# sloisel/MultiGridBarrier.jl

Measured on AMD Instinct MI355X. Metric: Newton iters/sec + wall-clock to converge, 2D P2 p-Laplace L=9, higher is better.
Workload: dtype f64

## Files before the change

### include/mgbhip.h

```cpp
#ifndef MGBHIP_H
#define MGBHIP_H

#include <stdint.h>

#ifdef __cplusplus
extern "C" {
#endif

#define MGBHIP_OK 0
#define MGBHIP_ERR_INVALID 1
#define MGBHIP_ERR_HIP 2
#define MGBHIP_ERR_NOT_SPD 3
#define MGBHIP_ERR_NONFINITE 4
#define MGBHIP_ERR_CONVERGENCE 5

#define MGBHIP_MAX_PIECES 4
#define MGBHIP_MAX_IDX 10
#define MGBHIP_MAX_LIN 4
#define MGBHIP_MAX_ND 13
#define MGBHIP_MAX_NU 4
#define MGBHIP_MAX_OPS 8

#define MGBHIP_KIND_EP 1
#define MGBHIP_KIND_LINEAR 2
// ... 9 lines not shown
    const double* A;
    const double* b;
    const double* p;
    const double* mu;
    double p_const, mu_const;
    const double* select;
} mgbhip_piece;

typedef struct {
    int32_t npieces;
    mgbhip_piece pieces[MGBHIP_MAX_PIECES];
    int32_t feasibility;
    int32_t NC;
} mgbhip_cone;

typedef struct {
    int64_t rows, cols;
    const int32_t* rowptr;
    const int32_t* colidx;
    const double* values;
} mgbhip_csr;

typedef struct {
    int32_t p;
    int64_t N;
    int32_t nu;
    int32_t nD;
    int32_t n_ops;
    const double* ops[MGBHIP_MAX_OPS];
    int32_t D_state[MGBHIP_MAX_ND];
    int32_t D_op[MGBHIP_MAX_ND];
    const double* w;
    int32_t L;
    const mgbhip_csr* R;
    mgbhip_cone cone;
    const double* barrier_weights;
    const double* x;
    int32_t dim;
} mgbhip_problem_desc;

typedef struct {
    double tol;
    double t;
    double kappa;
    int32_t maxit;
    int32_t max_newton;
    double ls_beta, ls_c1;
    int32_t line_search;
    double stop_lambda_tol;
    double stop_theta;
    int32_t finalize;
    double finalize_theta;
    int32_t early_stop;
    int (*stopping_criterion)(double ymin, double ynext, double gmin, double gnorm_next, double ndecmin, double ndec,
                              void* user);
    int (*early_stop_fn)(const double* z, double t, void* user);
    void* user;
} mgbhip_options;

typedef struct {
    int32_t k;
    int32_t L;
    int32_t failure_code;
    double t_final, t_elapsed;
    double solve_seconds;
    int64_t newton_iterations;
    int64_t f0_evals, f1_evals, f2_evals, factorizations;
    int32_t cap_steps;
    int64_t* its;
    double* ts;
    double* kappas;
    double* times;
    double* c_dot_Dz;
} mgbhip_core_result;

int mgbhip_create(mgbhip_ctx** ctx, int device_id, void* hip_stream );
int mgbhip_destroy(mgbhip_ctx* ctx);
const char* mgbhip_last_error(void);
const char* mgbhip_version(void);

int mgbhip_problem_create(mgbhip_ctx* ctx, const mgbhip_problem_desc* desc,
                          mgbhip_problem* share, mgbhip_problem** out);
int mgbhip_problem_destroy(mgbhip_problem* prob);
int mgbhip_problem_set_box(mgbhip_problem* prob, double b, double R);
int mgbhip_problem_set_barrier_weights(mgbhip_problem* prob, const double* bw );
int64_t mgbhip_level_size(const mgbhip_problem* prob, int32_t level);

int mgbhip_f0(mgbhip_problem* prob, int32_t level, const double* s, const double* c,
              const double* z0, double* value);
int mgbhip_f1(mgbhip_problem* prob, int32_t level, const double* s, const double* c,
              const double* z0, double* grad );
int mgbhip_f2(mgbhip_problem* prob, int32_t level, const double* s, const double* c,
              const double* z0, double* values );
int mgbhip_hessian_pattern(mgbhip_problem* prob, int32_t level, int64_t* nnz,
                           const int32_t** rowptr, const int32_t** colidx);
int mgbhip_solve(mgbhip_problem* prob, int32_t level, const double* g, double* x);
int mgbhip_set_hessian(mgbhip_problem* prob, int32_t level, const double* values );
int mgbhip_solve_newton(mgbhip_problem* prob, int32_t level, const double* g, double* x, double* lambda2);
typedef int (*mgbhip_allreduce_fn)(void* user, double* buf, int64_t count, int32_t op, int32_t on_device);
int mgbhip_problem_set_sharding(mgbhip_problem* prob, int32_t level, int64_t n_iface,
                                const int32_t* iface_cols, const double* own_mask );
int mgbhip_problem_set_collective(mgbhip_problem* prob, mgbhip_allreduce_fn allreduce, void* user,
                                  int32_t accepts_device_ptr);
int mgbhip_newton_direction(mgbhip_problem* prob, int32_t level, const double* s, const double* c,
                            const double* z0, double* x, double* lambda2, int32_t* condensed);
int mgbhip_node_barrier(mgbhip_problem* prob, const double* z, double* F , double* Dz );
int mgbhip_node_slack(mgbhip_problem* prob, const double* z, double* slack );

int mgbhip_mgb_core(mgbhip_problem* prob, double* z , const double* c ,
                    const mgbhip_options* opt, mgbhip_core_result* res);
int mgbhip_matched_t(mgbhip_problem* prob, const double* z, const double* c, double t_default,
                     double* t_out);
void mgbhip_default_options(mgbhip_options* opt, int64_t n_nodes);

typedef struct mgbhip_vec mgbhip_vec;
int mgbhip_vec_alloc(mgbhip_ctx* ctx, int64_t len, mgbhip_vec** out);
int mgbhip_vec_free(mgbhip_vec* v);
int64_t mgbhip_vec_len(const mgbhip_vec* v);
int mgbhip_vec_upload(mgbhip_vec* v, const double* host, int64_t len);
int mgbhip_vec_download(const mgbhip_vec* v, double* host, int64_t len);
int mgbhip_vec_fill(mgbhip_vec* v, double value);
int mgbhip_vec_copy(mgbhip_vec* dst, const mgbhip_vec* src);
int mgbhip_vec_axpy(double alpha, const mgbhip_vec* x, mgbhip_vec* y);
int mgbhip_vec_scale(double alpha, mgbhip_vec* x);
int mgbhip_vec_dot(const mgbhip_vec* a, const mgbhip_vec* b, double* out);
int mgbhip_vec_norm(const mgbhip_vec* a, double* out);
int mgbhip_vec_isfinite(const mgbhip_vec* a, int32_t* all_finite);
int mgbhip_f0_d(mgbhip_problem* prob, int32_t level, const mgbhip_vec* s, const mgbhip_vec* c,
                const mgbhip_vec* z0, double* value);
int mgbhip_f1_d(mgbhip_problem* prob, int32_t level, const mgbhip_vec* s, const mgbhip_vec* c,
                const mgbhip_vec* z0, mgbhip_vec* grad);
int mgbhip_f2_d(mgbhip_problem* prob, int32_t level, const mgbhip_vec* s, const mgbhip_vec* c,
                const mgbhip_vec* z0);
int mgbhip_solve_d(mgbhip_problem* prob, int32_t level, const mgbhip_vec* g, mgbhip_vec* x);
int mgbhip_prolong_add(mgbhip_problem* prob, int32_t level, const mgbhip_vec* s, mgbhip_vec* z);

int mgbhip_stage_ms(mgbhip_problem* prob, const char* stage, double* total_ms, int64_t* launches);
int mgbhip_reset_stage_timers(mgbhip_problem* prob, int enable);
int mgbhip_solver_stats(mgbhip_problem* prob, int32_t level, double* out8);
int mgbhip_solver_chain(mgbhip_problem* prob, int32_t level, double* out8);
enum { MGBHIP_PROJ_NONE = 0, MGBHIP_PROJ_LOOP = 1, MGBHIP_PROJ_STAGED = 2, MGBHIP_PROJ_MFMA = 3, MGBHIP_PROJ_ACCUMULATE = 4 };
int mgbhip_level_plan(mgbhip_problem* prob, int32_t level, int32_t* out16);
enum { MGBHIP_ELEM_F0 = 0, MGBHIP_ELEM_F1 = 1, MGBHIP_ELEM_F2 = 2, MGBHIP_ELEM_NODE_F = 3, MGBHIP_ELEM_NODE_SLACK = 4, MGBHIP_ELEM_F01 = 5 };
enum { MGBHIP_ELEM_KIND_DENSE = 0, MGBHIP_ELEM_KIND_WIDE = 1, MGBHIP_ELEM_KIND_FAST_DEFAULT = 2, MGBHIP_ELEM_KIND_FAST_RUNTIME = 3,
       MGBHIP_ELEM_KIND_CONDENSE = 4, MGBHIP_ELEM_KIND_GENERIC = 5 };
int mgbhip_elem_plan(mgbhip_problem* prob, int32_t mode, int32_t* out16);
int mgbhip_trial_values(mgbhip_problem* prob, int32_t level, const double* x, const double* dir, double step, const double* c,
                        const double* z0, double* y, double* g, double* xn, int32_t* moved, int32_t* finite, int32_t* path);
enum { MGBHIP_LAUNCH_ROW = 16 };
enum { MGBHIP_ASM_NONE = 0, MGBHIP_ASM_GATHER = 1, MGBHIP_ASM_COLUMNS = 2 };
enum { MGBHIP_B0_NA = 0, MGBHIP_B0_GATHER = 1, MGBHIP_B0_DIAG0 = 2, MGBHIP_B0_STEP0 = 3 };
enum { MGBHIP_BWD_NA = 0, MGBHIP_BWD_K8 = 1, MGBHIP_BWD_K16 = 2, MGBHIP_BWD_GENERAL = 3 };
int64_t mgbhip_solver_launches(mgbhip_problem* prob, int32_t level, int32_t* out, int64_t cap);

#define MGBHIP_INTERP_FEM1D 1
#define MGBHIP_INTERP_QK 2
#define MGBHIP_INTERP_P1 3
#define MGBHIP_INTERP_P2 4
#define MGBHIP_INTERP_SPECTRAL1D 5
#define MGBHIP_INTERP_SPECTRAL2D 6
#define MGBHIP_INTERP_P2C 7
int mgbhip_interpolate(mgbhip_ctx* ctx, int32_t family, int32_t d, int32_t k, int32_t p, int64_t N,
                       const double* x, const double* table, int32_t ncomp, const double* z, int64_t M,
                       const double* pts, double* out, int32_t* elem);
int mgbhip_interpolate_grad(mgbhip_ctx* ctx, int32_t family, int32_t d, int32_t k, int32_t p, int64_t N,
                            const double* x, const double* table, int32_t ncomp, const double* z, int64_t M,
                            const double* pts, double* out ,
                            double* grad , int32_t* elem );

typedef struct mgbhip_locator mgbhip_locator;
int mgbhip_locator_create(mgbhip_ctx* ctx, int32_t family, int32_t d, int32_t k, int32_t p, int64_t N,
                          const double* x, const double* table, int64_t M, const double* pts,
                          mgbhip_locator** out);
int mgbhip_locator_elements(const mgbhip_locator* loc, int32_t* elem );
int mgbhip_locator_evaluate(mgbhip_locator* loc, int32_t ncomp, const double* z ,
                            double* out ,
                            double* grad );
int mgbhip_locator_destroy(mgbhip_locator* loc);

typedef struct mgbhip_closest mgbhip_closest;
int mgbhip_closest_create(mgbhip_ctx* ctx, int32_t d, int32_t e, int32_t k, int64_t N, const double* x,
                          const double* nodes, int64_t M, const double* pts, double max_distance,
                          mgbhip_closest** out);
int mgbhip_closest_fetch(const mgbhip_closest* cp, int32_t* elem , double* xi ,
                         double* foot , double* dist , int32_t* flag );
int mgbhip_closest_evaluate(mgbhip_closest* cp, int32_t ncomp, const double* z ,
                            double* out ,
                            double* grad );
int mgbhip_closest_destroy(mgbhip_closest* cp);

enum { MGBHIP_QUAD_VALUE = 0, MGBHIP_QUAD_LP = 1, MGBHIP_QUAD_W1P = 2, MGBHIP_QUAD_ENERGY = 3 };
typedef struct mgbhip_quadrature mgbhip_quadrature;
int mgbhip_quadrature_create(mgbhip_ctx* ctx, int32_t d, int32_t e, int32_t p, int64_t N, const double* x, int32_t Q,
                             const double* wref, const double* phi, const double* dphi, mgbhip_quadrature** out);
int mgbhip_quadrature_points(mgbhip_quadrature* quad, double* points );
int mgbhip_quadrature_weights(mgbhip_quadrature* quad, double* weights );
int mgbhip_quadrature_integrate(mgbhip_quadrature* quad, int32_t kind, double pexp, int32_t ncol,
                                const double* z , const double* minus ,
                                const double* source ,
                                double* per_element , double* totals );
int mgbhip_quadrature_max(mgbhip_quadrature* quad, int32_t kind, int32_t ncol, const double* z ,
                          const double* minus , double* maxima );
int mgbhip_quadrature_plan(int32_t d, int32_t e, int32_t p, int32_t Q, int64_t N, int32_t* out16);
int mgbhip_quadrature_times(const mgbhip_quadrature* quad, double* ms2);
int mgbhip_quadrature_destroy(mgbhip_quadrature* quad);

enum { MGBHIP_FACE_VALUE = 0, MGBHIP_FACE_FLUX = 1 };
typedef struct mgbhip_faces mgbhip_faces;
int mgbhip_faces_create(mgbhip_ctx* ctx, int32_t d, int32_t p, int64_t N, const double* x, const int32_t* t, int32_t F,
                        int32_t Qf, const double* wf, const double* phi, const double* dphi, const double* tangents,
                        const double* normals, const int32_t* corners, int32_t ncode, const int32_t* perm,
                        mgbhip_faces** out, int64_t* nboundary, int64_t* ninterior);
int mgbhip_faces_topology(const mgbhip_faces* faces, int32_t* boundary, int32_t* interior, int32_t* orientation,
                          int32_t* element_faces);
int mgbhip_faces_geometry(mgbhip_faces* faces, int32_t which, double* points, double* normals, double* measures);
int mgbhip_faces_sizes(const mgbhip_faces* faces, double* sizes );
int mgbhip_faces_integrate(mgbhip_faces* faces, int32_t kind, double pexp, int32_t ncol, const double* z ,
                           const double* weight , double* per_face ,
                           double* totals );
int mgbhip_faces_jumps(mgbhip_faces* faces, int32_t kind, double pexp, int32_t ncol, const double* z ,
                       double* jumps );
int mgbhip_faces_indicator(mgbhip_faces* faces, double pexp, int32_t ncol, const double* z ,
                           double* eta2 , double* totals );
int mgbhip_faces_plan(int32_t d, int32_t p, int32_t Qf, int32_t F, int32_t sides, int64_t nfaces, int32_t* out16);
int mgbhip_faces_times(const mgbhip_faces* faces, double* ms3);
int mgbhip_faces_destroy(mgbhip_faces* faces);

typedef struct mgbhip_contour mgbhip_contour;
int mgbhip_contour_create(mgbhip_ctx* ctx, int32_t family, int32_t d, int32_t k, int32_t p, int64_t N,
                          const double* x, const double* table, int32_t nfield , const double* fields,
                          int32_t nlevels, const double* levels, int32_t refine,
                          mgbhip_contour** out, int64_t* nsimplices);
int mgbhip_contour_fetch(const mgbhip_contour* c, double* points, int32_t* level, int32_t* element,
                         double* carried );
int mgbhip_contour_destroy(mgbhip_contour* c);

int mgbhip_contour_create_embedded(mgbhip_ctx* ctx, int32_t family, int32_t d, int32_t e, int32_t k, int32_t p,
                                   int64_t N, const double* x , const double* table,
                                   int32_t nfield , const double* fields, int32_t nlevels,
                                   const double* levels, int32_t refine, mgbhip_contour** out, int64_t* nsimplices);

typedef struct mgbhip_tessellation mgbhip_tessellation;
int mgbhip_tessellate_create(mgbhip_ctx* ctx, int32_t family, int32_t d, int32_t e, int32_t k, int32_t p, int64_t N,
                             const double* x , const double* table, int32_t nfield ,
                             const double* fields, int32_t refine, mgbhip_tessellation** out, int64_t* ntriangles);
int mgbhip_tessellate_fetch(const mgbhip_tessellation* t, double* points, int32_t* element,
                            double* values );
int mgbhip_tessellate_destroy(mgbhip_tessellation* t);

typedef struct mgbhip_weld mgbhip_weld;
int mgbhip_weld_create(mgbhip_ctx* ctx, int64_t S, int32_t nv, int32_t e, const double* points,
                       const int32_t* group , double tol, int32_t want_normals,
                       mgbhip_weld** out, int64_t* V, int64_t* ncomponents);
int mgbhip_weld_fetch(const mgbhip_weld* w, int32_t* cells , int32_t* first_corner ,
                      int32_t* component , double* normals );
int mgbhip_weld_rounds(const mgbhip_weld* w, int32_t* vertex_rounds, int32_t* component_rounds);
int mgbhip_weld_destroy(mgbhip_weld* w);

typedef struct mgbhip_polyline mgbhip_polyline;
int mgbhip_polyline_create(mgbhip_ctx* ctx, int64_t V, int32_t e, const double* vertices , int64_t S,
                           const int32_t* cells , mgbhip_polyline** out, int64_t* L, int64_t* P,
                           int64_t* ndropped);
int mgbhip_polyline_fetch(const mgbhip_polyline* pl, int64_t* offsets , int32_t* vertex ,
                          int32_t* segment , uint8_t* closed , double* arclength ,
                          double* length );
int mgbhip_polyline_rounds(const mgbhip_polyline* pl, int32_t* rounds , int32_t* nphases);
int mgbhip_polyline_destroy(mgbhip_polyline* pl);
int mgbhip_polyline_sample(mgbhip_ctx* ctx, int32_t e, int64_t P, const double* points, int32_t C,
                           const double* data , int64_t L, const int64_t* offsets,
                           const double* arclength, int64_t Q, const int32_t* line, const double* s,
                           double* out_points, double* out_data );

typedef struct mgbhip_raycast mgbhip_raycast;
int mgbhip_raycast_create(mgbhip_ctx* ctx, int32_t family, int32_t d, int32_t k, int32_t p, int64_t N,
                          const double* x, const double* table, int64_t R, const double* origin, const double* dir,
                          const double* box, double step, double t_min, double t_max,
                          mgbhip_raycast** out, int64_t* nsamples);
int mgbhip_raycast_offsets(const mgbhip_raycast* rc, int64_t* offsets );
int mgbhip_raycast_samples(const mgbhip_raycast* rc, double* pts );
int mgbhip_raycast_lengths(const mgbhip_raycast* rc, double* step , double* length );
int mgbhip_raycast_integrate(mgbhip_raycast* rc, int32_t ncomp, const double* z ,
                             double* out );
int mgbhip_raycast_render(mgbhip_raycast* rc, const double* u , int32_t K, const double* transfer ,
                          double lo, double hi, double* out );
int mgbhip_raycast_destroy(mgbhip_raycast* rc);
int mgbhip_raycast_render_layers(mgbhip_raycast* rc, const double* u , int32_t K,
                                 const double* transfer , double lo, double hi, int32_t nhits,
                                 const double* t_hit , const double* layer ,
                                 double* out );

typedef struct mgbhip_surface mgbhip_surface;
int mgbhip_surface_create(mgbhip_ctx* ctx, int64_t T, const double* points , mgbhip_surface** out);
int mgbhip_surface_trace(mgbhip_surface* s, int64_t R, const double* origin, const double* dir, double t_min,
                         double t_max, int32_t K, double* t, int32_t* tri, double* u, double* v );
int mgbhip_surface_shade(mgbhip_surface* s, int64_t R, int32_t K, const double* dir, const int32_t* tri,
                         const double* u, const double* v, const double* values , int32_t Kt,
                         const double* table , double lo, double hi, double ambient,
                         double* layer );
int mgbhip_surface_destroy(mgbhip_surface* s);

typedef struct mgbhip_tubes mgbhip_tubes;
int mgbhip_tubes_create(mgbhip_ctx* ctx, int64_t S, const double* points , const double* radii ,
                        mgbhip_tubes** out);
int mgbhip_tubes_trace(mgbhip_tubes* s, int64_t R, const double* origin, const double* dir, double t_min, double t_max,
                       int32_t K, double* t, int32_t* segment, double* sp );
int mgbhip_tubes_shade(mgbhip_tubes* s, int64_t R, int32_t K, const double* origin, const double* dir, const double* t,
// ... 39 lines not shown
```

### multigridbarrier.jl_amd/csrc/api.cpp

```cpp
#include <chrono>
#include <cmath>
#include <cstring>
#include <algorithm>
#include <limits>
#include <memory>
#include <string>

#include "closest.hpp"
#include "contour.hpp"
#include "faces.hpp"
#include "figure.hpp"
#include "interpolate.hpp"
#include "polyline.hpp"
#include "problem.hpp"
#include "quadrature.hpp"
#include "raycast.hpp"
#include "stream.hpp"
#include "surface.hpp"
#include "tubes.hpp"
#include "weld.hpp"

using namespace mgbhip;

mgbhip_problem* problem_create(mgbhip_ctx* ctx, const mgbhip_problem_desc* d, mgbhip_problem* share);
// ... 589 lines not shown
    *value = P->eval_f0(level, s->buf.p, z0->buf.p, c->buf.p);
    return MGBHIP_OK;
    MGB_API_END
}

int mgbhip_f1_d(mgbhip_problem* P, int32_t level, const mgbhip_vec* s, const mgbhip_vec* c, const mgbhip_vec* z0, mgbhip_vec* grad) {
    MGB_API_BEGIN_ON(P)
    check_closure_args(P, level, s, c, z0);
    MGB_REQUIRE(grad && grad->ctx == P->ctx && grad->len == s->len, "grad has the wrong length");
    P->touch();
    P->eval_f1(level, s->buf.p, z0->buf.p, c->buf.p, grad->buf.p);
    return MGBHIP_OK;
    MGB_API_END
}

int mgbhip_f2_d(mgbhip_problem* P, int32_t level, const mgbhip_vec* s, const mgbhip_vec* c, const mgbhip_vec* z0) {
    MGB_API_BEGIN_ON(P)
    check_closure_args(P, level, s, c, z0);
    P->touch();
    P->eval_f2(level, s->buf.p, z0->buf.p, c->buf.p);
    return MGBHIP_OK;
    MGB_API_END
}

int mgbhip_solve_d(mgbhip_problem* P, int32_t level, const mgbhip_vec* g, mgbhip_vec* x) {
    MGB_API_BEGIN_ON(P)
    check_level(P, level);
    MGB_REQUIRE(g && x && g->ctx == P->ctx && x->ctx == P->ctx, "bad vector");
    MGB_REQUIRE(g->len == P->levels[level].m && x->len == g->len, "solve: length mismatch");
    hipStream_t st = P->stream();
    P->factor(level);
    P->trisolve(level, g->buf.p, x->buf.p);
    const int status = P->levels[level].solver.status(st);
    if (status != MGBHIP_OK) g_last_error = "Cholesky met a non-positive pivot";
    return status;
    MGB_API_END
}

int mgbhip_prolong_add(mgbhip_problem* P, int32_t level, const mgbhip_vec* s, mgbhip_vec* z) {
    MGB_API_BEGIN_ON(P)
    check_level(P, level);
    MGB_REQUIRE(s && z && s->ctx == P->ctx && z->ctx == P->ctx, "bad vector");
    const Level& Lv = P->levels[level];
    MGB_REQUIRE(s->len == Lv.m && z->len == Lv.rows, "prolong_add: length mismatch");
    launch_csr_matvec(Lv.rows, Lv.Rptr.p, Lv.Rcol.p, Lv.Rval.p, s->buf.p, z->buf.p, true, false, P->stream());
    P->touch();
    return MGBHIP_OK;
    MGB_API_END
}

static int node_map(mgbhip_problem* P, const double* z, double* F, double* Dz, int mode) {
    MGB_REQUIRE(P && z && F, "null argument");
    hipStream_t st = P->stream();
    P->d_z0.upload(z, (size_t)P->nu * P->n, st);
    ElemParams E = P->elem_params(nullptr);
    E.z0 = P->d_z0.p;
    if (Dz) {
        P->d_nodeDz.ensure((size_t)P->n * P->nD);
        E.out_Dz = P->d_nodeDz.p;
    }
    launch_elem(E, mode, st);
    P->d_nodeF.download(F, (size_t)P->n, st);
    if (Dz) P->d_nodeDz.download(Dz, (size_t)P->n * P->nD, st);
    MGB_HIP_CHECK(hipStreamSynchronize(st));
    return MGBHIP_OK;
}

int mgbhip_node_barrier(mgbhip_problem* P, const double* z, double* F, double* Dz) {
    MGB_API_BEGIN_ON(P)
    return node_map(P, z, F, Dz, MODE_NODE_F);
    MGB_API_END
}

int mgbhip_node_slack(mgbhip_problem* P, const double* z, double* slack) {
    MGB_API_BEGIN_ON(P)
    return node_map(P, z, slack, nullptr, MODE_NODE_SLACK);
    MGB_API_END
}

void mgbhip_default_options(mgbhip_options* o, int64_t n_nodes) {
    const double eps = std::numeric_limits<double>::epsilon();
    o->tol = std::sqrt(eps);
    o->t = 0.1;
    o->kappa = 10.0;
    o->maxit = 10000;
    o->max_newton = (int32_t)std::ceil(std::log2(-std::log2(eps)) + 2);
    o->ls_beta = 0.5;
    o->ls_c1 = 0.1;
    o->line_search = 0;
    o->stop_lambda_tol = 0.25 / std::sqrt((double)n_nodes);
    o->stop_theta = 0.9;
    o->finalize = 1;
    o->finalize_theta = 0.9;
    o->early_stop = 0;
    o->stopping_criterion = nullptr;
    o->early_stop_fn = nullptr;
    o->user = nullptr;
}

int mgbhip_mgb_core(mgbhip_problem* P, double* z, const double* c, const mgbhip_options* opt, mgbhip_core_result* res) {
    MGB_API_BEGIN_ON(P)
    MGB_REQUIRE(P && z && c && opt && res, "null argument");
    MGB_REQUIRE(opt->tol > 0 && opt->t > 0 && opt->kappa > 1 && opt->maxit >= 1 && opt->max_newton >= 1, "bad options");
    int rc = core_run(P, z, c, opt, res);
    if (rc == MGBHIP_ERR_CONVERGENCE)
        g_last_error = res->failure_code == 2 ? "Convergence failure in mgb_solve: iteration_limit"
                                              : "Convergence failure in mgb_solve: stall";
    return rc;
    MGB_API_END
}

int mgbhip_matched_t(mgbhip_problem* P, const double* z, const double* c, double t_default, double* t_out) {
    MGB_API_BEGIN_ON(P)
    MGB_REQUIRE(P && z && c && t_out, "null argument");
    return matched_t_run(P, z, c, t_default, t_out);
    MGB_API_END
}

int mgbhip_stage_ms(mgbhip_problem* P, const char* stage, double* total_ms, int64_t* launches) {
    MGB_API_BEGIN_ON(P)
    MGB_REQUIRE(P && stage, "null argument");
    P->ctx->timers.collect();
    auto it = P->ctx->timers.recs.find(stage);
    if (total_ms) *total_ms = it == P->ctx->timers.recs.end() ? 0.0 : it->second.ms;
    if (launches) *launches = it == P->ctx->timers.recs.end() ? 0 : it->second.launches;
    return MGBHIP_OK;
    MGB_API_END
}

int mgbhip_solver_stats(mgbhip_problem* P, int32_t level, double* out) {
    MGB_API_BEGIN
    check_level(P, level);
    MGB_REQUIRE(out != nullptr, "null argument");
    const Level& L = P->levels[level];
    const MfPlan& pl = L.solver.plan;
    out[0] = (double)pl.fronts.size();
    out[1] = (double)pl.max_m;
    out[2] = (double)pl.arena_doubles;
    out[3] = (double)pl.factor_flops;
    out[4] = (double)pl.peeled;
    out[5] = pl.level_ptr.empty() ? 0.0 : (double)(pl.level_ptr.size() - 1);
    out[6] = (double)L.nnz;
    out[7] = (double)L.m;
    return MGBHIP_OK;
    MGB_API_END
}

int mgbhip_solver_chain(mgbhip_problem* P, int32_t level, double* out) {
    MGB_API_BEGIN
    check_level(P, level);
    MGB_REQUIRE(out != nullptr, "null argument");
    MGB_REQUIRE(P->levels[level].solver.analyzed, "mgbhip_solver_chain: the level has not been factored yet");
    P->levels[level].solver.chain_stats(out);
    return MGBHIP_OK;
    MGB_API_END
}

static_assert(MGBHIP_LAUNCH_ROW == mgbhip::MF_LAUNCH_ROW && MGBHIP_ASM_GATHER == mgbhip::MF_ASM_GATHER &&
              MGBHIP_ASM_COLUMNS == mgbhip::MF_ASM_COLS && MGBHIP_B0_GATHER == mgbhip::MF_B0_GATHER &&
              MGBHIP_B0_DIAG0 == mgbhip::MF_B0_DIAG0 && MGBHIP_B0_STEP0 == mgbhip::MF_B0_STEP0 && MGBHIP_BWD_K8 == mgbhip::MF_BWD_K8 &&
              MGBHIP_BWD_K16 == mgbhip::MF_BWD_K16 && MGBHIP_BWD_GENERAL == mgbhip::MF_BWD_GENERAL, "mgbhip.h and mf_launch_plan.hpp disagree");

int64_t mgbhip_solver_launches(mgbhip_problem* P, int32_t level, int32_t* out, int64_t cap) {
    int64_t count = 0;
    const int rc = [&]() -> int {
        MGB_API_BEGIN
        check_level(P, level);
        MGB_REQUIRE(cap >= 0 && (out != nullptr || cap == 0), "bad output buffer");
        MGB_REQUIRE(P->levels[level].solver.analyzed, "mgbhip_solver_launches: the level has not been factored yet");
        count = P->levels[level].solver.launches(out, cap);
        return MGBHIP_OK;
        MGB_API_END
    }();
    return rc == MGBHIP_OK ? count : -(int64_t)rc;
}

#ifdef MGB_STEP_PROBE
int mgbhip_debug_probe(long long* out64) { (void)hipDeviceSynchronize(); mgbhip::mf_debug_probe(out64); return 0; }
#endif

int mgbhip_reset_stage_timers(mgbhip_problem* P, int enable) {
    MGB_API_BEGIN_ON(P)
    MGB_REQUIRE(P, "null argument");
    P->ctx->timers.reset(enable != 0);
    return MGBHIP_OK;
    MGB_API_END
}

static void interpolate_check_geometry(InterpIn& in) {
    const int32_t family = in.family, d = in.d, k = in.k, p = in.p;
    const int64_t N = in.N;
    const double* x = in.x;
    const bool fem = interp_is_fem(family);
    if (fem) {
        MGB_REQUIRE(x != nullptr && in.table != nullptr, "interpolate: FEM families need node coordinates and a table");
        MGB_REQUIRE(k >= 1 && k <= INTERP_MAX_DEGREE, "interpolate: element degree out of range");
    }
    switch (family) {
        case MGBHIP_INTERP_FEM1D:
            MGB_REQUIRE(d == 1 && p == k + 1, "interpolate: fem1d needs d = 1, p = k + 1");
            in.table_len = k + 1;
            for (int64_t e = 1; e < N && in.sorted; ++e) in.sorted = x[e * p] >= x[(e - 1) * p];
            break;
        case MGBHIP_INTERP_QK: {
            MGB_REQUIRE(d == 2 || d == 3, "interpolate: Q_k needs d = 2 or 3");
            int64_t s = 1;
            for (int a = 0; a < d; ++a) s *= k + 1;
            MGB_REQUIRE(p == s, "interpolate: Q_k needs p = (k + 1)^d");
            in.table_len = k + 1;
            break;
        }
        case MGBHIP_INTERP_P1:
        case MGBHIP_INTERP_P2:
        case MGBHIP_INTERP_P2C:
            MGB_REQUIRE(d == 2, "interpolate: triangles need d = 2");
            MGB_REQUIRE(family == MGBHIP_INTERP_P1 ? p == 3 : (p == 6 || p == 7), "interpolate: bad nodes per triangle");
            in.table_len = (int64_t)p * 10;
            break;
        case MGBHIP_INTERP_SPECTRAL1D:
            MGB_REQUIRE(d == 1 && N == 1 && k >= 0 && p == k + 1, "interpolate: spectral1d needs d = 1, N = 1, p = n");
            in.table = nullptr;
            break;
        case MGBHIP_INTERP_SPECTRAL2D:
            MGB_REQUIRE(d == 2 && N == 1 && k >= 0 && (int64_t)p == (int64_t)(k + 1) * (k + 1),
                        "interpolate: spectral2d needs d = 2, N = 1, p = n^2");
            in.table = nullptr;
            break;
        default:
            throw InvalidArgument("interpolate: unknown family");
    }
    MGB_REQUIRE((int64_t)p * N < (int64_t)INT32_MAX && in.M < (int64_t)INT32_MAX, "interpolate: sizes exceed 32-bit indexing");
}

static void interpolate_checked(mgbhip_ctx* ctx, int32_t family, int32_t d, int32_t k, int32_t p, int64_t N,
                                const double* x, const double* table, int32_t ncomp, const double* z, int64_t M,
                                const double* pts, double* out, double* grad, int32_t* elem) {
    const bool need_out = grad == nullptr;
    MGB_REQUIRE(ctx != nullptr, "null context");
    MGB_REQUIRE(N > 0, "interpolate: no elements (N = 0)");
    MGB_REQUIRE(M >= 0 && ncomp >= 1 && p >= 1, "interpolate: bad sizes");
    MGB_REQUIRE(z != nullptr && (M == 0 || (pts != nullptr && (out != nullptr || !need_out))), "null argument");
    InterpIn in;
    in.family = family; in.d = d; in.k = k; in.p = p; in.N = N; in.ncomp = ncomp; in.M = M;
    in.x = x; in.table = table; in.z = z; in.pts = pts; in.out = out; in.grad = grad; in.elem = elem;
    interpolate_check_geometry(in);
    MGB_REQUIRE(M * ncomp * (grad ? d : 1) < (int64_t)INT32_MAX, "interpolate: sizes exceed 32-bit indexing");
    interpolate_run(in, ctx->stream);
}

int mgbhip_interpolate(mgbhip_ctx* ctx, int32_t family, int32_t d, int32_t k, int32_t p, int64_t N, const double* x,
                       const double* table, int32_t ncomp, const double* z, int64_t M, const double* pts, double* out,
                       int32_t* elem) {
    MGB_API_BEGIN_ON(ctx)
    interpolate_checked(ctx, family, d, k, p, N, x, table, ncomp, z, M, pts, out, nullptr, elem);
    return MGBHIP_OK;
    MGB_API_END
}

int mgbhip_interpolate_grad(mgbhip_ctx* ctx, int32_t family, int32_t d, int32_t k, int32_t p, int64_t N,
                            const double* x, const double* table, int32_t ncomp, const double* z, int64_t M,
                            const double* pts, double* out, double* grad, int32_t* elem) {
    MGB_API_BEGIN_ON(ctx)
    MGB_REQUIRE(grad != nullptr, "interpolate_grad: null gradient array");
    interpolate_checked(ctx, family, d, k, p, N, x, table, ncomp, z, M, pts, out, grad, elem);
    return MGBHIP_OK;
    MGB_API_END
}

int mgbhip_locator_create(mgbhip_ctx* ctx, int32_t family, int32_t d, int32_t k, int32_t p, int64_t N, const double* x,
                          const double* table, int64_t M, const double* pts, mgbhip_locator** out) {
    MGB_API_BEGIN_ON(ctx)
    MGB_REQUIRE(ctx != nullptr, "null context");
    MGB_REQUIRE(out != nullptr, "null output pointer");
    MGB_REQUIRE(N > 0, "interpolate: no elements (N = 0)");
    MGB_REQUIRE(M >= 0 && p >= 1, "interpolate: bad sizes");
    MGB_REQUIRE(M == 0 || pts != nullptr, "null argument");
    InterpIn in;
    in.family = family; in.d = d; in.k = k; in.p = p; in.N = N; in.M = M;
    in.x = x; in.table = table; in.pts = pts;
    interpolate_check_geometry(in);
    create_handle(ctx, out, [&](Locator& L) { locator_build(L, in, ctx->stream); });
    return MGBHIP_OK;
    MGB_API_END
}

int mgbhip_locator_elements(const mgbhip_locator* loc, int32_t* elem) {
    MGB_API_BEGIN_ON(loc)
    MGB_REQUIRE(loc != nullptr, "null locator");
    MGB_REQUIRE(loc->obj.M == 0 || elem != nullptr, "null argument");
    locator_elements(loc->obj, elem, loc->ctx->stream);
    return MGBHIP_OK;
    MGB_API_END
}

int mgbhip_locator_evaluate(mgbhip_locator* loc, int32_t ncomp, const double* z, double* out, double* grad) {
    MGB_API_BEGIN_ON(loc)
    MGB_REQUIRE(loc != nullptr, "null locator");
    const Locator& L = loc->obj;
    MGB_REQUIRE(ncomp >= 1, "interpolate: bad sizes");
    MGB_REQUIRE(z != nullptr && (L.M == 0 || out != nullptr || grad != nullptr), "null argument");
    MGB_REQUIRE(L.M * ncomp * (grad ? L.d : 1) < (int64_t)INT32_MAX, "interpolate: sizes exceed 32-bit indexing");
    locator_evaluate(loc->obj, ncomp, z, out, grad, loc->ctx->stream);
    return MGBHIP_OK;
    MGB_API_END
}

// ... 817 lines not shown
```

### multigridbarrier.jl_amd/csrc/driver.cpp

```cpp
#include <chrono>
#include <cstdio>
#include <cstdlib>
#include <cmath>
#include <cstring>
#include <functional>
#include <limits>

#include "problem.hpp"

using namespace mgbhip;

namespace {

constexpr double EPS = std::numeric_limits<double>::epsilon();

bool debug_on() {
    static const bool on = env_on("MGBHIP_DEBUG");
    return on;
}
#define DBG(...) do { if (debug_on()) { fprintf(stderr, __VA_ARGS__); } } while (0)

struct Stop {
    double lambda_tol;
    double theta;
    int (*fn)(double, double, double, double, double, double, void*) = nullptr;
    void* user = nullptr;
    bool operator()(double ymin, double ynext, double gmin, double gnorm_next, double ndecmin, double ndec) const {
        if (fn) return fn(ymin, ynext, gmin, gnorm_next, ndecmin, ndec, user) != 0;
        const bool exact = (ynext >= ymin) && (gnorm_next >= theta * gmin);
        if (lambda_tol >= 0) return (ndec < lambda_tol) || exact;
        return exact;
    }
};

struct NewtonResult {
    int k = 0;
    bool converged = false;
    double y = 0;
};

struct VecStats { double sumsq, bad; };

VecStats vec_stats(mgbhip_problem* P, int level, const double* d_v, int64_t len) {
    hipStream_t st = P->stream();
    launch_vec_stats(d_v, len, P->d_scratch.p, P->d_scal.p + 2, st, P->own_mask(level));
    P->read_scalars(2, 2);
    if (P->sharded()) P->allreduce_host(P->pin.d + 2, 2, 0);
    return VecStats{P->pin.d[2], P->pin.d[3]};
}

double dev_dot(mgbhip_problem* P, int level, const double* a, const double* b, int64_t len) {
    hipStream_t st = P->stream();
    launch_dot(a, b, len, P->d_scratch.p, P->d_scal.p + 4, st, P->own_mask(level));
    P->read_scalars(4, 1);
    if (P->sharded()) P->allreduce_host(P->pin.d + 4, 1, 0);
    return P->pin.d[4];
}

struct NewtonCtx {
    mgbhip_problem* P;
    int level;
    const double* d_zJ;
    const double* d_c;
    int64_t m;
    double F0(const double* d_s) { return P->eval_f0(level, d_s, d_zJ, d_c); }
    void F1(const double* d_s, double* d_out, double* d_part) { P->eval_f1(level, d_s, d_zJ, d_c, d_out, P->sharded() ? d_part : nullptr); }
    const double* rhs_of_g() const { return P->sharded() ? P->d_gpart.p : P->d_g.p; }
    void F2(const double* d_s) { P->eval_f2(level, d_s, d_zJ, d_c, false, rhs_of_g()); }
};

bool trial_values(NewtonCtx& C, double& ynext, double& gnorm_next, int32_t* moved = nullptr, const double* step = nullptr,
                  bool* restrict_fused_out = nullptr) {
    mgbhip_problem* P = C.P;
    hipStream_t st = P->stream();
    const bool onfly = step && P->can_fuse_step(C.level);
    if (step) {
        ++P->step_stamp;
        if (!onfly) launch_step(P->d_x.p, P->d_nv.p, *step, P->d_xn.p, C.m, P->d_flag.p, P->step_stamp, st);
        P->touch();
    }
    const bool fused = !P->dense;
    static const bool fuse_restrict = !env_on("MGBHIP_NO_FUSED_RESTRICT");
    TrialRestrict fuse;
    TrialPoint point{};
    if (onfly) {
        point = TrialPoint{P->d_x.p, P->d_nv.p, *step};
        fuse = TrialRestrict{P->d_x.p, P->d_nv.p, *step, P->d_xn.p, P->d_flag.p, P->step_stamp};
    }
    const bool restrict_fused = P->eval_f01_launch(C.level, P->d_xn.p, C.d_zJ, C.d_c, P->d_gn.p, P->sharded() ? P->d_gnpart.p : nullptr, fused,
                                                   onfly ? &point : nullptr, (fused && fuse_restrict) ? &fuse : nullptr);
    if (restrict_fused_out) *restrict_fused_out = restrict_fused;
    if (onfly && !restrict_fused) launch_step(P->d_x.p, P->d_nv.p, *step, P->d_xn.p, C.m, P->d_flag.p, P->step_stamp, st);
    const double seq = P->next_seq();
    launch_trial_finish(P->d_gn.p, C.m, P->d_scratch.p, fused ? P->d_partials.p : nullptr, elem_grid(P->p, P->N), P->d_scal.p,
                        P->d_flag.p, P->pin.dev, st, P->own_mask(C.level), seq, restrict_fused);
    P->wait_results(seq);
    P->pin.i[0] = P->pin.d[4] == (double)P->step_stamp ? 1 : 0;
    if (P->sharded()) {
        P->pin.d[1] = (double)P->pin.i[0];
        P->allreduce_host(P->pin.d, 4, 0);
        P->pin.i[0] = P->pin.d[1] != 0.0 ? 1 : 0;
    }
    if (moved) *moved = P->pin.i[0];
    ynext = P->pin.d[0];
    if (!std::isfinite(ynext)) return false;
    if (P->pin.d[3] != 0.0 || !std::isfinite(P->pin.d[2])) return false;
    gnorm_next = std::sqrt(P->pin.d[2]);
    return true;
}

bool linesearch_backtracking(NewtonCtx& C, const mgbhip_options& opt, double y, double inc, double& ynext,
                             double& gnorm_next) {
    mgbhip_problem* P = C.P;
    hipStream_t st = P->stream();
    double s = 1.0;
    bool have = false;
    while (s > 0.0) {
        double yn, gn;
        int32_t moved = 0;
        if (trial_values(C, yn, gn, &moved, &s)) {
            have = true;
            ynext = yn;
            gnorm_next = gn;
            const bool stalled = (moved == 0);
            if (stalled || yn <= y - opt.ls_c1 * inc * s) return true;
        }
        s *= opt.ls_beta;
    }
    return have;
}

bool linesearch_illinois(NewtonCtx& C, const mgbhip_options& opt, double inc, double& ynext, double& gnorm_next) {
    mgbhip_problem* P = C.P;
    hipStream_t st = P->stream();
    struct Reject {};
    auto phi = [&](double sigma) -> double {
        launch_step(P->d_x.p, P->d_nv.p, sigma, P->d_xn.p, C.m, P->d_flag.p, ++P->step_stamp, st);
        P->touch();
        const double f = C.F0(P->d_xn.p);
        if (!std::isfinite(f)) throw Reject();
        C.F1(P->d_xn.p, P->d_gn.p, P->d_gnpart.p);
        const double v = dev_dot(P, C.level, P->d_gn.p, P->d_nv.p, C.m);
        if (!std::isfinite(v)) throw Reject();
        return v;
    };
    double s = 1.0;
    bool have = false;
    while (s > 0.0) {
        try {
            double a = 0.0, b = s, fa = inc, fb = phi(s), root = b;
            bool done = false;
            if (fa == 0) { root = a; done = true; }
            else if (fa * fb >= 0) { root = b; done = true; }
            for (int it = 0; it < 10000 && !done; ++it) {
                const double c = (a * fb - b * fa) / (fb - fa);
                const double fc = phi(c);
                if (c <= std::fmin(a, b) || c >= std::fmax(a, b) || fc * fa == 0 || fc * fb == 0) { root = c; done = true; break; }
                if (fb * fc < 0) { a = b; fa = fb; } else { fa /= 2; }
                b = c; fb = fc;
            }
            if (!done) throw Reject();
            launch_step(P->d_x.p, P->d_nv.p, root, P->d_xn.p, C.m, P->d_flag.p, ++P->step_stamp, st);
        P->touch();
            double yn, gn;
            if (!trial_values(C, yn, gn)) throw Reject();
            ynext = yn;
            gnorm_next = gn;
            return true;
        } catch (Reject&) {
        }
        s *= opt.ls_beta;
    }
    return have;
}

NewtonResult newton(NewtonCtx& C, const mgbhip_options& opt, const Stop& stop, int maxit) {
    mgbhip_problem* P = C.P;
    hipStream_t st = P->stream();
    NewtonResult R;
    P->d_x.zero(st, (size_t)C.m);
    P->touch();
    double y = C.F0(P->d_x.p);
    if (!std::isfinite(y)) throw InvalidArgument("newton: initial objective value is not finite");
    double ymin = y;
    if (P->sharded()) { P->d_gpart.ensure((size_t)C.m); P->d_gnpart.ensure((size_t)C.m); }
    C.F1(P->d_x.p, P->d_g.p, P->d_gpart.p);
    VecStats gs = vec_stats(P, C.level, P->d_g.p, C.m);
    if (gs.bad != 0.0 || !std::isfinite(gs.sumsq)) throw InvalidArgument("newton: initial gradient has non-finite entries");
    double gnorm = std::sqrt(gs.sumsq);
    double gmin = gnorm;
    double incmin = INFINITY;
    int k = 0;
    bool converged = false;
    Level& L = P->levels[C.level];
    struct RobustReset {
        MfSolver& s;
        ~RobustReset() { s.robust = false; }
    } robust_reset{L.solver};
    while (k < maxit && !converged) {
        ++k;
        C.F2(P->d_x.p);
        auto t0 = std::chrono::steady_clock::now();
        int fstatus = MGBHIP_OK;
        int leaf_flag = 0;
        for (int attempt = 0; attempt < 2; ++attempt) {
            P->factor(C.level, C.rhs_of_g());
            P->trisolve_carried(C.level, P->d_nv.p);
            const double seq = P->next_seq();
            launch_dir_finish(P->d_nv.p, P->d_g.p, C.m, P->d_scratch.p, P->d_scal.p, L.solver.status_flags_rw(), P->pin.dev, st,
                              P->own_mask(C.level), seq);
            L.solver.flags_cleared();
            P->wait_results(seq);
            P->pin.i[1] = P->pin.d[5] != 0.0 ? 1 : 0;
            leaf_flag |= P->pin.d[6] != 0.0 ? 1 : 0;
            P->pin.i[2] = leaf_flag;
            fstatus = MfSolver::status_from(P->pin.i + 1, L.solver.factored_condensed);
            if (P->sharded()) {
                P->pin.d[5] = fstatus != MGBHIP_OK ? 1.0 : 0.0;
                P->allreduce_host(P->pin.d + 2, 4, 0);
                fstatus = P->pin.d[5] != 0.0 ? MGBHIP_ERR_NOT_SPD : MGBHIP_OK;
            }
            const bool at_floor = std::fabs(P->pin.d[4]) <= EPS * std::fmax(std::fabs(y), 1.0);
            const bool suspicious = fstatus != MGBHIP_OK || P->pin.d[3] != 0.0 || !std::isfinite(P->pin.d[2]) ||
                                    (!(P->pin.d[4] > 0) && !at_floor);
            if (!suspicious || attempt == 1 || !L.solver.has_inverse_path() || L.solver.robust) break;
            DBG("newton[lev %d] k=%d: direction rejected (status %d, lambda^2=%.3e): refactoring with the substitution kernels\n",
                C.level, k, fstatus, P->pin.d[4]);
            L.solver.robust = true;
            L.H.drop_factors();
        }
        if (fstatus != MGBHIP_OK && P->lu_fallback(C.level, P->d_g.p, P->d_nv.p)) {
            DBG("newton[lev %d] k=%d: LDL' met a zero pivot; direction from the pivoted LU fallback\n", C.level, k);
            launch_dir_finish(P->d_nv.p, P->d_g.p, C.m, P->d_scratch.p, P->d_scal.p, L.solver.status_flags_rw(), P->pin.dev, st,
                              P->own_mask(C.level));
            L.solver.flags_cleared();
            MGB_HIP_CHECK(hipStreamSynchronize(st));
            fstatus = MGBHIP_OK;
        }
        P->cnt.solve_seconds += std::chrono::duration<double>(std::chrono::steady_clock::now() - t0).count();
        if (fstatus != MGBHIP_OK) {
            DBG("newton[lev %d] k=%d: Cholesky met a non-positive pivot (y=%.17g |g|=%.6e)\n", C.level, k, y, gnorm);
            converged = false;
            break;
        }
        if (P->pin.d[3] != 0.0 || !std::isfinite(P->pin.d[2])) throw InvalidArgument("newton: Newton direction has non-finite entries");
        const double inc = P->pin.d[4];
        DBG("newton[lev %d] k=%d y=%.17g |g|=%.6e lambda^2=%.6e\n", C.level, k, y, gnorm, inc);
        if (inc <= 0) {
            converged = std::fabs(inc) <= EPS * std::fmax(std::fabs(y), 1.0);
            break;
        }
        double ynext = y, gnorm_next = gnorm;
        bool moved = (opt.line_search == 1) ? linesearch_illinois(C, opt, inc, ynext, gnorm_next)
                                            : linesearch_backtracking(C, opt, y, inc, ynext, gnorm_next);
        if (!moved) {
            ynext = y;
            gnorm_next = gnorm;
        }
        if (stop(ymin, ynext, gmin, gnorm_next, std::sqrt(incmin), std::sqrt(inc))) converged = true;
        if (moved) {
            std::swap(P->d_x, P->d_xn);
            std::swap(P->d_g, P->d_gn);
            std::swap(P->d_gpart, P->d_gnpart);
        }
        y = ynext;
        gnorm = gnorm_next;
        gmin = std::fmin(gmin, gnorm);
        ymin = std::fmin(ymin, y);
        incmin = std::fmin(inc, incmin);
    }
    DBG("newton[lev %d] done k=%d converged=%d y=%.17g\n", C.level, k, (int)converged, y);
    R.k = k;
    R.converged = converged;
    R.y = y;
    P->cnt.newton += k;
    return R;
}

struct StepResult {
    bool converged;
    std::vector<int64_t> its;
};

StepResult mgb_step(mgbhip_problem* P, const double* d_c, const mgbhip_options& opt, bool finalize_now,
                    bool initial_step) {
    const int L = (int)P->levels.size();
    StepResult out;
    out.its.assign(L, 0);
    hipStream_t st = P->stream();
    const Stop sc{opt.stop_lambda_tol, opt.stop_theta, opt.stopping_criterion, opt.user};
    const Stop fin{-1.0, opt.finalize_theta};
    const size_t zn = (size_t)P->nu * P->n;
    auto eta = [&](int j, int J, const Stop& stop, int maxit) -> bool {
        (void)j;
        const int lev = J - 1;
        MGB_HIP_CHECK(hipMemcpyAsync(P->d_z0.p, P->d_z.p, zn * sizeof(double), hipMemcpyDeviceToDevice, st));
        NewtonCtx C{P, lev, P->d_z0.p, d_c, P->levels[lev].m};
        NewtonResult r = newton(C, opt, stop, maxit);
        out.its[lev] += r.k;
        if (r.converged) {
            const Level& Lv = P->levels[lev];
            StageScope scp(P->ctx->timers, "prolong");
            launch_csr_matvec(Lv.rows, Lv.Rptr.p, Lv.Rcol.p, Lv.Rval.p, P->d_x.p, P->d_z.p, true, false, st);
        }
        return r.converged;
    };
    std::function<bool(int, int)> dac = [&](int j, int J) -> bool {
        const int mn = (initial_step && J - j == 1) ? opt.maxit : opt.max_newton;
        if (eta(j, J, sc, mn)) return true;
        const int jmid = (j + J) / 2;
        if (jmid == j || jmid == J) return false;
        return dac(j, jmid) && dac(jmid, J);
    };
    bool converged = dac(0, L);
    if (finalize_now) {
        const bool foo = eta(L - 1, L, fin, opt.maxit);
        converged = converged && foo;
    }
    out.converged = converged;
    return out;
}

double c_dot_Dz(mgbhip_problem* P, const double* d_c) {
    hipStream_t st = P->stream();
    ElemParams E = P->elem_params(d_c);
    E.z0 = P->d_z.p;
    E.invn = 0.0;
    E.bw = nullptr;
    launch_elem(E, MODE_F0, st);
    launch_reduce_partials(P->d_partials.p, elem_grid(P->p, P->N), P->d_scal.p, st);
    double v;
    P->d_scal.download(&v, 1, st);
    MGB_HIP_CHECK(hipStreamSynchronize(st));
    if (P->sharded()) P->allreduce_host(&v, 1, 0);
    return v;
}

bool slack_feasible(mgbhip_problem* P, std::vector<double>& hbuf) {
    hipStream_t st = P->stream();
    hbuf.resize((size_t)P->n);
    MGB_HIP_CHECK(hipMemcpyAsync(hbuf.data(), P->d_z.p + (size_t)(P->nu - 1) * P->n, (size_t)P->n * sizeof(double),
                                 hipMemcpyDeviceToHost, st));
    MGB_HIP_CHECK(hipStreamSynchronize(st));
    double mx = -INFINITY;
    for (double v : hbuf) mx = std::fmax(mx, v);
    if (P->sharded()) P->allreduce_host(&mx, 1, 1);
    return mx < 0;
}

}

void trial_values_run(mgbhip_problem* P, int level, double step, double* y, int32_t* moved, int32_t* finite, int32_t* path) {
    NewtonCtx C{P, level, P->d_z0.p, P->d_c.p, P->levels[level].m};
    double yn = 0.0, gn = 0.0;
    const bool onfly = P->can_fuse_step(level);
    bool restrict_fused = false;
    *finite = trial_values(C, yn, gn, moved, &step, &restrict_fused) ? 1 : 0;
    *y = yn;
    *path = (onfly ? 1 : 0) | (restrict_fused ? 2 : 0);
}

int core_run(mgbhip_problem* P, double* z, const double* c, const mgbhip_options* optp, mgbhip_core_result* res) {
    const mgbhip_options opt = *optp;
    hipStream_t st = P->stream();
    const size_t zn = (size_t)P->nu * P->n;
    const size_t cn = (size_t)P->n * P->nD;
    const int L = (int)P->levels.size();
    P->prepare_all();
    P->d_z.upload(z, zn, st);
    P->d_c0.upload(c, cn, st);
    P->cnt = Counters();
    auto tb = std::chrono::steady_clock::now();
    auto now = [&] { return std::chrono::duration<double>(std::chrono::steady_clock::now() - tb).count(); };
    double t = opt.t;
    const double target = 1.0 / opt.tol;
    double kappa = opt.kappa;
    const double kappa0 = kappa;
    int k = 1;
    std::vector<double> hbuf;
    double t_first = INFINITY;
    std::vector<double> zhost;
    auto early = [&](double tt) -> bool {
        if (opt.early_stop_fn) {
            zhost.resize(zn);
            P->d_z.download(zhost.data(), zn, st);
            MGB_HIP_CHECK(hipStreamSynchronize(st));
            if (opt.early_stop_fn(zhost.data(), tt, opt.user) != 0) return true;
        }
        if (opt.early_stop != 1) return false;
        if (!slack_feasible(P, hbuf)) return false;
        t_first = std::fmin(t_first, tt);
        return tt >= 2 * t_first;
    };
    auto record = [&](int kk, const std::vector<int64_t>& its, bool add) {
        if (kk - 1 < res->cap_steps && res->its) {
            for (int l = 0; l < L; ++l) {
                if (add) res->its[(size_t)(kk - 1) * L + l] += its[l];
                else res->its[(size_t)(kk - 1) * L + l] = its[l];
            }
        }
    };
    auto setc = [&](double tt) { launch_scale_copy(P->d_c0.p, tt, P->d_c.p, (int64_t)cn, st); };
    res->failure_code = 0;
    res->L = L;
    if (res->times && res->cap_steps > 0) res->times[0] = now();
    setc(t);
    StepResult S = mgb_step(P, P->d_c.p, opt, opt.finalize && t >= target, true);
    if (!S.converged) {
        res->failure_code = 1;
        res->k = 1;
        res->t_final = t;
        res->t_elapsed = now();
        return MGBHIP_ERR_CONVERGENCE;
    }
    record(1, S.its, false);
    auto diag = [&](int kk) {
        if (kk - 1 < res->cap_steps) {
            if (res->ts) res->ts[kk - 1] = t;
            if (res->kappas) res->kappas[kk - 1] = kappa;
            if (res->c_dot_Dz) res->c_dot_Dz[kk - 1] = c_dot_Dz(P, P->d_c0.p);
        }
    };
    diag(1);
    bool stopped_early = false;
    while (t < target && kappa > 1 && k < opt.maxit) {
        if (early(t)) { stopped_early = true; break; }
        ++k;
        if (k - 1 < res->cap_steps && res->its)
            for (int l = 0; l < L; ++l) res->its[(size_t)(k - 1) * L + l] = 0;
        if (res->times && k - 1 < res->cap_steps) res->times[k - 1] = now();
        while (kappa > 1) {
            const double t1 = kappa * t;
            setc(t1);
            P->d_tmp.ensure(zn);
            MGB_HIP_CHECK(hipMemcpyAsync(P->d_tmp.p, P->d_z.p, zn * sizeof(double), hipMemcpyDeviceToDevice, st));
            S = mgb_step(P, P->d_c.p, opt, opt.finalize && t1 >= target, false);
            record(k, S.its, true);
            if (S.converged) {
                int64_t mx = 0;
                for (int64_t v : S.its) mx = std::max(mx, v);
                if ((double)mx <= opt.max_newton * 0.5) kappa = std::fmin(kappa0, kappa * kappa);
                t = t1;
                break;
            }
            MGB_HIP_CHECK(hipMemcpyAsync(P->d_z.p, P->d_tmp.p, zn * sizeof(double), hipMemcpyDeviceToDevice, st));
            kappa = std::sqrt(kappa);
        }
        diag(k);
    }
    bool converged = (t >= target) || stopped_early || early(t);
    res->k = k;
    res->t_final = t;
    res->t_elapsed = now();
    res->solve_seconds = P->cnt.solve_seconds;
    res->newton_iterations = P->cnt.newton;
    res->f0_evals = P->cnt.f0;
    res->f1_evals = P->cnt.f1;
    res->f2_evals = P->cnt.f2;
    res->factorizations = P->cnt.factor;
    P->d_z.download(z, zn, st);
    MGB_HIP_CHECK(hipStreamSynchronize(st));
    if (!converged) {
        res->failure_code = (kappa <= 1) ? 1 : 2;
        return MGBHIP_ERR_CONVERGENCE;
    }
    return MGBHIP_OK;
}

int matched_t_run(mgbhip_problem* P, const double* z, const double* c, double t_default, double* t_out) {
    hipStream_t st = P->stream();
    const size_t zn = (size_t)P->nu * P->n;
    const size_t cn = (size_t)P->n * P->nD;
    const int lev = (int)P->levels.size() - 1;
    const int64_t m = P->levels[lev].m;
    P->d_z0.upload(z, zn, st);
    P->d_c0.upload(c, cn, st);
    P->d_c.zero(st, cn);
    P->d_x.zero(st, (size_t)m);
    P->touch();
    *t_out = t_default;
    const bool sh = P->sharded();
    if (sh) { P->d_gpart.ensure((size_t)m); P->d_gnpart.ensure((size_t)m); }
    P->eval_f1(lev, P->d_x.p, P->d_z0.p, P->d_c.p, P->d_g.p, sh ? P->d_gpart.p : nullptr);
    P->eval_f1(lev, P->d_x.p, P->d_z0.p, P->d_c0.p, P->d_gn.p, sh ? P->d_gnpart.p : nullptr);
    launch_axpy(-1.0, P->d_g.p, P->d_gn.p, m, st);
    if (sh) launch_axpy(-1.0, P->d_gpart.p, P->d_gnpart.p, m, st);
    P->eval_f2(lev, P->d_x.p, P->d_z0.p, P->d_c0.p);
    if (sh) {
        P->d_tmp.ensure((size_t)m + 1);
        P->factor(lev, P->d_gpart.p);
        P->trisolve_carried(lev, P->d_tmp.p);
        int bad = P->levels[lev].solver.status(st) != MGBHIP_OK;
        MGB_HIP_CHECK(hipMemcpyAsync(P->d_nv.p, P->d_tmp.p, sizeof(double) * (size_t)m, hipMemcpyDeviceToDevice, st));
        P->levels[lev].H.drop_factors();
        P->factor(lev, P->d_gnpart.p);
        P->trisolve_carried(lev, P->d_tmp.p);
        bad |= P->levels[lev].solver.status(st) != MGBHIP_OK;
        MGB_HIP_CHECK(hipMemcpyAsync(P->d_xn.p, P->d_tmp.p, sizeof(double) * (size_t)m, hipMemcpyDeviceToDevice, st));
        double fb = bad ? 1.0 : 0.0;
        P->allreduce_host(&fb, 1, 0);
        if (fb != 0.0) return MGBHIP_OK;
    } else {
        P->factor(lev);
        if (P->levels[lev].solver.status(st) != MGBHIP_OK) return MGBHIP_OK;
        P->trisolve(lev, P->d_g.p, P->d_nv.p);
        P->trisolve(lev, P->d_gn.p, P->d_xn.p);
    }
    const double d = dev_dot(P, lev, P->d_gn.p, P->d_xn.p, m);
    const double b = dev_dot(P, lev, P->d_g.p, P->d_xn.p, m) + dev_dot(P, lev, P->d_gn.p, P->d_nv.p, m);
    if (!(d > 0)) return MGBHIP_OK;
    const double tstar = -b / (2 * d);
    if (!(std::isfinite(tstar) && tstar > 0)) return MGBHIP_OK;
    *t_out = std::fmin(std::fmax(tstar, std::sqrt(EPS)), t_default);
    return MGBHIP_OK;
}
```

### multigridbarrier.jl_amd/csrc/kernels.hpp

```cpp
#pragma once
#include "common.hpp"
#include "cone.hpp"
#include "elem_layout.hpp"
#include "panel_layout.hpp"

namespace mgbhip {

struct LeafDesc {
    int64_t F_off;
    int32_t interior;
    uint32_t packed;
};

struct ElemParams {
    int32_t p, nu, nD, nstage;
    int32_t ymask;
    int64_t N, n;
    const double* ops[MGBHIP_MAX_OPS];
    const double* stage_ptr[MGBHIP_MAX_OPS];
    int32_t D_state[MGBHIP_MAX_ND];
    int32_t D_op[MGBHIP_MAX_ND];
    int32_t D_stage[MGBHIP_MAX_ND];
    const double* w;
    const double* c;
    const double* z0;
    const double* bw;
    double invn;
    ConeDev cone;
    double* out_partial;
    double* out_ret;
    double* out_hel;
    double* out_F;
    double* out_Dz;
    int32_t diag_mask;
    int64_t blk_off[MGBHIP_MAX_NU * (MGBHIP_MAX_NU + 1) / 2];
    double* dn_Dz;
    double* dn_Y;
    const LeafDesc* leaf_desc;
    double* leaf_arena;
    const double* leaf_g;
    int64_t leaf_slack0;
    int32_t* leaf_status;
    int32_t leaf_packed;
    const int32_t* zsel;
    const double* zs;
    double* zout;
    const double* zx;
    double zalpha;
    int32_t wide;
};
static_assert(sizeof(ElemParams) <= 4096 - 64, "ElemParams must stay well inside the kernel argument limit");

bool launch_elem_f2_condense(const ElemParams& P, hipStream_t st);

int64_t elem_grid(int p, int64_t N);
inline size_t elem_lds_bytes(const ElemParams& P, int mode) {
    return elem_lds_bytes(elem_threads(P.wide != 0, mode), P.p, P.nu, P.nD, P.nstage, mode);
}
inline bool elem_default_signature(const ElemParams& P) {
    const int NY = P.nD;
    if (P.nu != 2 || P.ymask != (((1 << NY) - 1) & ~1)) return false;
    for (int k = 0; k < NY; ++k) {
        if (P.D_state[k] != (k == NY - 1 ? 1 : 0)) return false;
        if (P.D_stage[k] != ((k == 0 || k == NY - 1) ? -1 : k - 1)) return false;
    }
    return true;
}
inline int elem_unstaged_rows(const ElemParams& P) {
    int cnt = 0;
    for (int k = 0; k < P.nD; ++k) cnt += P.D_stage[k] == -2;
    return cnt;
}
inline ElemPlan elem_plan_of(const ElemParams& P, int mode, bool condensing) {
    return elem_decide(P.p, P.nu, P.nD, P.nstage, P.wide != 0, P.p > 64, elem_unstaged_rows(P) == 0, elem_default_signature(P), mode,
                       condensing, P.N);
}
void launch_elem(const ElemParams& P, int mode, hipStream_t st);

void launch_reduce_partials(const double* partials, int64_t count, double* out, hipStream_t st);
void launch_vec_stats(const double* v, int64_t n, double* scratch, double* stats, hipStream_t st, const double* mask = nullptr,
                      const int32_t* ints = nullptr, int nints = 0);
void launch_dir_stats(const double* v, const double* g, int64_t n, double* scratch, double* stats3, hipStream_t st,
                      const double* mask = nullptr, const int32_t* ints = nullptr, int nints = 0);
void launch_dot(const double* a, const double* b, int64_t n, double* scratch, double* out, hipStream_t st, const double* mask = nullptr);
void launch_restrict_trial(int64_t rows, const int32_t* ptr, const int32_t* col, const double* val, const double* ret, double* g,
                            double* scratch, const double* x, const double* nn, double s, double* xn, int32_t* moved, int32_t stamp,
                            hipStream_t st);
void launch_publish(const double* src, int n, double* host_block, int host_lo, double seq, hipStream_t st);
void launch_dir_finish(const double* v, const double* g, int64_t n, double* scratch, double* scal, int32_t* status2, double* host,
                       hipStream_t st, const double* mask = nullptr, double seq = 0.0);
void launch_trial_finish(const double* g, int64_t n, double* scratch, const double* f0_partials, int64_t f0_count, double* scal,
                         int32_t* moved, double* host, hipStream_t st, const double* mask = nullptr, double seq = 0.0,
                         bool partials_ready = false);
void launch_index_gather(const double* v, const int32_t* idx, int64_t cnt, double* out, hipStream_t st);
void launch_index_scatter(const double* in, const int32_t* idx, int64_t cnt, double* v, hipStream_t st);
int64_t reduce_scratch_doubles(int64_t n);

void launch_csr_matvec(int64_t rows, const int32_t* ptr, const int32_t* col, const double* val,
                       const double* x, double* y, bool add, bool long_rows, hipStream_t st);
int csr_chunks(int64_t max_row_len);
void launch_csr_matvec_chunked(int64_t rows, const int32_t* ptr, const int32_t* col, const double* val,
                               const double* x, double* y, double* scratch, int nchunk, hipStream_t st);
void launch_prolong(int64_t rows, const int32_t* ptr, const int32_t* col, const double* val, const double* s,
                    const double* z0, double* zfull, hipStream_t st);
void launch_step(const double* x, const double* n, double s, double* xn, int64_t len, int32_t* moved, int32_t stamp,
                 hipStream_t st);
void launch_scale_copy(const double* src, double alpha, double* dst, int64_t len, hipStream_t st);
void launch_border_tail(const double* g, double* tail, int64_t m, hipStream_t st);
void launch_axpy(double alpha, const double* x, double* y, int64_t len, hipStream_t st);
void launch_fill(double value, double* y, int64_t len, hipStream_t st);

void launch_gather_shared(int64_t nshared, const int32_t* sh_q, const int32_t* cptr, const int32_t* cidx, const double* slab,
                          double* out, hipStream_t st);
void launch_gather_assemble(int64_t nnz, const int32_t* cptr, const int32_t* cidx, const double* slab,
                            double* Hval, bool long_lists, hipStream_t st, int32_t chunk = 0, int32_t nchunk = 0,
                            double* part = nullptr, const int32_t* qmap = nullptr, int64_t nq = 0);

struct PanelParams {
    int32_t p, nu;
    int64_t N;
    const int32_t* ecol_ptr;
    const double* panels;
    const int32_t* eoff;
    const double* hel;
    double* slab;
    int32_t cmax;
    int32_t upper_only;
    const int32_t* spos;
};
bool launch_panel_project_mfma(const PanelParams& P, hipStream_t st);
void launch_invert_lists(const int32_t* cidx, int64_t total, int32_t* spos, hipStream_t st);
void launch_panel_project(const PanelParams& P, hipStream_t st);
void launch_panel_accumulate(const PanelParams& P, const int32_t* ecols, int32_t m, int32_t nstream, int32_t nsplit,
                             int32_t chunk, int32_t ctmax, double* partial, double* H, hipStream_t st);
void launch_panel_project_staged(const PanelParams& P, int32_t ctmax, hipStream_t st);

}
```

### multigridbarrier.jl_amd/csrc/mf_numeric.hip

```cpp
#include <hip/hip_runtime.h>

#include <cstdio>

#include <algorithm>
#include <cstdlib>

#include "../../include/mgbhip.h"
#include "mf_solver.hpp"
#include "mf_device.hpp"
#include "mf_small.hpp"
#include "mf_big_subst.hpp"
#include "mf_big_inv.hpp"

namespace mgbhip {

namespace {

int32_t query_lds_cap() {
    if (hipFuncSetAttribute((const void*)mf_factor_small<8, true>, hipFuncAttributeMaxDynamicSharedMemorySize,
                            (int)factor_small_lds(128)) == hipSuccess)
        return 128;
    (void)hipGetLastError();
    return 88;
}
bool query_inv_optin() {
    if (hipFuncSetAttribute((const void*)mf_fwd_inv, hipFuncAttributeMaxDynamicSharedMemorySize, (int)fwd_inv_lds(BIG_INV_MAX_M)) == hipSuccess &&
        hipFuncSetAttribute((const void*)mf_bwd_inv, hipFuncAttributeMaxDynamicSharedMemorySize,
                            (int)bwd_inv_lds(BIG_INV_MAX_M, BIG_INV_MAX_M)) == hipSuccess &&
        hipFuncSetAttribute((const void*)mf_bwd_inv_split, hipFuncAttributeMaxDynamicSharedMemorySize,
                            (int)bwd_inv_lds(BIG_INV_MAX_M, BIG_INV_MAX_M)) == hipSuccess)
        return true;
    (void)hipGetLastError();
    return false;
}

void build_gather_lists(const MfPlan& plan, const std::vector<char>& on_big_path, std::vector<FrontDev>& fd,
                        std::vector<int64_t>& ug_ptr, std::vector<int64_t>& ug_src) {
    for (int32_t i = 0; i < (int32_t)plan.fronts.size(); ++i) {
        const Front& f = plan.fronts[i];
        if (!on_big_path[i]) continue;
        fd[i].ug_off = (int64_t)ug_ptr.size();
        std::vector<int32_t> cnt((size_t)f.m + 1, 0);
        for (int32_t c = 0; c < f.nchild; ++c) {
            const Front& ch = plan.fronts[plan.children[f.child_off + c]];
            for (int32_t j = 0; j < ch.m - ch.k; ++j) cnt[plan.rel[ch.rel_off + j] + 1]++;
        }
        const int64_t base = (int64_t)ug_src.size();
        std::vector<int64_t> pos((size_t)f.m + 1);
        pos[0] = base;
        for (int32_t j = 0; j < f.m; ++j) pos[j + 1] = pos[j] + cnt[j + 1];
        ug_ptr.insert(ug_ptr.end(), pos.begin(), pos.end());
        ug_src.resize((size_t)pos[f.m]);
        std::vector<int64_t> fill(pos.begin(), pos.end() - 1);
        for (int32_t c = 0; c < f.nchild; ++c) {
            const Front& ch = plan.fronts[plan.children[f.child_off + c]];
            for (int32_t j = 0; j < ch.m - ch.k; ++j) ug_src[(size_t)fill[plan.rel[ch.rel_off + j]]++] = ch.u_off + j;
        }
    }
    if (ug_ptr.empty()) ug_ptr.push_back(0);
    if (ug_src.empty()) ug_src.push_back(0);
}

bool pack_leaf_fronts(const MfPlan& plan, const LevelLaunches& levels, const std::vector<char>& on_big_path,
                      std::vector<FrontDev>& fd) {
    if (!leaf_fronts_packable(plan, levels, on_big_path)) return false;
    for (auto& lev : levels)
        for (auto& L : lev)
            if (L.tiny)
                for (int32_t q = L.first; q < L.first + L.count; ++q) fd[q].packed = 1;
    return true;
}

std::vector<int32_t> remap_a_dst(const MfPlan& plan, const LevelLaunches& levels) {
    std::vector<int32_t> ad(plan.a_dst);
    for (auto& lev : levels)
        for (auto& L : lev) {
            const int stride = L.tiny ? 16 : (L.wave ? (L.cls <= 32 ? 32 : 48) : 0);
            const bool lds_front = L.cls >= 88 && !stride;
            if (!stride && !lds_front) continue;
            for (int32_t q = L.first; q < L.first + L.count; ++q) {
                const Front& f = plan.fronts[q];
                const int32_t sd = lds_front ? f.m : stride;
                for (int32_t t = 0; t < f.a_cnt; ++t) {
                    const int32_t d = plan.a_dst[f.a_off + t], lu = d % f.m, lv = d / f.m;
                    ad[f.a_off + t] = lv * sd - lv * (lv - 1) / 2 + (lu - lv);
                }
            }
        }
    return ad;
}

void dump_plan(const MfPlan& plan, const LevelLaunches& levels) {
    fprintf(stderr, "[mgbhip] solver plan: n=%lld fronts=%d levels=%d arena=%.1f MB\n", (long long)plan.n, (int)plan.fronts.size(),
            (int)levels.size(), plan.arena_doubles * 8e-6);
    for (size_t l = 0; l < levels.size(); ++l)
        for (auto& L : levels[l]) {
            double sm = 0, sk = 0, fl = 0;
            for (int32_t q = L.first; q < L.first + L.count; ++q) {
                const Front& f = plan.fronts[q];
                sm += f.m; sk += f.k;
                for (int c = 0; c < f.k; ++c) fl += (double)(f.m - c) * (f.m - c);
            }
            fprintf(stderr, "[mgbhip]   level %2d cls %3d count %7d max_m %4d max_k %4d avg_m %6.1f avg_k %6.1f Mflop %8.2f\n",
                    (int)l, L.cls, L.count, L.max_m, L.max_k, sm / L.count, sk / L.count, fl * 1e-6);
        }
}

StageTimers g_dummy_timers;
struct LevelScope {
    char nm[32];
    StageScope scope;
    static StageTimers& timers_or_dummy(StageTimers* t) {
        static const bool on = env_on("MGBHIP_LEVEL_TIMING");
        return (t && on) ? *t : g_dummy_timers;
    }
    LevelScope(StageTimers* t, const char* sweep, int level)
        : scope(timers_or_dummy(t), (snprintf(nm, sizeof(nm), "%s_lv%02d", sweep, level), nm)) {}
};

}

void MfSolver::upload_plan(hipStream_t st) {
    d_front_idx.upload(plan.front_idx, st);
    d_children.upload(plan.children, st);
    d_rel.upload(plan.rel, st);
    d_a_src.upload(plan.a_src, st);
    d_a_colptr.upload(plan.a_colptr, st);
    d_arena.alloc((size_t)std::max<int64_t>(plan.arena_doubles, 1));
    d_uvec.alloc((size_t)std::max<int64_t>(plan.uvec_doubles, 1));
    d_y.alloc((size_t)plan.n + 1);
    y_zero = y_border_one = status_zero = leaf_zero = false;
    d_bx.alloc((size_t)plan.n + 1);
    d_xx.alloc((size_t)plan.n + 1);
    {
        const double one = 1.0;
        d_one.upload(&one, 1, st);
        MGB_HIP_CHECK(hipStreamSynchronize(st));
    }
    d_tbig.alloc(plan.front_idx.size() ? plan.front_idx.size() : 1);
    d_tsol.alloc(plan.front_idx.size() ? plan.front_idx.size() : 1);
    d_dvec.alloc(plan.front_idx.size() ? plan.front_idx.size() : 1);
    d_status.alloc(2);
    d_status.zero(st);
}

void MfSolver::analyze(int64_t n, const int32_t* rowptr, const int32_t* colidx, hipStream_t st,
                       const double* coords, int dim, bool protect_peeled, const int32_t* top, int64_t ntop) {
    const MfSwitches sw = MfSwitches::from_env();
    MfOptions opt;
    opt.protect_peeled = protect_peeled;
    opt.top = top;
    opt.ntop = ntop;
    opt.border = true;
    mf_analyze(n, rowptr, colidx, opt, plan, sw.no_geo ? nullptr : coords, dim);
    const int32_t nf = (int32_t)plan.fronts.size();
    std::vector<FrontDev> fd(nf);
    for (int32_t i = 0; i < nf; ++i) {
        const Front& f = plan.fronts[i];
        fd[i] = FrontDev{f.k, f.m, f.nchild, f.a_cnt, f.F_off, f.idx_off, f.u_off, f.child_off, f.rel_off, f.a_off, f.acol_off, -1, 0, 0};
    }
    upload_plan(st);

    lds_cap = query_lds_cap();
    const bool inv_ok = !sw.old_big && query_inv_optin();
    level_launches = classify_launches(plan, lds_cap, inv_ok, sw);
    level_solves = merge_level_solves(level_launches);
    uses_inv = false;
    const std::vector<char> on_big_path = fronts_on_big_path(plan, level_launches);
    int32_t max_big = 1;
    for (auto& lev : level_launches)
        for (auto& L : lev) {
            uses_inv = uses_inv || L.inv;
            if (!L.cls) max_big = std::max(max_big, L.count);
        }
    d_dscr.alloc((size_t)max_big * 2 * NB * NB);
    {
        int64_t need[2] = {0, 0};
        if (sw.bwd_split) bwd_split_scratch(level_solves, need);
        if (need[0] == 0) { d_bwd_g.release(); d_bwd_cnt.release(); }
        else {
            d_bwd_g.alloc((size_t)need[1]);
            d_bwd_cnt.alloc((size_t)need[0]);
            d_bwd_cnt.zero(st);
        }
    }

    std::vector<int64_t> ug_ptr, ug_src;
    build_gather_lists(plan, on_big_path, fd, ug_ptr, ug_src);
    leaf_packed = sw.packed_leaves && pack_leaf_fronts(plan, level_launches, on_big_path, fd);
    d_ug_ptr.upload(ug_ptr, st);
    d_ug_src.upload(ug_src, st);
    std::vector<GatherRec> grec;
    std::vector<int32_t> gmap;
    if (!sw.gather_lds_maps) build_gather_maps(plan, level_launches, grec, gmap);
    gather_ct = sw.gather_ct;
    if (grec.empty()) { d_grec.release(); d_gmap.release(); }
    else { d_grec.upload(grec, st); d_gmap.upload(gmap, st); }
    d_fronts.upload(fd, st);
    h_fronts = fd;
    h_a_dst = remap_a_dst(plan, level_launches);
    d_a_dst.upload(h_a_dst, st);
    if (debug_level() >= 2) dump_plan(plan, level_launches);
    analyzed = true;
    MGB_HIP_CHECK(hipStreamSynchronize(st));
}

void MfSolver::set_direct_map(const int32_t* value_map, int64_t nnz, int64_t tail_base, hipStream_t st) {
    std::vector<int32_t> as(plan.a_src.size());
    for (size_t t = 0; t < as.size(); ++t) {
        const int64_t src = plan.a_src[t];
        const int64_t v = src < nnz ? (int64_t)value_map[src] : tail_base + (src - nnz);
        MGB_REQUIRE(v < (int64_t)INT32_MAX, "direct value index exceeds 32 bits");
        as[t] = (int32_t)v;
    }
    d_a_src_direct.upload(as, st);
    MGB_HIP_CHECK(hipStreamSynchronize(st));
}

void MfSolver::factor(const double* d_values, hipStream_t st, StageTimers* timers, bool direct, bool condensed) {
    MGB_REQUIRE(!direct || d_a_src_direct.n > 0, "MfSolver::factor: no direct value map");
    MGB_REQUIRE(!condensed || (direct && condensed_ok), "MfSolver::factor: condensed leaves are not enabled");
    MGB_REQUIRE(analyzed, "MfSolver::factor before analyze");
    const FactorArgs a{condensed ? d_fronts_c.p : d_fronts.p, d_children.p, d_rel.p,
                       condensed ? d_a_src_c.p : (direct ? d_a_src_direct.p : d_a_src.p), condensed ? d_a_dst_c.p : d_a_dst.p,
                       condensed ? d_a_colptr_c.p : d_a_colptr.p, d_values, d_arena.p, d_dscr.p, d_dvec.p, d_status.p, st,
                       d_grec.n ? d_grec.p : nullptr, d_gmap.p, gather_ct};
    if (timers) timers->begin("factor");
    factored_inv = !robust;
    if (!status_zero) MGB_HIP_CHECK(hipMemsetAsync(d_status.p, 0, sizeof(int32_t), st));
    status_zero = false;
    factored_condensed = condensed;
    int lvno = -1;
    for (auto& lev : level_launches) {
        LevelScope lvscope(timers, "fac", ++lvno);
        for (auto& L : lev) {
            if (L.count == 0) continue;
            if (condensed && lvno == 0) continue;
            if (L.tiny) launch_factor_tiny(a, L);
            else if (L.wave && L.cls <= 32) launch_factor_wave<32>(a, L);
            else if (L.wave) launch_factor_wave<48>(a, L);
            else if (L.cls) launch_factor_small(a, L);
            else {
                const bool inv = L.inv && !robust;
                const MfBlock0 b0 = big_block0_kind(L, inv);
                MGB_REQUIRE(!L.iface || (bool)iface_reduce, "MfSolver: interface front without a reduction hook");
                launch_big_assemble(a, L, b0 == MF_B0_GATHER);
                if (L.iface) {
                    const Front& fi = plan.fronts[L.first];
                    const int64_t tri = (int64_t)fi.m * (fi.m + 1) / 2;
                    d_ifpack.ensure((size_t)tri);
                    launch_tri_pack(fi.m, d_arena.p + fi.F_off, d_ifpack.p, false, st);
                    iface_reduce(d_ifpack.p, tri);
                    launch_tri_pack(fi.m, d_arena.p + fi.F_off, d_ifpack.p, true, st);
                }
                if (inv) {
                    if (b0 == MF_B0_DIAG0) launch_big_diag0(a, L, L.count);
                    launch_inv_steps(a, L, L.count, b0 == MF_B0_STEP0);
                } else
                    launch_subst_steps(a, L, L.count);
            }
        }
    }
    MGB_HIP_CHECK(hipGetLastError());
    if (timers) timers->end();
}

void MfSolver::solve(const double* d_b, double* d_x, hipStream_t st, StageTimers* timers) {
    MGB_REQUIRE(analyzed, "MfSolver::solve before analyze");
    if (timers) timers->begin("trisolve");
    const size_t n = (size_t)plan.n;
    MGB_HIP_CHECK(hipMemcpyAsync(d_bx.p, d_b, n * sizeof(double), hipMemcpyDeviceToDevice, st));
    MGB_HIP_CHECK(hipMemsetAsync(d_bx.p + n, 0, sizeof(double), st));
    forward_pass(d_bx.p, st, timers);
    backward_pass(d_xx.p, st, timers);
    MGB_HIP_CHECK(hipMemcpyAsync(d_x, d_xx.p, n * sizeof(double), hipMemcpyDeviceToDevice, st));
    MGB_HIP_CHECK(hipGetLastError());
    if (timers) timers->end();
}

void MfSolver::solve_border(double* d_x_np1, hipStream_t st, StageTimers* timers) {
    MGB_REQUIRE(analyzed, "MfSolver::solve_border before analyze");
    if (timers) timers->begin("trisolve");
    const size_t n = (size_t)plan.n;
    if (!y_zero) {
        MGB_HIP_CHECK(hipMemsetAsync(d_y.p, 0, n * sizeof(double), st));
        y_zero = true;
    }
    if (!y_border_one) {
        MGB_HIP_CHECK(hipMemcpyAsync(d_y.p + n, d_one.p, sizeof(double), hipMemcpyDeviceToDevice, st));
        y_border_one = true;
    }
    backward_pass(d_x_np1, st, timers);
    MGB_HIP_CHECK(hipGetLastError());
    if (timers) timers->end();
}

void MfSolver::forward_pass(const double* d_b, hipStream_t st, StageTimers* timers) {
    y_border_one = false;
    y_zero = false;
    const SolveArgs a = solve_args(d_b, nullptr, st);
    int lvno = -1;
    for (auto& lev : level_solves) {
        LevelScope lvscope(timers, "fwd", ++lvno);
        for (auto& L : lev) {
            if (L.count == 0) continue;
            if (L.tiny) launch_forward_tiny(a, L);
            else if (L.cls) launch_forward_small(a, L);
            else if (L.inv && factored_inv) launch_fwd_inv(a, L);
            else if (L.max_m <= BIG1_MAX_M) launch_fwd_big1(a, L);
            else launch_fwd_big_steps(a, L);
        }
    }
}

void MfSolver::backward_pass(double* d_x, hipStream_t st, StageTimers* timers) {
    const SolveArgs a = solve_args(nullptr, d_x, st);
    for (int32_t l = (int32_t)level_solves.size() - 1; l >= 0; --l) {
        LevelScope lvscope(timers, "bwd", l);
        for (auto it = level_solves[l].rbegin(); it != level_solves[l].rend(); ++it) {
            const MfLaunch& L = *it;
            if (L.count == 0) continue;
            if (L.tiny) launch_backward_tiny(a, L);
            else if (L.cls) launch_backward_small(a, L);
            else if (L.inv && factored_inv) launch_bwd_inv(a, L);
            else if (L.max_m <= BIG1_MAX_M) launch_bwd_big1(a, L);
            else launch_bwd_big_steps(a, L);
        }
    }
}

#ifdef MGB_STEP_PROBE
void mf_debug_probe(long long* out64) {
    (void)hipMemcpyFromSymbol(out64, HIP_SYMBOL(g_probe), 64 * sizeof(long long));
    long long init[64];
    for (int i = 0; i < 64; ++i) init[i] = 0;
    init[56] = 0x7fffffffffffffffll;
    (void)hipMemcpyToSymbol(HIP_SYMBOL(g_probe), init, sizeof(init));
}
#endif

void MfSolver::chain_stats(double* out) const {
    double blocks = 0, big_levels = 0, fac = 0, bwd = 0, extra = 0;
    for (auto& lev : level_launches) {
        int lev_blocks = 0;
        for (auto& L : lev) {
            if (L.count == 0) continue;
            if (L.tiny || L.wave || L.cls) { fac += 1; continue; }
            const int nb = (L.max_k + NB - 1) / NB;
            lev_blocks = std::max(lev_blocks, nb);
            fac += 1 + nb + (L.iface ? 3 : 0);
            for (int32_t q = L.first; q < L.first + L.count; ++q) {
                const Front& f = plan.fronts[q];
                const double mk = (double)(f.m - f.k), steps = (double)((f.k + NB - 1) / NB);
                extra += 2.0 * 0.5 * (mk * mk + mk * f.k) * std::max(0.0, steps - 1.0);
            }
        }
        if (lev_blocks) { big_levels += 1; blocks += lev_blocks; }
    }
    for (auto& lev : level_solves)
        for (auto& L : lev)
            if (L.count) bwd += 1;
    out[0] = blocks; out[1] = big_levels; out[2] = fac; out[3] = bwd;
    out[4] = (double)plan.arena_doubles; out[5] = (double)plan.factor_flops; out[6] = extra; out[7] = 0.0;
}

int64_t MfSolver::launches(int32_t* out, int64_t cap) const {
    return launch_rows(level_launches, level_solves, leaf_packed, robust, out, cap);
}

void MfSolver::status_async(int32_t* h_dst2, hipStream_t st) const {
    MGB_HIP_CHECK(hipMemcpyAsync(h_dst2, d_status.p, 2 * sizeof(int32_t), hipMemcpyDeviceToHost, st));
}

int MfSolver::status(hipStream_t st) {
    int32_t h[2] = {0, 0};
    d_status.download(h, 2, st);
    MGB_HIP_CHECK(hipStreamSynchronize(st));
    return status_from(h, factored_condensed);
}

bool MfSolver::enable_condensed(int64_t N, int P, const int32_t* ucol, int64_t slack0, int64_t nnz, int64_t tail_base,
                                hipStream_t st) {
    condensed_ok = false;
    int why = 0;
    struct Report { int& w; ~Report() { if (w) if (debug_level() >= 2) fprintf(stderr, "[mgbhip] condensed leaves: plan shape check %d failed\n", w); } } report{why};
    const int32_t nlev = (int32_t)plan.level_ptr.size() - 1;
    if (!analyzed || !plan.border || nlev < 2 || P > 7) { why = 1; return false; }
    const int32_t n0 = plan.level_ptr[1];
    if ((int64_t)n0 != N) { why = 2; return false; }
    const int32_t nbor = (int32_t)plan.n;
    std::vector<LeafDesc> desc((size_t)N);
    std::vector<char> seen((size_t)N, 0);
    for (int32_t i = 0; i < n0; ++i) {
        const Front& f = plan.fronts[i];
        const int32_t* idx = plan.front_idx.data() + f.idx_off;
        if (f.k != P + 1 || f.m > 15 || f.nchild != 0 || idx[f.m - 1] != nbor) { why = 3; return false; }
        const int64_t e = ((int64_t)idx[0] - slack0) / P;
        if (e < 0 || e >= N || seen[(size_t)e]) { why = 4; return false; }
        for (int q = 0; q < P; ++q)
            if ((int64_t)idx[q] != slack0 + e * P + q) { why = 5; return false; }
        if (idx[P] != ucol[e * P + (P - 1)] || idx[P] < 0) { why = 6; return false; }
        uint32_t packed = (uint32_t)f.m;
        int found = 0;
        for (int q = 0; q < P - 1; ++q) {
            uint32_t pos = 15;
            const int32_t c = ucol[e * P + q];
            if (c >= 0)
                for (int32_t t = P + 1; t < f.m - 1; ++t)
                    if (idx[t] == c) { pos = (uint32_t)t; ++found; break; }
            packed |= pos << (4 + 4 * q);
        }
        if (found != f.m - 1 - (P + 1)) { why = 7; return false; }
        for (int q = 0; q < P - 1; ++q)
            if (ucol[e * P + q] >= 0 && ((packed >> (4 + 4 * q)) & 15u) == 15u) { why = 8; return false; }
        packed |= 15u << (4 + 4 * (P - 1));
        desc[(size_t)e] = LeafDesc{f.F_off, idx[P], packed};
        seen[(size_t)e] = 1;
    }
    const int32_t nf = (int32_t)plan.fronts.size();
    std::vector<FrontDev> fd(h_fronts);
    std::vector<int32_t> as, ad, ac;
    for (int32_t i = 0; i < nf; ++i) {
        const Front& f = plan.fronts[i];
        fd[i].a_off = (int64_t)as.size();
        fd[i].acol_off = (int64_t)ac.size();
        const int32_t* cp = plan.a_colptr.data() + f.acol_off;
        for (int32_t c = 0; c < f.k; ++c) {
            ac.push_back((int32_t)((int64_t)as.size() - fd[i].a_off));
            if (i < n0) continue;
            for (int32_t t = cp[c]; t < cp[c + 1]; ++t) {
                const int64_t src = plan.a_src[f.a_off + t];
                if (src < nnz) continue;
                const int64_t v = tail_base + (src - nnz);
                if (v >= (int64_t)INT32_MAX) return false;
                as.push_back((int32_t)v);
                ad.push_back(h_a_dst[f.a_off + t]);
            }
        }
        fd[i].a_cnt = (int32_t)((int64_t)as.size() - fd[i].a_off);
        ac.push_back(fd[i].a_cnt);
    }
    if (as.empty()) { as.push_back(0); ad.push_back(0); }
    d_fronts_c.upload(fd, st);
    d_a_src_c.upload(as, st);
    d_a_dst_c.upload(ad, st);
    d_a_colptr_c.upload(ac, st);
    d_leaf_desc.upload(desc, st);
    MGB_HIP_CHECK(hipStreamSynchronize(st));
    condensed_ok = true;
    return true;
}

}
```

### multigridbarrier.jl_amd/csrc/mf_solver.hpp

```cpp
#pragma once
#include <functional>

#include "common.hpp"
#include "mf_analysis.hpp"
#include "mf_launch_plan.hpp"
#include "kernels.hpp"

namespace mgbhip {

struct FrontDev {
    int32_t k, m, nchild, a_cnt;
    int64_t F_off, idx_off, u_off, child_off, rel_off, a_off, acol_off;
    int64_t ug_off;
    int32_t packed;
    int32_t pad_;
};

struct FactorArgs {
    const FrontDev* fr;
    const int32_t *children, *rel, *a_src, *a_dst, *a_colptr;
    const double* values;
    double *arena, *dscr, *dvec;
    int32_t* status;
    hipStream_t st;
    const GatherRec* grec;
    const int32_t* gmap;
    int gather_ct;
};
struct SolveArgs {
    const FrontDev* fr;
    const int32_t *front_idx, *children, *rel;
    const int64_t *ug_ptr, *ug_src;
    const double *arena, *dvec;
    const double* b;
    double *y, *x, *uvec, *tbig, *tsol;
    hipStream_t st;
    double* bwd_g;
    uint32_t* bwd_cnt;
};

class MfSolver {
   public:
    MfPlan plan;
    void analyze(int64_t n, const int32_t* rowptr, const int32_t* colidx, hipStream_t st,
                 const double* coords = nullptr, int dim = 0, bool protect_peeled = false,
                 const int32_t* top = nullptr, int64_t ntop = 0);
    std::function<void(double*, int64_t)> iface_reduce;
    void factor(const double* d_values, hipStream_t st, StageTimers* timers, bool direct = false, bool condensed = false);
    bool enable_condensed(int64_t N, int P, const int32_t* ucol, int64_t slack0, int64_t nnz, int64_t tail_base, hipStream_t st);
    bool condensed_ready() const { return condensed_ok; }
    bool leaves_packed() const { return leaf_packed; }
    const LeafDesc* leaf_desc() const { return d_leaf_desc.p; }
    double* arena() { return d_arena.p; }
    int32_t* leaf_status() { return d_status.p + 1; }
    const int32_t* status_flags() const { return d_status.p; }
    int32_t* status_flags_rw() { return d_status.p; }
    void flags_cleared() { status_zero = true; leaf_zero = true; }
    bool leaf_flag_zero() const { return leaf_zero; }
    void leaf_flag_used() { leaf_zero = false; }
    void set_direct_map(const int32_t* value_map, int64_t nnz, int64_t tail_base, hipStream_t st);
    bool has_direct_map() const { return d_a_src_direct.n > 0; }
    void solve(const double* d_b, double* d_x, hipStream_t st, StageTimers* timers);
    void solve_border(double* d_x_np1, hipStream_t st, StageTimers* timers);
    void chain_stats(double* out8) const;
    int64_t launches(int32_t* out, int64_t cap) const;
    int status(hipStream_t st);
    void status_async(int32_t* h_dst, hipStream_t st) const;
    static int status_from(const int32_t* flags2, bool with_leaves) {
        return (flags2[0] || (with_leaves && flags2[1])) ? MGBHIP_ERR_NOT_SPD : MGBHIP_OK;
    }
    bool factored_condensed = false;
    bool analyzed = false;
    bool robust = false;
    bool has_inverse_path() const { return uses_inv; }
    bool factored_inv = false;

   private:
    void upload_plan(hipStream_t st);
    SolveArgs solve_args(const double* d_b, double* d_x, hipStream_t st) const {
        return {d_fronts.p, d_front_idx.p, d_children.p, d_rel.p, d_ug_ptr.p, d_ug_src.p, d_arena.p, d_dvec.p, d_b, d_y.p, d_x,
                d_uvec.p, d_tbig.p, d_tsol.p, st, d_bwd_g.p, d_bwd_cnt.n ? d_bwd_cnt.p : nullptr};
    }
    void forward_pass(const double* d_b_np1, hipStream_t st, StageTimers* timers);
    void backward_pass(double* d_x_np1, hipStream_t st, StageTimers* timers);
    DevBuf<double> d_bx, d_xx, d_one;
    DevBuf<FrontDev> d_fronts;
    DevBuf<int32_t> d_front_idx, d_children, d_rel, d_a_src, d_a_src_direct, d_a_dst, d_a_colptr;
    DevBuf<GatherRec> d_grec;
    DevBuf<int32_t> d_gmap;
    DevBuf<int64_t> d_ug_ptr, d_ug_src;
    DevBuf<double> d_arena, d_uvec, d_y, d_tbig, d_tsol, d_dscr, d_dvec;
    DevBuf<double> d_ifpack;
    DevBuf<int32_t> d_status;
    DevBuf<double> d_bwd_g;
    DevBuf<uint32_t> d_bwd_cnt;
    bool condensed_ok = false;
    bool leaf_packed = false;
    std::vector<FrontDev> h_fronts;
    std::vector<int32_t> h_a_dst;
    DevBuf<FrontDev> d_fronts_c;
    DevBuf<int32_t> d_a_src_c, d_a_dst_c, d_a_colptr_c;
    DevBuf<LeafDesc> d_leaf_desc;
    std::vector<std::vector<MfLaunch>> level_launches;
    std::vector<std::vector<MfLaunch>> level_solves;
    int gather_ct = 0;
    int32_t lds_cap = 88;
    bool uses_inv = false;
    bool y_border_one = false;
    bool y_zero = false;
    bool status_zero = false, leaf_zero = false;
};

}
```

### multigridbarrier.jl_amd/csrc/problem.cpp

```cpp
#include "problem.hpp"
#include "assembly_plan.hpp"
#include "plan_device.hpp"
#include "dense.hpp"

#include <algorithm>
#include <cmath>
#include <cstdio>
#include <atomic>
#include <exception>
#include <cstdlib>
#include <string>
#include <thread>
#include <cstring>
#include <numeric>

using namespace mgbhip;



static void upload_csr(const mgbhip_csr& R, Level& L, hipStream_t st) {
    MGB_REQUIRE(R.rows >= 0 && R.cols >= 0 && R.rowptr && (R.rowptr[R.rows] == 0 || (R.colidx && R.values)),
                "bad prolongation CSR");
    MGB_REQUIRE(R.rows < INT32_MAX && R.cols < INT32_MAX, "prolongation too large for 32-bit indices");
    L.rows = R.rows;
// ... 540 lines not shown
        launch_restrict_trial(L.m, L.Tptr.p, L.Tcol.p, L.Tval.p, d_ret.p, d_gout, d_scratch.p, fuse->x, fuse->n, fuse->s,
                              fuse->xn, fuse->moved, fuse->stamp, st);
        return true;
    }
    if (L.T_chunks > 0)
        launch_csr_matvec_chunked(L.m, L.Tptr.p, L.Tcol.p, L.Tval.p, d_ret.p, d_gout, d_tchunk.p, L.T_chunks, st);
    else
        launch_csr_matvec(L.m, L.Tptr.p, L.Tcol.p, L.Tval.p, d_ret.p, d_gout, false, L.T_long, st);
    return false;
}

void mgbhip_problem::eval_f1(int level, const double* d_s, const double* d_zz, const double* d_cc, double* d_gout, double* d_part) {
    {
        StageScope sc(ctx->timers, stage_name(STAGE_F1, level));
        ElemParams E = elem_params(d_cc);
        launch_elem_at(E, MODE_F1, level, d_s, d_zz);
    }
    restrict_ret(level, d_gout);
    if (levels[level].sharded) reduce_interface(level, d_gout, d_part);
    cnt.f1++;
}

bool mgbhip_problem::eval_f01_launch(int level, const double* d_s, const double* d_zz, const double* d_cc, double* d_gout,
                                     double* d_part, bool defer_f0_sum, const TrialPoint* trial, const TrialRestrict* fuse) {
    MGB_REQUIRE(!trial || can_fuse_step(level), "a trial point is given only on a level whose element kernel forms it on the fly");
    if (dense) {
        eval_f0_launch(level, d_s, d_zz, d_cc);
        eval_f1(level, d_s, d_zz, d_cc, d_gout, d_part);
        return false;
    }
    hipStream_t st = stream();
    {
        StageScope sc(ctx->timers, stage_name(STAGE_F01, level));
        ElemParams E = elem_params(d_cc);
        launch_elem_at(E, MODE_F01, level, d_s, d_zz, trial);
        if (!defer_f0_sum) launch_reduce_partials(d_partials.p, elem_grid(p, N), d_scal.p, st);
    }
    const bool fused = restrict_ret(level, d_gout, fuse);
    if (levels[level].sharded) reduce_interface(level, d_gout, d_part);
    cnt.f0++;
    cnt.f1++;
    return fused;
}

bool mgbhip_problem::try_enable_condensed(int level) {
    Level& L = levels[level];
    static const bool off = env_on("MGBHIP_NO_CONDENSE");
    if (off || dense || !L.selection || !L.direct || nu != 2 || p != 7 || L.hRptr.empty()) return false;
    if (!L.solver.analyzed || !L.solver.has_direct_map()) return false;
    const int64_t slack0 = L.m - n;
    if (slack0 < 0 || L.rows != 2 * n) return false;
    std::vector<int32_t> ucol((size_t)n, -1);
    for (int64_t node = 0; node < n; ++node) {
        const int32_t b = L.hRptr[node], e = L.hRptr[node + 1];
        if (e - b > 1) return false;
        if (e - b == 1) ucol[(size_t)node] = L.hRcol[b];
        const int64_t rs = n + node;
        if (L.hRptr[rs + 1] - L.hRptr[rs] != 1 || (int64_t)L.hRcol[L.hRptr[rs]] != slack0 + node) return false;
    }
    const bool ok = L.solver.enable_condensed(N, p, ucol.data(), slack0, L.nnz, hel_cap + L.nshared, stream());
    if (debug_level() >= 2)
        fprintf(stderr, "[mgbhip] level %d: condensed leaves %s\n", level, ok ? "enabled" : "not applicable");
    return ok;
}

void mgbhip_problem::eval_f2(int level, const double* d_s, const double* d_zz, const double* d_cc, bool materialize,
                             const double* rhs) {
    ensure_plan(level);
    hipStream_t st = stream();
    Level& L = levels[level];
    int E_ymask = 0;
    if (L.condense && !materialize && rhs != nullptr && L.selection && L.direct && !dense) {
        StageScope sc(ctx->timers, stage_name(STAGE_F2, level));
        ElemParams E = elem_params(d_cc);
        const bool writes_zfull = bind_point(E, level, d_s, d_zz);
        E.leaf_desc = L.solver.leaf_desc();
        E.leaf_arena = L.solver.arena();
        E.leaf_g = rhs;
        E.leaf_slack0 = L.m - n;
        E.leaf_status = L.solver.leaf_status();
        E.leaf_packed = L.solver.leaves_packed() ? 1 : 0;
        if (!L.solver.leaf_flag_zero()) MGB_HIP_CHECK(hipMemsetAsync(E.leaf_status, 0, sizeof(int32_t), st));
        L.solver.leaf_flag_used();
        if (launch_elem_f2_condense(E, st)) {
            if (writes_zfull) zf = PointKey{zstamp, level, d_s, d_zz};
            L.H.written_condensed(hel_owner, level, rhs);
            cnt.f2++;
            return;
        }
    }
    L.proj_kernel = MGBHIP_PROJ_NONE;
    {
        StageScope sc(ctx->timers, stage_name(STAGE_F2, level));
        ElemParams E = elem_params(d_cc);
        E_ymask = E.ymask;
        E.diag_mask = (L.selection && !dense) ? diag_mask_sel : 0;
        hel_layout(nu, N, p, E.diag_mask, E.blk_off);
        launch_elem_at(E, MODE_F2, level, d_s, d_zz);
    }
    {
        StageScope sc(ctx->timers, stage_name(STAGE_ASSEMBLE, level));
        if (dense) {
            int klo = nD, khi = -1;
            for (int k = 0; k < nD; ++k)
                if ((E_ymask >> k) & 1) { klo = std::min(klo, k); khi = std::max(khi, k); }
            const int64_t ld = (int64_t)nD * n;
            if (khi < klo) {
                MGB_HIP_CHECK(hipMemsetAsync(L.Hval.p, 0, sizeof(double) * (size_t)L.nnz, st));
            } else {
                launch_dense_weight(nD, klo, khi, n, L.m, ld, L.denseDR.p, d_dnY.p, L.denseW.p, st);
                launch_dense_gemm_tn((int)L.m, (int)L.m, (int)((khi - klo + 1) * n), L.denseDR.p + (int64_t)klo * n, ld,
                                     nullptr, L.denseW.p + (int64_t)klo * n, ld, L.Hval.p, L.m, false, true, st);
            }
        } else if (L.selection && L.direct && !materialize) {
            launch_gather_shared(L.nshared, L.sh_q.p, L.cptr.p, L.cidx.p, d_hel.p, d_hel.p + hel_cap, st);
        } else if (L.selection) {
            launch_gather_assemble(L.nnz, L.cptr.p, L.cidx.p, d_hel.p, L.Hval.p, L.long_lists, st, L.gather_chunk, L.gather_nchunk, L.gather_part.p);
        } else {
            PanelParams PP;
            PP.p = p; PP.nu = nu; PP.N = N;
            PP.ecol_ptr = L.ecol_ptr.p; PP.panels = L.panels.p; PP.eoff = L.eoff.p;
            PP.hel = d_hel.p; PP.slab = L.slab.p; PP.cmax = L.cmax; PP.spos = nullptr;
            static const bool full_h = env_on("MGBHIP_FULL_COARSE_H");
            const bool upper = !materialize && rhs != nullptr && L.nup > 0 && !L.acc && !full_h;
            PP.upper_only = upper ? 1 : 0;
            if (L.acc) {
                L.proj_kernel = MGBHIP_PROJ_ACCUMULATE;
                launch_panel_accumulate(PP, L.ecols.p, (int32_t)L.m, L.acc_waves, L.acc_split, L.acc_chunk, L.acc_ctmax,
                                        L.acc_copies.p, L.Hval.p, st);
            } else {
                PP.spos = L.sorted_slab ? L.spos.p : nullptr;
                if (launch_panel_project_mfma(PP, st)) {
                    L.proj_kernel = MGBHIP_PROJ_MFMA;
                } else if (panel_accumulate_lds(p, nu, L.acc_ctmax) <= 40 * 1024) {
                    L.proj_kernel = MGBHIP_PROJ_STAGED;
                    launch_panel_project_staged(PP, L.acc_ctmax, st);
                } else {
                    L.proj_kernel = MGBHIP_PROJ_LOOP;
                    launch_panel_project(PP, st);
                }
                launch_gather_assemble(L.nnz, L.cptr.p, L.sorted_slab ? nullptr : L.cidx.p, L.slab.p, L.Hval.p, L.long_lists, st, L.gather_chunk,
                                       L.gather_nchunk, L.gather_part.p, upper ? L.upq.p : nullptr, upper ? L.nup : 0);
            }
        }
    }
    if (L.selection && L.direct && !materialize && !dense) L.H.written_to_slab(hel_owner, level);
    else L.H.written_to_csr(hel_owner);
    cnt.f2++;
}

void mgbhip_problem::wait_results(double seq) {
    static const bool poll = !env_on("MGBHIP_NO_POLL");
    hipStream_t st = stream();
    if (poll && seq != 0.0) {
        volatile const double* stamp = pin.d + 15;
        const Stopwatch sw;
        for (int spins = 0;; ++spins) {
            if (__atomic_load_n(reinterpret_cast<const volatile uint64_t*>(stamp), __ATOMIC_ACQUIRE) ==
                *reinterpret_cast<const uint64_t*>(&seq))
                return;
            if ((spins & 1023) == 1023 && sw.seconds() > 1e-3)
                break;
        }
    }
    MGB_HIP_CHECK(hipStreamSynchronize(st));
}

void mgbhip_problem::read_scalars(int lo, int n) {
    const double seq = next_seq();
    launch_publish(d_scal.p + lo, n, pin.dev, lo, seq, stream());
    wait_results(seq);
}

bool mgbhip_problem::can_fuse_step(int level) const {
    static const bool off = env_on("MGBHIP_NO_FUSED_STEP");
    return !off && !dense && !sharded() && levels[level].R_unit;
}

void mgbhip_problem::ensure_analysis(int level) {
    Level& L = levels[level];
    if (L.solver.analyzed) return;
    hipStream_t st = stream();
    const Stopwatch sw;
    std::vector<double> cen;
    if (!hx.empty() && xdim > 0 && !L.hRptr.empty()) {
        cen.assign((size_t)L.m * xdim, 0.0);
        std::vector<double> wsum((size_t)L.m, 0.0);
        for (int64_t r = 0; r < L.rows; ++r) {
            const int64_t node = r % n;
            for (int32_t q = L.hRptr[r]; q < L.hRptr[r + 1]; ++q) {
                const double a = std::fabs(L.hRval[q]);
                const int32_t j = L.hRcol[q];
                wsum[j] += a;
                for (int d = 0; d < xdim; ++d) cen[(size_t)j * xdim + d] += a * hx[(size_t)d * n + node];
            }
        }
        for (int64_t j = 0; j < L.m; ++j)
            for (int d = 0; d < xdim; ++d) cen[(size_t)j * xdim + d] = wsum[j] > 0 ? cen[(size_t)j * xdim + d] / wsum[j] : 0.0;
    }
    const bool leaves = L.selection && L.direct && !dense && nu == 2 && p == 7;
    if (L.sharded) {
        mgbhip_problem* self = this;
        L.solver.iface_reduce = [self](double* d, int64_t cnt2) { self->allreduce_device(d, cnt2, 0); };
    }
    L.solver.analyze(L.m, L.hHptr.data(), L.hHcol.data(), st, cen.empty() ? nullptr : cen.data(), xdim, leaves,
                     L.sharded ? L.h_iface.data() : nullptr, L.sharded ? (int64_t)L.h_iface.size() : 0);
    if (debug_level() >= 2)
        fprintf(stderr, "[mgbhip] symbolic analysis level %d (m=%lld, nnz=%lld): %.2f s\n", level, (long long)L.m,
                (long long)L.nnz, sw.seconds());
}

void mgbhip_problem::prepare_all() {
    if (prepared) return;
    prepared = true;
    static const bool off = env_on("MGBHIP_LAZY_PLANS");
    if (off || dense || sharded() || levels.size() < 2) return;
    const int Ln = (int)levels.size();
    const Stopwatch prep_sw;
    std::vector<std::exception_ptr> errors((size_t)Ln);
    std::atomic<int> next{Ln - 1};
    auto worker = [&] {
        (void)hipSetDevice(ctx->device);
        for (int l = next.fetch_sub(1); l >= 0; l = next.fetch_sub(1)) {
            try {
                Level& L = levels[l];
                if (L.sharded) continue;
                ensure_plan(l);
                if (L.m < 1) continue;
                ensure_analysis(l);
                ensure_direct(l);
            } catch (...) {
                errors[(size_t)l] = std::current_exception();
            }
        }
    };
    const int nthreads = std::min(Ln, 3);
    std::vector<std::thread> pool;
    for (int t = 1; t < nthreads; ++t) pool.emplace_back(worker);
    worker();
    for (auto& t : pool) t.join();
    if (debug_level() >= 2)
        fprintf(stderr, "[mgbhip] prepare_all: %d levels in %.3f s\n", Ln, prep_sw.seconds());
    for (size_t l = 0; l < errors.size(); ++l) {
        if (!errors[l]) continue;
        (void)hipGetLastError();
        if (debug_level() >= 1) {
            try { std::rethrow_exception(errors[l]); }
            catch (const std::exception& ex) { fprintf(stderr, "[mgbhip] prepare: level %zu left to the lazy path (%s)\n", l, ex.what()); }
            catch (...) { fprintf(stderr, "[mgbhip] prepare: level %zu left to the lazy path\n", l); }
        }
    }
}

void mgbhip_problem::ensure_direct(int level) {
    Level& L = levels[level];
    if (!(L.selection && L.direct) || dense || !L.solver.analyzed) return;
    hipStream_t st = stream();
    const bool dbg2 = debug_level() >= 2;
    if (!L.solver.has_direct_map()) {
        const Stopwatch sw;
        L.solver.set_direct_map(L.h_vmap.data(), L.nnz, hel_cap + L.nshared, st);
        std::vector<int32_t>().swap(L.h_vmap);
        if (dbg2) fprintf(stderr, "[mgbhip] direct value map level %d: %.2f s\n", level, sw.seconds());
    }
    if (!L.condense_tried) {
        const Stopwatch sw;
        L.condense_tried = true;
        L.condense = try_enable_condensed(level);
        if (dbg2) fprintf(stderr, "[mgbhip] condensed-leaf set-up level %d: %.2f s\n", level, sw.seconds());
    }
}

void mgbhip_problem::factor(int level, const double* rhs) {
    Level& L = levels[level];
    const FactorPlan plan = L.H.about_to_factor(hel_owner, level, rhs);
    hipStream_t st = stream();
    ensure_analysis(level);
    if (plan.slab()) {
        ensure_direct(level);
        launch_border_tail(rhs, d_hel.p + hel_cap + L.nshared, L.m, st);
        L.solver.factor(d_hel.p, st, &ctx->timers, true, plan.condensed());
    } else {
        if (plan.write == HTail::Rhs) {
            launch_border_tail(rhs, L.Hval.p + L.nnz, L.m, st);
        } else if (plan.write == HTail::Identity) {
            MGB_HIP_CHECK(hipMemsetAsync(L.Hval.p + L.nnz, 0, sizeof(double) * (size_t)L.m, st));
            launch_fill(1.0, L.Hval.p + L.nnz + L.m, 1, st);
        }
        L.solver.factor(L.Hval.p, st, &ctx->timers);
    }
    L.H.factors_ready(plan);
    cnt.factor++;
}

bool mgbhip_problem::lu_fallback(int level, const double* d_g, double* d_xout) {
    Level& L = levels[level];
    static const bool off = env_on("MGBHIP_NO_LU_FALLBACK");
    if (off || sharded() || !L.H.in_csr() || L.m < 1 || L.m > DENSE_LU_MAX_M || L.Hval.n < (size_t)L.nnz || !L.Hptr.p || !L.Hcol.p)
        return false;
    hipStream_t st = stream();
    d_lu.ensure((size_t)L.m * (size_t)L.m);
    d_lustat.ensure(1);
    d_lustat.zero(st, 1);
    launch_dense_lu_solve((int)L.m, L.Hptr.p, L.Hcol.p, L.Hval.p, d_lu.p, d_g, d_xout, d_lustat.p, st);
    int32_t bad = 1;
    d_lustat.download(&bad, 1, st);
    MGB_HIP_CHECK(hipStreamSynchronize(st));
    if (bad == 0) ++lu_fallbacks;
    return bad == 0;
}

void mgbhip_problem::trisolve(int level, const double* d_g, double* d_xout) {
    Level& L = levels[level];
    L.H.may_solve();
    L.solver.solve(d_g, d_xout, stream(), &ctx->timers);
}

void mgbhip_problem::trisolve_carried(int level, double* d_xout_np1) {
    Level& L = levels[level];
    L.H.may_solve_carried();
    L.solver.solve_border(d_xout_np1, stream(), &ctx->timers);
}
```

### multigridbarrier.jl_amd/csrc/problem.hpp

```cpp
#pragma once
#include <mutex>
#include <memory>
#include <string>
#include <vector>

#include "../../include/mgbhip.h"
#include "common.hpp"
#include "hessian_state.hpp"
#include "kernels.hpp"
#include "mf_solver.hpp"

struct mgbhip_ctx {
    int device = 0;
    hipStream_t stream = nullptr;
    bool own_stream = false;
    mgbhip::StageTimers timers;
    mgbhip::DevBuf<double> vscratch, vscal;
};

struct mgbhip_vec {
    mgbhip_ctx* ctx = nullptr;
    mgbhip::DevBuf<double> buf;
    int64_t len = 0;
};

namespace mgbhip {

struct OpStore {
    std::vector<DevBuf<double>> ops;
    std::vector<bool> identity;
    DevBuf<double> w;
};

struct Level {
    int64_t rows = 0, m = 0;
    std::vector<int32_t> hRptr, hRcol;
    std::vector<double> hRval;
    DevBuf<int32_t> Rptr, Rcol, Tptr, Tcol;
    DevBuf<double> Rval, Tval;
    bool T_long = false, R_long = false;
    int32_t max_row = 0, max_col = 0;
    bool R_unit = false;
    DevBuf<int32_t> Rsel;
    int32_t T_chunks = 0;
    bool planned = false;
    bool selection = false;
    bool acc = false;
    int32_t acc_waves = 0, acc_ctmax = 0;
    int32_t acc_split = 1, acc_chunk = 0;
    DevBuf<double> acc_copies;
    std::vector<int32_t> hHptr, hHcol;
    DevBuf<int32_t> Hptr, Hcol, cptr, cidx, ecol_ptr, ecols, eoff;
    DevBuf<int32_t> spos;
    bool sorted_slab = false;
    DevBuf<double> Hval, panels, slab;
    int64_t slab_doubles = 0;
    int32_t cmax = 1;
    bool long_lists = false;
    int64_t list_total = 0;
    int32_t proj_kernel = 0;
    int32_t gather_chunk = 0, gather_nchunk = 0;
    DevBuf<double> gather_part;
    DevBuf<int32_t> upq;
    int64_t nup = 0;
    int64_t nnz = 0;
    DevBuf<double> denseDR, denseW;
    MfSolver solver;
    HessianState H;
    bool direct = false;
    int64_t nshared = 0;
    DevBuf<int32_t> sh_q;
    std::vector<int32_t> h_vmap;
    bool sharded = false;
    std::vector<int32_t> h_iface;
    DevBuf<int32_t> d_iface;
    DevBuf<double> own, iface_buf;
    bool condense_tried = false, condense = false;
};

struct TrialPoint { const double* x; const double* dir; double alpha; };

struct TrialRestrict { const double* x = nullptr; const double* n = nullptr; double s = 0.0;
                       double* xn = nullptr; int32_t* moved = nullptr; int32_t stamp = 0; };

struct Counters {
    int64_t f0 = 0, f1 = 0, f2 = 0, factor = 0, newton = 0;
    double solve_seconds = 0;
};

}

struct mgbhip_problem {
    mgbhip_ctx* ctx = nullptr;
    int32_t p = 0, nu = 0, nD = 0;
    int64_t N = 0, n = 0;
    int32_t diag_mask_sel = 0;
    bool dense = false;
    bool wide = false;
    std::shared_ptr<mgbhip::OpStore> store;
    int32_t D_state[MGBHIP_MAX_ND], D_op[MGBHIP_MAX_ND], D_stage[MGBHIP_MAX_ND];
    int32_t nstage = 0;
    const double* stage_ptr[MGBHIP_MAX_OPS];
    mgbhip::ConeDev cone;
    std::vector<mgbhip::DevBuf<double>> cone_grids;
    mgbhip::DevBuf<double> bw;
    bool has_bw = false;
    std::vector<mgbhip::Level> levels;
    std::vector<double> hx;
    int32_t xdim = 0;
    mgbhip::DevBuf<double> d_z, d_z0, d_zfull, d_c, d_ret, d_hel, d_partials, d_scal, d_scratch, d_nodeF, d_nodeDz, d_dnDz, d_dnY, d_tchunk;
    mgbhip::DevBuf<double> d_x, d_g, d_nv, d_xn, d_gn, d_tmp, d_c0;
    mgbhip::DevBuf<int32_t> d_flag;
    int32_t step_stamp = 0;
    mgbhip::PinnedBuf pin;
    mgbhip::Counters cnt;
    int64_t zstamp = 0;
    struct PointKey {
        int64_t stamp = -1; int level = -1; const double* s = nullptr; const double* z = nullptr;
        bool operator==(const PointKey& o) const { return stamp == o.stamp && level == o.level && s == o.s && z == o.z; }
    } zf;
    void touch() { ++zstamp; }
    mgbhip_allreduce_fn coll_fn = nullptr;
    void* coll_user = nullptr;
    bool coll_device = false;
    bool sharded() const { return coll_fn != nullptr; }
    std::vector<double> coll_host;
    void allreduce_host(double* h, int64_t count, int op);
    void allreduce_device(double* d, int64_t count, int op);
    void reduce_interface(int level, double* d_g, double* d_part);
    const double* own_mask(int level) const { return levels[level].sharded ? levels[level].own.p : nullptr; }
    mgbhip::DevBuf<double> d_gpart, d_gnpart;

    mgbhip::ElemParams elem_params(const double* d_cc) const;
    bool bind_point(mgbhip::ElemParams& E, int level, const double* d_s, const double* d_zz, const mgbhip::TrialPoint* trial = nullptr);
    void launch_elem_at(mgbhip::ElemParams& E, int mode, int level, const double* d_s, const double* d_zz,
                        const mgbhip::TrialPoint* trial = nullptr);
    enum Stage { STAGE_F0, STAGE_F1, STAGE_F01, STAGE_F2, STAGE_ASSEMBLE };
    const char* stage_name(Stage s, int level) const;
    bool restrict_ret(int level, double* d_gout, const mgbhip::TrialRestrict* fuse = nullptr);
    hipStream_t stream() const { return ctx->stream; }
    void ensure_plan(int level);
    void ensure_analysis(int level);
    void ensure_direct(int level);
    void prepare_all();
    double next_seq() { return ++result_seq; }
    void wait_results(double seq);
    bool can_fuse_step(int level) const;
    void read_scalars(int lo, int n);
    double result_seq = 0.0;
    std::mutex shared_mutex;
    bool prepared = false;
    void ensure_plan_dense(int level);
    double eval_f0(int level, const double* d_s, const double* d_zz, const double* d_cc);
    void eval_f0_launch(int level, const double* d_s, const double* d_zz, const double* d_cc);
    void eval_f1(int level, const double* d_s, const double* d_zz, const double* d_cc, double* d_gout, double* d_part = nullptr);
    bool eval_f01_launch(int level, const double* d_s, const double* d_zz, const double* d_cc, double* d_gout, double* d_part = nullptr,
                         bool defer_f0_sum = false, const mgbhip::TrialPoint* trial = nullptr, const mgbhip::TrialRestrict* fuse = nullptr);
    void eval_f2(int level, const double* d_s, const double* d_zz, const double* d_cc, bool materialize = true,
                 const double* rhs = nullptr);
    bool try_enable_condensed(int level);
    int64_t hel_cap = 0;
    mgbhip::SlabOwner hel_owner;
    void factor(int level, const double* rhs = nullptr);
    void trisolve(int level, const double* d_g, double* d_xout);
    void trisolve_carried(int level, double* d_xout_np1);
    bool lu_fallback(int level, const double* d_g, double* d_xout);
    mgbhip::DevBuf<double> d_lu;
    mgbhip::DevBuf<int32_t> d_lustat;
    int64_t lu_fallbacks = 0;
};
```

### multigridbarrier.jl_amd/csrc/vector_kernels.hpp

```cpp
#pragma once
#include "reduce_kernels.hpp"

namespace mgbhip {

namespace {


template <bool ADD>
__global__ __launch_bounds__(256) void csr_matvec_row_kernel(int64_t rows, const int32_t* __restrict__ ptr,
                                                             const int32_t* __restrict__ col,
                                                             const double* __restrict__ val,
                                                             const double* __restrict__ x, double* __restrict__ y) {
    const int64_t i = (int64_t)blockIdx.x * 256 + threadIdx.x;
    if (i >= rows) return;
    double s = 0.0;
    for (int32_t q = ptr[i]; q < ptr[i + 1]; ++q) s += val[q] * x[col[q]];
    y[i] = ADD ? y[i] + s : s;
}

template <bool ADD>
__global__ __launch_bounds__(256) void csr_matvec_wave_kernel(int64_t rows, const int32_t* __restrict__ ptr,
                                                              const int32_t* __restrict__ col,
                                                              const double* __restrict__ val,
                                                              const double* __restrict__ x, double* __restrict__ y) {
    const int lane = threadIdx.x & 63;
    const int64_t i = (int64_t)blockIdx.x * 4 + (threadIdx.x >> 6);
    if (i >= rows) return;
    DSum a;
    for (int32_t q = ptr[i] + lane; q < ptr[i + 1]; q += 64) a.add(val[q] * x[col[q]]);
    dsum_wave_reduce(a);
    if (lane == 0) y[i] = ADD ? y[i] + a.value() : a.value();
}

constexpr int CHUNK = 4096;
__global__ __launch_bounds__(256) void csr_matvec_chunk_kernel(const int32_t* __restrict__ ptr,
                                                               const int32_t* __restrict__ col,
                                                               const double* __restrict__ val,
                                                               const double* __restrict__ x,
                                                               double* __restrict__ partial, int nchunk) {
    __shared__ double red[256];
    const int row = blockIdx.y, ch = blockIdx.x, tid = threadIdx.x;
    const int32_t q0 = ptr[row] + ch * CHUNK;
    const int32_t q1 = min(ptr[row + 1], q0 + CHUNK);
    __shared__ double redc[256];
    DSum a;
    for (int32_t q = q0 + tid; q < q1; q += 256) a.add(val[q] * x[col[q]]);
    red[tid] = a.s;
    redc[tid] = a.c;
    __syncthreads();
    for (int off = 128; off > 0; off >>= 1) {
        if (tid < off) {
            DSum b;
            b.s = red[tid]; b.c = redc[tid];
            b.merge(red[tid + off], redc[tid + off]);
            red[tid] = b.s; redc[tid] = b.c;
        }
        __syncthreads();
    }
    if (tid == 0) {
        partial[2 * ((int64_t)row * nchunk + ch)] = red[0];
        partial[2 * ((int64_t)row * nchunk + ch) + 1] = redc[0];
    }
}

__global__ __launch_bounds__(256) void csr_matvec_chunk_sum_kernel(int64_t rows, const double* __restrict__ partial,
                                                                   int nchunk, double* __restrict__ y) {
    const int lane = threadIdx.x & 63;
    const int64_t i = (int64_t)blockIdx.x * 4 + (threadIdx.x >> 6);
    if (i >= rows) return;
    DSum a;
    for (int c = lane; c < nchunk; c += 64) a.merge(partial[2 * (i * nchunk + c)], partial[2 * (i * nchunk + c) + 1]);
    dsum_wave_reduce(a);
    if (lane == 0) y[i] = a.value();
}

__global__ __launch_bounds__(256) void prolong_kernel(int64_t rows, const int32_t* __restrict__ ptr,
                                                      const int32_t* __restrict__ col,
                                                      const double* __restrict__ val,
                                                      const double* __restrict__ s, const double* __restrict__ z0,
                                                      double* __restrict__ zfull) {
    const int64_t i = (int64_t)blockIdx.x * 256 + threadIdx.x;
    if (i >= rows) return;
    double v = z0[i];
    for (int32_t q = ptr[i]; q < ptr[i + 1]; ++q) v += val[q] * s[col[q]];
    zfull[i] = v;
}

__global__ __launch_bounds__(256) void step_kernel(const double* __restrict__ x, const double* __restrict__ nn,
                                                   double s, double* __restrict__ xn, int64_t len,
                                                   int32_t* __restrict__ moved, int32_t stamp) {
    const int64_t i = (int64_t)blockIdx.x * 256 + threadIdx.x;
    bool m = false;
    if (i < len) {
        const double xi = x[i];
        const double v = __builtin_fma(-s, nn[i], xi);
        xn[i] = v;
        m = (v != xi);
    }
    __shared__ int any_moved;
    if (threadIdx.x == 0) any_moved = 0;
    __syncthreads();
    if (m) any_moved = 1;
    __syncthreads();
    if (threadIdx.x == 0 && any_moved) *moved = stamp;
}

__global__ __launch_bounds__(256) void scale_copy_kernel(const double* __restrict__ src, double alpha,
                                                         double* __restrict__ dst, int64_t len) {
    const int64_t i = (int64_t)blockIdx.x * 256 + threadIdx.x;
    if (i < len) dst[i] = alpha * src[i];
}

__global__ __launch_bounds__(256) void border_tail_kernel(const double* __restrict__ g, double* __restrict__ tail, int64_t m) {
    const int64_t i = (int64_t)blockIdx.x * 256 + threadIdx.x;
    if (i < m) tail[i] = -1.0 * g[i];
    else if (i == m) tail[i] = -1.0;
}

__global__ __launch_bounds__(256) void axpy_kernel(double alpha, const double* __restrict__ x,
                                                   double* __restrict__ y, int64_t len) {
    const int64_t i = (int64_t)blockIdx.x * 256 + threadIdx.x;
    if (i < len) y[i] += alpha * x[i];
}

__global__ __launch_bounds__(256) void fill_kernel(double value, double* __restrict__ y, int64_t len) {
    const int64_t i = (int64_t)blockIdx.x * 256 + threadIdx.x;
    if (i < len) y[i] = value;
}

}

__global__ __launch_bounds__(256) void index_gather_kernel(const double* __restrict__ v, const int32_t* __restrict__ idx,
                                                           int64_t cnt, double* __restrict__ out) {
    const int64_t i = (int64_t)blockIdx.x * 256 + threadIdx.x;
    if (i < cnt) out[i] = v[idx[i]];
}
__global__ __launch_bounds__(256) void index_scatter_kernel(const double* __restrict__ in, const int32_t* __restrict__ idx,
                                                            int64_t cnt, double* __restrict__ v) {
    const int64_t i = (int64_t)blockIdx.x * 256 + threadIdx.x;
    if (i < cnt) v[idx[i]] = in[i];
}
void launch_index_gather(const double* v, const int32_t* idx, int64_t cnt, double* out, hipStream_t st) {
    if (cnt == 0) return;
    hipLaunchKernelGGL(index_gather_kernel, dim3((unsigned)((cnt + 255) / 256)), dim3(256), 0, st, v, idx, cnt, out);
    MGB_HIP_CHECK(hipGetLastError());
}
void launch_index_scatter(const double* in, const int32_t* idx, int64_t cnt, double* v, hipStream_t st) {
    if (cnt == 0) return;
    hipLaunchKernelGGL(index_scatter_kernel, dim3((unsigned)((cnt + 255) / 256)), dim3(256), 0, st, in, idx, cnt, v);
    MGB_HIP_CHECK(hipGetLastError());
}

void launch_csr_matvec(int64_t rows, const int32_t* ptr, const int32_t* col, const double* val,
                       const double* x, double* y, bool add, bool long_rows, hipStream_t st) {
    if (rows == 0) return;
    if (long_rows) {
        const dim3 grid((unsigned)((rows + 3) / 4));
        if (add) hipLaunchKernelGGL(csr_matvec_wave_kernel<true>, grid, dim3(256), 0, st, rows, ptr, col, val, x, y);
        else hipLaunchKernelGGL(csr_matvec_wave_kernel<false>, grid, dim3(256), 0, st, rows, ptr, col, val, x, y);
    } else {
        const dim3 grid((unsigned)((rows + 255) / 256));
        if (add) hipLaunchKernelGGL(csr_matvec_row_kernel<true>, grid, dim3(256), 0, st, rows, ptr, col, val, x, y);
        else hipLaunchKernelGGL(csr_matvec_row_kernel<false>, grid, dim3(256), 0, st, rows, ptr, col, val, x, y);
    }
    MGB_HIP_CHECK(hipGetLastError());
}

int csr_chunks(int64_t max_row_len) { return (int)((max_row_len + CHUNK - 1) / CHUNK); }

void launch_csr_matvec_chunked(int64_t rows, const int32_t* ptr, const int32_t* col, const double* val,
                               const double* x, double* y, double* scratch, int nchunk, hipStream_t st) {
    if (rows == 0) return;
    hipLaunchKernelGGL(csr_matvec_chunk_kernel, dim3((unsigned)nchunk, (unsigned)rows), dim3(256), 0, st, ptr, col, val, x,
                       scratch, nchunk);
    hipLaunchKernelGGL(csr_matvec_chunk_sum_kernel, dim3((unsigned)((rows + 3) / 4)), dim3(256), 0, st, rows, scratch,
                       nchunk, y);
    MGB_HIP_CHECK(hipGetLastError());
}

void launch_prolong(int64_t rows, const int32_t* ptr, const int32_t* col, const double* val, const double* s,
                    const double* z0, double* zfull, hipStream_t st) {
    if (rows == 0) return;
    hipLaunchKernelGGL(prolong_kernel, dim3((unsigned)((rows + 255) / 256)), dim3(256), 0, st, rows, ptr, col, val, s,
                       z0, zfull);
    MGB_HIP_CHECK(hipGetLastError());
}

void launch_step(const double* x, const double* n, double s, double* xn, int64_t len, int32_t* moved, int32_t stamp,
                 hipStream_t st) {
    if (len == 0) return;
    hipLaunchKernelGGL(step_kernel, dim3((unsigned)((len + 255) / 256)), dim3(256), 0, st, x, n, s, xn, len, moved, stamp);
    MGB_HIP_CHECK(hipGetLastError());
}

void launch_scale_copy(const double* src, double alpha, double* dst, int64_t len, hipStream_t st) {
    if (len == 0) return;
    hipLaunchKernelGGL(scale_copy_kernel, dim3((unsigned)((len + 255) / 256)), dim3(256), 0, st, src, alpha, dst, len);
    MGB_HIP_CHECK(hipGetLastError());
}

void launch_border_tail(const double* g, double* tail, int64_t m, hipStream_t st) {
    hipLaunchKernelGGL(border_tail_kernel, dim3((unsigned)((m + 1 + 255) / 256)), dim3(256), 0, st, g, tail, m);
    MGB_HIP_CHECK(hipGetLastError());
}

void launch_axpy(double alpha, const double* x, double* y, int64_t len, hipStream_t st) {
    if (len == 0) return;
    hipLaunchKernelGGL(axpy_kernel, dim3((unsigned)((len + 255) / 256)), dim3(256), 0, st, alpha, x, y, len);
    MGB_HIP_CHECK(hipGetLastError());
}

void launch_fill(double value, double* y, int64_t len, hipStream_t st) {
    if (len == 0) return;
    hipLaunchKernelGGL(fill_kernel, dim3((unsigned)((len + 255) / 256)), dim3(256), 0, st, value, y, len);
    MGB_HIP_CHECK(hipGetLastError());
}

}
```

### multigridbarrier.jl_amd/device.py

```python
from __future__ import annotations

import ctypes as C
import os
import weakref
from typing import List, Optional

import numpy as np
import scipy.sparse as sp

from .blockmatrices import BlockColumn, BlockDiag
from .convex import KIND_EP, KIND_LINEAR, Convex
from .multigrid import AMG
from .problem import MGBProblem

MAX_PIECES, MAX_IDX, MAX_ND, MAX_NU, MAX_OPS = 4, 10, 13, 4, 8
MAX_LIN = 4
OK, ERR_INVALID, ERR_HIP, ERR_NOT_SPD, ERR_NONFINITE, ERR_CONVERGENCE = range(6)


class Device:
    """reference: src/device.jl:18"""


class CPUDevice(Device):
    """Marker only: the native CPU path is the reference itself (src/device.jl:25)."""


class HIPDevice(Device):
    """The MI355X backend (the reference's `CUDADevice` slot, src/device.jl:32)."""


_DEFAULT = [HIPDevice]


def default_device():
    return _DEFAULT[0]


def default_device_set(D):
    _DEFAULT[0] = D
    return D



_dp = C.POINTER(C.c_double)
_ip = C.POINTER(C.c_int32)


class _Piece(C.Structure):
    _fields_ = [("kind", C.c_int32), ("ni", C.c_int32), ("nc", C.c_int32), ("idx", C.c_int32 * MAX_IDX),
                ("A", _dp), ("b", _dp), ("p", _dp), ("mu", _dp), ("p_const", C.c_double),
                ("mu_const", C.c_double), ("select", _dp)]


class _Cone(C.Structure):
    _fields_ = [("npieces", C.c_int32), ("pieces", _Piece * MAX_PIECES), ("feasibility", C.c_int32),
                ("NC", C.c_int32)]


class _CSR(C.Structure):
    _fields_ = [("rows", C.c_int64), ("cols", C.c_int64), ("rowptr", _ip), ("colidx", _ip), ("values", _dp)]


class _Desc(C.Structure):
    _fields_ = [("p", C.c_int32), ("N", C.c_int64), ("nu", C.c_int32), ("nD", C.c_int32), ("n_ops", C.c_int32),
                ("ops", _dp * MAX_OPS), ("D_state", C.c_int32 * MAX_ND), ("D_op", C.c_int32 * MAX_ND),
                ("w", _dp), ("L", C.c_int32), ("R", C.POINTER(_CSR)), ("cone", _Cone),
                ("barrier_weights", _dp), ("x", _dp), ("dim", C.c_int32)]


class Options(C.Structure):
    _fields_ = [("tol", C.c_double), ("t", C.c_double), ("kappa", C.c_double), ("maxit", C.c_int32),
                ("max_newton", C.c_int32), ("ls_beta", C.c_double), ("ls_c1", C.c_double),
                ("line_search", C.c_int32), ("stop_lambda_tol", C.c_double), ("stop_theta", C.c_double),
                ("finalize", C.c_int32), ("finalize_theta", C.c_double), ("early_stop", C.c_int32),
                ("stopping_criterion", C.c_void_p), ("early_stop_fn", C.c_void_p), ("user", C.c_void_p)]


STOP_FN = C.CFUNCTYPE(C.c_int, C.c_double, C.c_double, C.c_double, C.c_double, C.c_double, C.c_double, C.c_void_p)
EARLY_FN = C.CFUNCTYPE(C.c_int, C.POINTER(C.c_double), C.c_double, C.c_void_p)
ALLREDUCE_FN = C.CFUNCTYPE(C.c_int, C.c_void_p, C.c_void_p, C.c_int64, C.c_int32, C.c_int32)


class _CoreResult(C.Structure):
    _fields_ = [("k", C.c_int32), ("L", C.c_int32), ("failure_code", C.c_int32), ("t_final", C.c_double),
                ("t_elapsed", C.c_double), ("solve_seconds", C.c_double), ("newton_iterations", C.c_int64),
                ("f0_evals", C.c_int64), ("f1_evals", C.c_int64), ("f2_evals", C.c_int64),
                ("factorizations", C.c_int64), ("cap_steps", C.c_int32), ("its", C.POINTER(C.c_int64)),
                ("ts", _dp), ("kappas", _dp), ("times", _dp), ("c_dot_Dz", _dp)]


EXPORTS = [
    "mgbhip_create", "mgbhip_destroy", "mgbhip_last_error", "mgbhip_version", "mgbhip_problem_create",
    "mgbhip_problem_destroy", "mgbhip_problem_set_box", "mgbhip_problem_set_barrier_weights",
    "mgbhip_level_size", "mgbhip_f0", "mgbhip_f1", "mgbhip_f2", "mgbhip_hessian_pattern", "mgbhip_solve",
    "mgbhip_set_hessian", "mgbhip_solve_newton", "mgbhip_newton_direction", "mgbhip_problem_set_sharding",
    "mgbhip_problem_set_collective",
    "mgbhip_node_barrier", "mgbhip_node_slack", "mgbhip_mgb_core", "mgbhip_matched_t",
    "mgbhip_default_options", "mgbhip_stage_ms", "mgbhip_reset_stage_timers", "mgbhip_solver_stats", "mgbhip_solver_chain",
    "mgbhip_vec_alloc", "mgbhip_vec_free", "mgbhip_vec_len", "mgbhip_vec_upload", "mgbhip_vec_download",
    "mgbhip_vec_fill", "mgbhip_vec_copy", "mgbhip_vec_axpy", "mgbhip_vec_scale", "mgbhip_vec_dot",
    "mgbhip_vec_norm", "mgbhip_vec_isfinite", "mgbhip_f0_d", "mgbhip_f1_d", "mgbhip_f2_d", "mgbhip_solve_d",
    "mgbhip_prolong_add", "mgbhip_level_plan", "mgbhip_elem_plan", "mgbhip_trial_values", "mgbhip_solver_launches", "mgbhip_interpolate", "mgbhip_interpolate_grad",
    "mgbhip_locator_create", "mgbhip_locator_elements", "mgbhip_locator_evaluate", "mgbhip_locator_destroy",
    "mgbhip_closest_create", "mgbhip_closest_fetch", "mgbhip_closest_evaluate", "mgbhip_closest_destroy",
    "mgbhip_quadrature_create", "mgbhip_quadrature_points", "mgbhip_quadrature_weights", "mgbhip_quadrature_integrate",
    "mgbhip_quadrature_max", "mgbhip_quadrature_plan", "mgbhip_quadrature_times", "mgbhip_quadrature_destroy",
    "mgbhip_faces_create", "mgbhip_faces_topology", "mgbhip_faces_geometry", "mgbhip_faces_sizes", "mgbhip_faces_integrate",
    "mgbhip_faces_jumps", "mgbhip_faces_indicator", "mgbhip_faces_plan", "mgbhip_faces_times", "mgbhip_faces_destroy",
    "mgbhip_contour_create", "mgbhip_contour_fetch", "mgbhip_contour_destroy", "mgbhip_contour_create_embedded",
    "mgbhip_tessellate_create", "mgbhip_tessellate_fetch", "mgbhip_tessellate_destroy",
    "mgbhip_weld_create", "mgbhip_weld_fetch", "mgbhip_weld_rounds", "mgbhip_weld_destroy",
    "mgbhip_polyline_create", "mgbhip_polyline_fetch", "mgbhip_polyline_rounds", "mgbhip_polyline_destroy",
    "mgbhip_polyline_sample",
    "mgbhip_raycast_create", "mgbhip_raycast_offsets", "mgbhip_raycast_samples", "mgbhip_raycast_lengths",
    "mgbhip_raycast_integrate", "mgbhip_raycast_render", "mgbhip_raycast_destroy", "mgbhip_raycast_render_layers",
    "mgbhip_surface_create", "mgbhip_surface_trace", "mgbhip_surface_shade", "mgbhip_surface_destroy",
    "mgbhip_stream_create", "mgbhip_stream_set_field", "mgbhip_stream_trace", "mgbhip_stream_destroy",
    "mgbhip_tubes_create", "mgbhip_tubes_trace", "mgbhip_tubes_shade", "mgbhip_tubes_destroy",
    "mgbhip_figure_create", "mgbhip_figure_render", "mgbhip_figure_render_rgba8", "mgbhip_figure_counts",
    "mgbhip_figure_destroy",
]


def library_path() -> str:
    here = os.path.dirname(os.path.abspath(__file__))
    return os.environ.get("MGBHIP_LIB") or os.path.join(here, "lib", "libmgbhip.so")


_LIB = None


def load_library():
    global _LIB
    if _LIB is not None:
        return _LIB
    path = library_path()
    if not os.path.exists(path):
        raise RuntimeError(f"{path} not found: build it with `make -C multigridbarrier.jl_amd/csrc` "
                           "(or __graft_entry__.build()); this package has no CPU fallback")
    lib = C.CDLL(path)
    lib.mgbhip_last_error.restype = C.c_char_p
    lib.mgbhip_version.restype = C.c_char_p
    lib.mgbhip_level_size.restype = C.c_int64
    lib.mgbhip_level_size.argtypes = [C.c_void_p, C.c_int32]
    lib.mgbhip_create.argtypes = [C.POINTER(C.c_void_p), C.c_int, C.c_void_p]
    lib.mgbhip_destroy.argtypes = [C.c_void_p]
    lib.mgbhip_problem_create.argtypes = [C.c_void_p, C.POINTER(_Desc), C.c_void_p, C.POINTER(C.c_void_p)]
    lib.mgbhip_problem_destroy.argtypes = [C.c_void_p]
    lib.mgbhip_problem_set_box.argtypes = [C.c_void_p, C.c_double, C.c_double]
    lib.mgbhip_problem_set_barrier_weights.argtypes = [C.c_void_p, _dp]
    for name in ("mgbhip_f0", "mgbhip_f1", "mgbhip_f2"):
        getattr(lib, name).argtypes = [C.c_void_p, C.c_int32, _dp, _dp, _dp, _dp]
    lib.mgbhip_hessian_pattern.argtypes = [C.c_void_p, C.c_int32, C.POINTER(C.c_int64), C.POINTER(_ip), C.POINTER(_ip)]
    lib.mgbhip_solve.argtypes = [C.c_void_p, C.c_int32, _dp, _dp]
    lib.mgbhip_set_hessian.argtypes = [C.c_void_p, C.c_int32, _dp]
    lib.mgbhip_solve_newton.argtypes = [C.c_void_p, C.c_int32, _dp, _dp, _dp]
    lib.mgbhip_newton_direction.argtypes = [C.c_void_p, C.c_int32, _dp, _dp, _dp, _dp, _dp, _ip]
    lib.mgbhip_problem_set_sharding.argtypes = [C.c_void_p, C.c_int32, C.c_int64, _ip, _dp]
    lib.mgbhip_problem_set_collective.argtypes = [C.c_void_p, C.c_void_p, C.c_void_p, C.c_int32]
    lib.mgbhip_node_barrier.argtypes = [C.c_void_p, _dp, _dp, _dp]
    lib.mgbhip_node_slack.argtypes = [C.c_void_p, _dp, _dp]
    lib.mgbhip_mgb_core.argtypes = [C.c_void_p, _dp, _dp, C.POINTER(Options), C.POINTER(_CoreResult)]
    lib.mgbhip_matched_t.argtypes = [C.c_void_p, _dp, _dp, C.c_double, _dp]
    lib.mgbhip_default_options.argtypes = [C.POINTER(Options), C.c_int64]
    lib.mgbhip_default_options.restype = None
    lib.mgbhip_stage_ms.argtypes = [C.c_void_p, C.c_char_p, _dp, C.POINTER(C.c_int64)]
    lib.mgbhip_reset_stage_timers.argtypes = [C.c_void_p, C.c_int]
    lib.mgbhip_solver_stats.argtypes = [C.c_void_p, C.c_int32, _dp]
    lib.mgbhip_solver_chain.argtypes = [C.c_void_p, C.c_int32, _dp]
    lib.mgbhip_level_plan.argtypes = [C.c_void_p, C.c_int32, _ip]
    lib.mgbhip_elem_plan.argtypes = [C.c_void_p, C.c_int32, _ip]
    lib.mgbhip_trial_values.argtypes = [C.c_void_p, C.c_int32, _dp, _dp, C.c_double, _dp, _dp, _dp, _dp, _dp, _ip, _ip, _ip]
    lib.mgbhip_solver_launches.argtypes = [C.c_void_p, C.c_int32, _ip, C.c_int64]
    lib.mgbhip_solver_launches.restype = C.c_int64
    vp = C.c_void_p
    lib.mgbhip_vec_alloc.argtypes = [vp, C.c_int64, C.POINTER(vp)]
    lib.mgbhip_vec_free.argtypes = [vp]
    lib.mgbhip_vec_len.argtypes = [vp]
    lib.mgbhip_vec_len.restype = C.c_int64
    lib.mgbhip_vec_upload.argtypes = [vp, _dp, C.c_int64]
    lib.mgbhip_vec_download.argtypes = [vp, _dp, C.c_int64]
    lib.mgbhip_vec_fill.argtypes = [vp, C.c_double]
    lib.mgbhip_vec_copy.argtypes = [vp, vp]
    lib.mgbhip_vec_axpy.argtypes = [C.c_double, vp, vp]
    lib.mgbhip_vec_scale.argtypes = [C.c_double, vp]
    lib.mgbhip_vec_dot.argtypes = [vp, vp, _dp]
    lib.mgbhip_vec_norm.argtypes = [vp, _dp]
    lib.mgbhip_vec_isfinite.argtypes = [vp, C.POINTER(C.c_int32)]
    lib.mgbhip_f0_d.argtypes = [vp, C.c_int32, vp, vp, vp, _dp]
    lib.mgbhip_f1_d.argtypes = [vp, C.c_int32, vp, vp, vp, vp]
    lib.mgbhip_f2_d.argtypes = [vp, C.c_int32, vp, vp, vp]
    lib.mgbhip_solve_d.argtypes = [vp, C.c_int32, vp, vp]
    lib.mgbhip_prolong_add.argtypes = [vp, C.c_int32, vp, vp]
    lib.mgbhip_interpolate.argtypes = [vp, C.c_int32, C.c_int32, C.c_int32, C.c_int32, C.c_int64, _dp, _dp, C.c_int32,
                                       _dp, C.c_int64, _dp, _dp, _ip]
    lib.mgbhip_interpolate_grad.argtypes = [vp, C.c_int32, C.c_int32, C.c_int32, C.c_int32, C.c_int64, _dp, _dp,
                                            C.c_int32, _dp, C.c_int64, _dp, _dp, _dp, _ip]
    lib.mgbhip_locator_create.argtypes = [vp, C.c_int32, C.c_int32, C.c_int32, C.c_int32, C.c_int64, _dp, _dp, C.c_int64,
                                          _dp, C.POINTER(vp)]
    lib.mgbhip_locator_elements.argtypes = [vp, _ip]
    lib.mgbhip_locator_evaluate.argtypes = [vp, C.c_int32, _dp, _dp, _dp]
    lib.mgbhip_locator_destroy.argtypes = [vp]
    lib.mgbhip_closest_create.argtypes = [vp, C.c_int32, C.c_int32, C.c_int32, C.c_int64, _dp, _dp, C.c_int64, _dp, C.c_double,
                                          C.POINTER(vp)]
    lib.mgbhip_closest_fetch.argtypes = [vp, _ip, _dp, _dp, _dp, _ip]
    lib.mgbhip_closest_evaluate.argtypes = [vp, C.c_int32, _dp, _dp, _dp]
    lib.mgbhip_closest_destroy.argtypes = [vp]
    lib.mgbhip_quadrature_create.argtypes = [vp, C.c_int32, C.c_int32, C.c_int32, C.c_int64, _dp, C.c_int32, _dp, _dp, _dp,
                                             C.POINTER(vp)]
    lib.mgbhip_quadrature_points.argtypes = [vp, _dp]
    lib.mgbhip_quadrature_weights.argtypes = [vp, _dp]
    lib.mgbhip_quadrature_integrate.argtypes = [vp, C.c_int32, C.c_double, C.c_int32, _dp, _dp, _dp, _dp, _dp]
    lib.mgbhip_quadrature_max.argtypes = [vp, C.c_int32, C.c_int32, _dp, _dp, _dp]
    lib.mgbhip_quadrature_plan.argtypes = [C.c_int32, C.c_int32, C.c_int32, C.c_int32, C.c_int64, _ip]
    lib.mgbhip_quadrature_times.argtypes = [vp, _dp]
    lib.mgbhip_quadrature_destroy.argtypes = [vp]
    lib.mgbhip_faces_create.argtypes = [vp, C.c_int32, C.c_int32, C.c_int64, _dp, _ip, C.c_int32, C.c_int32, _dp, _dp, _dp, _dp,
                                        _dp, _ip, C.c_int32, _ip, C.POINTER(vp), C.POINTER(C.c_int64), C.POINTER(C.c_int64)]
    lib.mgbhip_faces_topology.argtypes = [vp, _ip, _ip, _ip, _ip]
    lib.mgbhip_faces_geometry.argtypes = [vp, C.c_int32, _dp, _dp, _dp]
    lib.mgbhip_faces_sizes.argtypes = [vp, _dp]
    lib.mgbhip_faces_integrate.argtypes = [vp, C.c_int32, C.c_double, C.c_int32, _dp, _dp, _dp, _dp]
    lib.mgbhip_faces_jumps.argtypes = [vp, C.c_int32, C.c_double, C.c_int32, _dp, _dp]
    lib.mgbhip_faces_indicator.argtypes = [vp, C.c_double, C.c_int32, _dp, _dp, _dp]
    lib.mgbhip_faces_plan.argtypes = [C.c_int32, C.c_int32, C.c_int32, C.c_int32, C.c_int32, C.c_int64, _ip]
    lib.mgbhip_faces_times.argtypes = [vp, _dp]
    lib.mgbhip_faces_destroy.argtypes = [vp]
    lib.mgbhip_contour_create.argtypes = [vp, C.c_int32, C.c_int32, C.c_int32, C.c_int32, C.c_int64, _dp, _dp, C.c_int32,
                                          _dp, C.c_int32, _dp, C.c_int32, C.POINTER(vp), C.POINTER(C.c_int64)]
    lib.mgbhip_contour_create_embedded.argtypes = [vp, C.c_int32, C.c_int32, C.c_int32, C.c_int32, C.c_int32, C.c_int64, _dp,
                                                   _dp, C.c_int32, _dp, C.c_int32, _dp, C.c_int32, C.POINTER(vp),
                                                   C.POINTER(C.c_int64)]
    lib.mgbhip_tessellate_create.argtypes = [vp, C.c_int32, C.c_int32, C.c_int32, C.c_int32, C.c_int32, C.c_int64, _dp, _dp,
                                             C.c_int32, _dp, C.c_int32, C.POINTER(vp), C.POINTER(C.c_int64)]
    lib.mgbhip_tessellate_fetch.argtypes = [vp, _dp, _ip, _dp]
    lib.mgbhip_tessellate_destroy.argtypes = [vp]
    lib.mgbhip_contour_fetch.argtypes = [vp, _dp, _ip, _ip, _dp]
    lib.mgbhip_contour_destroy.argtypes = [vp]
    lib.mgbhip_weld_create.argtypes = [vp, C.c_int64, C.c_int32, C.c_int32, _dp, _ip, C.c_double, C.c_int32, C.POINTER(vp),
                                       C.POINTER(C.c_int64), C.POINTER(C.c_int64)]
    lib.mgbhip_weld_fetch.argtypes = [vp, _ip, _ip, _ip, _dp]
    lib.mgbhip_weld_rounds.argtypes = [vp, _ip, _ip]
    lib.mgbhip_weld_destroy.argtypes = [vp]
    _lp = C.POINTER(C.c_int64)
    lib.mgbhip_polyline_create.argtypes = [vp, C.c_int64, C.c_int32, _dp, C.c_int64, _ip, C.POINTER(vp), _lp, _lp, _lp]
    lib.mgbhip_polyline_fetch.argtypes = [vp, _lp, _ip, _ip, C.POINTER(C.c_uint8), _dp, _dp]
    lib.mgbhip_polyline_rounds.argtypes = [vp, _ip, _ip]
    lib.mgbhip_polyline_destroy.argtypes = [vp]
    lib.mgbhip_polyline_sample.argtypes = [vp, C.c_int32, C.c_int64, _dp, C.c_int32, _dp, C.c_int64, _lp, _dp, C.c_int64,
                                           _ip, _dp, _dp, _dp]
    lib.mgbhip_raycast_create.argtypes = [vp, C.c_int32, C.c_int32, C.c_int32, C.c_int32, C.c_int64, _dp, _dp, C.c_int64,
                                          _dp, _dp, _dp, C.c_double, C.c_double, C.c_double, C.POINTER(vp),
                                          C.POINTER(C.c_int64)]
    lib.mgbhip_raycast_offsets.argtypes = [vp, C.POINTER(C.c_int64)]
    lib.mgbhip_raycast_samples.argtypes = [vp, _dp]
    lib.mgbhip_raycast_lengths.argtypes = [vp, _dp, _dp]
    lib.mgbhip_raycast_integrate.argtypes = [vp, C.c_int32, _dp, _dp]
    lib.mgbhip_raycast_render.argtypes = [vp, _dp, C.c_int32, _dp, C.c_double, C.c_double, _dp]
    lib.mgbhip_raycast_destroy.argtypes = [vp]
    lib.mgbhip_raycast_render_layers.argtypes = [vp, _dp, C.c_int32, _dp, C.c_double, C.c_double, C.c_int32, _dp, _dp, _dp]
    lib.mgbhip_surface_create.argtypes = [vp, C.c_int64, _dp, C.POINTER(vp)]
    lib.mgbhip_surface_trace.argtypes = [vp, C.c_int64, _dp, _dp, C.c_double, C.c_double, C.c_int32, _dp, _ip, _dp, _dp]
    lib.mgbhip_surface_shade.argtypes = [vp, C.c_int64, C.c_int32, _dp, _ip, _dp, _dp, _dp, C.c_int32, _dp, C.c_double,
                                         C.c_double, C.c_double, _dp]
    lib.mgbhip_surface_destroy.argtypes = [vp]
    lib.mgbhip_tubes_create.argtypes = [vp, C.c_int64, _dp, _dp, C.POINTER(vp)]
    lib.mgbhip_tubes_trace.argtypes = [vp, C.c_int64, _dp, _dp, C.c_double, C.c_double, C.c_int32, _dp, _ip, _dp]
    lib.mgbhip_tubes_shade.argtypes = [vp, C.c_int64, C.c_int32, _dp, _dp, _dp, _ip, _dp, _dp, C.c_int32, _dp, C.c_double,
                                       C.c_double, C.c_double, _dp]
    lib.mgbhip_tubes_destroy.argtypes = [vp]
    lib.mgbhip_stream_create.argtypes = [vp, C.c_int32, C.c_int32, C.c_int32, C.c_int32, C.c_int64, _dp, _dp, C.c_int32, _dp,
                                         C.POINTER(vp)]
    lib.mgbhip_stream_set_field.argtypes = [vp, _dp]
    lib.mgbhip_stream_trace.argtypes = [vp, C.c_int64, _dp, C.c_double, C.c_int32, C.c_int32, C.c_double, _dp, _ip, _ip]
    lib.mgbhip_stream_destroy.argtypes = [vp]
    lib.mgbhip_figure_create.argtypes = [vp, C.c_int32, C.c_int32, C.c_int32, C.c_int32, C.c_int64, _dp, _dp, C.c_int64,
                                         _dp, _dp, _dp, C.c_double, C.c_int32, C.c_int32, _dp, C.c_int32, _ip, _dp,
                                         C.c_int32, _dp, _dp, C.c_double, C.c_double, C.c_double, C.c_int32,
                                         C.POINTER(vp)]
    lib.mgbhip_figure_render.argtypes = [vp, _dp, _dp]
    lib.mgbhip_figure_render_rgba8.argtypes = [vp, _dp, _dp, C.POINTER(C.c_uint8)]
    lib.mgbhip_figure_counts.argtypes = [vp, C.POINTER(C.c_int64), C.POINTER(C.c_int64)]
    lib.mgbhip_figure_destroy.argtypes = [vp]
    _LIB = lib
    return lib


class MGBHipError(RuntimeError):
    def __init__(self, status, message):
        super().__init__(f"libmgbhip status {status}: {message}")
        self.status = status


def _check(lib, status):
    if status != OK:
        raise MGBHipError(status, lib.mgbhip_last_error().decode())


def _ptr(a: Optional[np.ndarray]):
    return None if a is None else a.ctypes.data_as(_dp)


def _f64(a, order="C") -> np.ndarray:
    return np.require(a, dtype=np.float64, requirements=["C" if order == "C" else "F", "ALIGNED"])


class HipContext:

    def __init__(self, device_id: int = 0, stream: Optional[int] = None):
        self.lib = load_library()
        h = C.c_void_p()
        _check(self.lib, self.lib.mgbhip_create(C.byref(h), int(device_id), C.c_void_p(stream) if stream else None))
        self.handle = h
        self._vectors = weakref.WeakSet()

    def close(self):
        if self.handle:
            for v in list(self._vectors):
                v.close()
            self.lib.mgbhip_destroy(self.handle)
            self.handle = None

    def __del__(self):
        try:
            self.close()
        except Exception:
            pass
# ... 274 lines not shown
        lam, cond = C.c_double(), C.c_int32()
        _check(self.lib, self.lib.mgbhip_newton_direction(self.handle, level, _ptr(s), _ptr(c), _ptr(z0), _ptr(x),
                                                          C.cast(C.byref(lam), _dp), C.byref(cond)))
        return x, lam.value, bool(cond.value)

    def node_barrier(self, z, want_Dz: bool = False):
        z = _f64(z)
        F = np.empty(self.n)
        Dz = np.empty((self.n, self.nD), order="F") if want_Dz else None
        _check(self.lib, self.lib.mgbhip_node_barrier(self.handle, _ptr(z), _ptr(F), _ptr(Dz)))
        return (F, Dz) if want_Dz else F

    def node_slack(self, z) -> np.ndarray:
        z = _f64(z)
        out = np.empty(self.n)
        _check(self.lib, self.lib.mgbhip_node_slack(self.handle, _ptr(z), _ptr(out)))
        return out

    def set_sharding(self, shards, collective, accepts_device_ptr: bool = False):
        for level, sh in enumerate(shards):
            ic = np.ascontiguousarray(sh.iface, dtype=np.int32)
            own = _f64(sh.own)
            _check(self.lib, self.lib.mgbhip_problem_set_sharding(self.handle, level, ic.size, ic.ctypes.data_as(_ip), _ptr(own)))
        self._collective = collective
        _check(self.lib, self.lib.mgbhip_problem_set_collective(self.handle, C.cast(collective, C.c_void_p), None,
                                                               1 if accepts_device_ptr else 0))

    def set_box(self, b: float, R: float):
        _check(self.lib, self.lib.mgbhip_problem_set_box(self.handle, float(b), float(R)))

    def set_barrier_weights(self, bw):
        a = None if bw is None else _f64(bw)
        _check(self.lib, self.lib.mgbhip_problem_set_barrier_weights(self.handle, _ptr(a)))

    def default_options(self, n_nodes: Optional[int] = None) -> Options:
        o = Options()
        self.lib.mgbhip_default_options(C.byref(o), int(self.n if n_nodes is None else n_nodes))
        return o

    def mgb_core(self, z, c, opt: Options, cap_steps: int = 256):
        z = _f64(z).copy()
        c = np.asfortranarray(c, dtype=np.float64)
        L = len(self.level_sizes)
        its = np.zeros((L, cap_steps), dtype=np.int64, order="F")
        ts, kappas, times, cdz = (np.zeros(cap_steps) for _ in range(4))
        r = _CoreResult()
        r.cap_steps = cap_steps
        r.its = its.ctypes.data_as(C.POINTER(C.c_int64))
        r.ts, r.kappas, r.times, r.c_dot_Dz = _ptr(ts), _ptr(kappas), _ptr(times), _ptr(cdz)
        status = self.lib.mgbhip_mgb_core(self.handle, _ptr(z), _ptr(c), C.byref(opt), C.byref(r))
        if status not in (OK, ERR_CONVERGENCE):
            _check(self.lib, status)
        k = min(r.k, cap_steps)
        diag = dict(its=its[:, :k].copy(), ts=ts[:k].copy(), kappas=kappas[:k].copy(), times=times[:k].copy(),
                    c_dot_Dz=cdz[:k].copy(), t_elapsed=r.t_elapsed, t_final=r.t_final,
                    solve_seconds=r.solve_seconds, newton_iterations=int(r.newton_iterations),
                    f0_evals=int(r.f0_evals), f1_evals=int(r.f1_evals), f2_evals=int(r.f2_evals),
                    factorizations=int(r.factorizations), failure_code=int(r.failure_code), k=int(r.k))
        return status, z, diag

    def matched_t(self, z, c, t_default: float) -> float:
        z = _f64(z)
        c = np.asfortranarray(c, dtype=np.float64)
        out = C.c_double()
        _check(self.lib, self.lib.mgbhip_matched_t(self.handle, _ptr(z), _ptr(c), float(t_default), C.cast(C.byref(out), _dp)))
        return out.value

    def reset_stage_timers(self, enable: bool = True):
        _check(self.lib, self.lib.mgbhip_reset_stage_timers(self.handle, 1 if enable else 0))

    def stage_ms(self, stage: str):
        ms, cnt = C.c_double(), C.c_int64()
        _check(self.lib, self.lib.mgbhip_stage_ms(self.handle, stage.encode(), C.cast(C.byref(ms), _dp), C.byref(cnt)))
        return ms.value, cnt.value

    def solver_stats(self, level: int) -> dict:
        out = np.zeros(8)
        _check(self.lib, self.lib.mgbhip_solver_stats(self.handle, level, _ptr(out)))
        keys = ("fronts", "max_front", "arena_doubles", "factor_flops", "peeled", "tree_levels", "nnz", "unknowns")
        return dict(zip(keys, out.tolist()))

    def solver_chain(self, level: int) -> dict:
        out = np.zeros(8)
        _check(self.lib, self.lib.mgbhip_solver_chain(self.handle, level, _ptr(out)))
        keys = ("pivot_blocks_on_critical_path", "large_front_tree_levels", "launches_per_factorization",
                "launches_per_backward_sweep", "arena_doubles", "factor_flops", "extra_trailing_doubles", "reserved")
        return dict(zip(keys, out.tolist()))

    PLAN_KEYS = ("R_unit", "R_long", "T_long", "T_chunks", "selection", "acc", "acc_split", "long_lists", "gather_chunk",
                 "gather_nchunk", "projection", "max_row", "max_col", "cmax", "mean_list", "planned")
    PROJECTION = ("none", "loop", "staged", "mfma", "accumulate")

    def level_plan(self, level: int) -> dict:
        out = (C.c_int32 * 16)()
        _check(self.lib, self.lib.mgbhip_level_plan(self.handle, level, out))
        d = dict(zip(self.PLAN_KEYS, (int(v) for v in out)))
        d["projection"] = self.PROJECTION[d["projection"]]
        d["direct"] = bool(d["selection"] & 2)
        d["selection"] = bool(d["selection"] & 1)
        for k in ("R_unit", "R_long", "T_long", "acc", "long_lists", "planned"):
            d[k] = bool(d[k])
        return d

    ELEM_MODES = ("f0", "f1", "f2", "node_F", "node_slack", "f01")
    ELEM_KINDS = ("dense", "wide", "fast_default", "fast_runtime", "condense", "generic")

    def elem_plan(self, mode) -> dict:
        mode = self.ELEM_MODES.index(mode) if isinstance(mode, str) else int(mode)
        out = (C.c_int32 * 16)()
        _check(self.lib, self.lib.mgbhip_elem_plan(self.handle, mode, out))
        keys = ("kind", "NY", "P", "threads", "G", "EPB", "grid", "lds", "nstage", "unstaged", "ymask", "newton_kind")
        d = dict(zip(keys, (int(v) for v in out)))
        d["kind"], d["newton_kind"] = self.ELEM_KINDS[d["kind"]], self.ELEM_KINDS[d["newton_kind"]]
        return d

    def trial_values(self, level: int, x, direction, step: float, c, z0) -> dict:
        x, direction, c, z0 = _f64(x), _f64(direction), np.asfortranarray(c, dtype=np.float64), _f64(z0)
        m = self.level_sizes[level]
        g, xn = np.empty(m), np.empty(m)
        y, moved, finite, path = C.c_double(), C.c_int32(), C.c_int32(), C.c_int32()
        _check(self.lib, self.lib.mgbhip_trial_values(self.handle, level, _ptr(x), _ptr(direction), float(step), _ptr(c), _ptr(z0),
                                                      C.cast(C.byref(y), _dp), _ptr(g), _ptr(xn), C.byref(moved), C.byref(finite),
                                                      C.byref(path)))
        return dict(y=y.value, g=g, xn=xn, moved=int(moved.value), finite=int(finite.value), on_the_fly=bool(path.value & 1),
                    fused_restrict=bool(path.value & 2))

    LAUNCH_KEYS = ("level", "first", "count", "cls", "max_m", "max_k", "max_child", "tiny", "wave", "inv", "iface", "packed",
                   "assembly", "block0", "backward")
    ASSEMBLY = ("none", "gather", "columns")
    BLOCK0 = ("n/a", "gather", "diag0", "step0")
    BACKWARD = ("n/a", "k8", "k16", "general")

    @classmethod
    def launch_rows(cls, raw) -> list:
        rows = []
        for r in np.asarray(raw, dtype=np.int64).reshape(-1, 16):
            d = dict(zip(cls.LAUNCH_KEYS, (int(v) for v in r)))
            for k in ("tiny", "wave", "inv", "iface", "packed"):
                d[k] = bool(d[k])
            d["assembly"], d["block0"], d["backward"] = cls.ASSEMBLY[d["assembly"]], cls.BLOCK0[d["block0"]], cls.BACKWARD[d["backward"]]
            rows.append(d)
        return rows

    def solver_launches(self, level: int) -> list:
        n = self.lib.mgbhip_solver_launches(self.handle, level, None, 0)
        if n < 0:
            _check(self.lib, int(-n))
        out = (C.c_int32 * (16 * max(int(n), 1)))()
        n = self.lib.mgbhip_solver_launches(self.handle, level, out, n)
        if n < 0:
            _check(self.lib, int(-n))
        return self.launch_rows(np.frombuffer(out, dtype=np.int32)[:16 * int(n)])

    def close(self):
        if self.handle:
            self.lib.mgbhip_problem_destroy(self.handle)
            self.handle = None

    def __del__(self):
        try:
            self.close()
        except Exception:
            pass


def dense_as_block(M: AMG) -> AMG:
    if isinstance(M.D_fine[0], BlockColumn):
        return M
    n = M.w.size
    geom = M.geometry
    ops = {k: BlockDiag(np.asarray(v, dtype=np.float64).reshape(n, n, 1)) for k, v in geom.operators.items()}
    from dataclasses import replace
    g2 = replace(geom, operators=ops)
    nu = len(M.state_names)
    D_fine = [BlockColumn(ops[name], state, nu) for (state, name) in M.D_spec]
    return AMG(geometry=g2, x=M.x, w=M.w, R_fine=M.R_fine, D_fine=D_fine, state_names=M.state_names, D_spec=M.D_spec)


class DeviceMGBProblem:

    def __init__(self, prob: MGBProblem, device_id: int = 0, stream: Optional[int] = None, shards=None, collective=None,
                 accepts_device_ptr: bool = False):
        self.prob = prob
        self.ctx = HipContext(device_id, stream)
        self.M1 = dense_as_block(prob.M[0])
        self.main = DeviceProblem(self.ctx, self.M1, prob.Q)
        self._feas = None
        self._shards, self._collective, self._coll_dev = shards, collective, accepts_device_ptr
        if shards is not None:
            self.main.set_sharding(shards[0], collective, accepts_device_ptr)

    @property
    def feasibility(self) -> DeviceProblem:
        if self._feas is None:
            M2 = dense_as_block(self.prob.M[1])
            self._feas = DeviceProblem(self.ctx, M2, self.prob.Q, feasibility=True, NC=self.main.nD + 1,
                                       share=self.main)
            if self._shards is not None:
                self._feas.set_sharding(self._shards[1], self._collective, self._coll_dev)
        return self._feas

    def close(self):
        if self._feas is not None:
            self._feas.close()
        self.main.close()
        self.ctx.close()


def native_to_device(D, prob: MGBProblem, **kw) -> DeviceMGBProblem:
    if D is HIPDevice:
        return DeviceMGBProblem(prob, **kw)
    raise RuntimeError(f"native_to_device: device {getattr(D, '__name__', D)} is unavailable in this package "
                       "(only HIPDevice is implemented; the CPU path is the reference itself)")


def device_to_native(D, sol):
    return sol


def mgb_cleanup(dev: Optional[DeviceMGBProblem] = None):
    if dev is not None:
        dev.close()
```

Before: 691.7.

## Skip trivial border root factor/solve and replace z copies with buffer swaps

When the bordered system's root front is a 1x1 border node, the factor and backward passes skip that last level and set the border solution entry to one directly, either in the border-tail kernel or with a small copy. Device-to-device copies of the z vector before each Newton level and around the kappa retry are replaced by pointer swaps. The prolongation now writes into the alternate buffer through a new add-to matvec kernel. Counters and an API for launch statistics are added. The intent is to cut kernel launches and memory copies per Newton step, at the cost of fragile guard-state logic and a new border-pivot finiteness check.

New measurement: 697.9, median of 3. No clear change (+0.9%).

```diff
diff --git a/include/mgbhip.h b/include/mgbhip.h
--- a/include/mgbhip.h
+++ b/include/mgbhip.h
@@ -185,6 +185,7 @@
 enum { MGBHIP_B0_NA = 0, MGBHIP_B0_GATHER = 1, MGBHIP_B0_DIAG0 = 2, MGBHIP_B0_STEP0 = 3 };
 enum { MGBHIP_BWD_NA = 0, MGBHIP_BWD_K8 = 1, MGBHIP_BWD_K16 = 2, MGBHIP_BWD_GENERAL = 3 };
 int64_t mgbhip_solver_launches(mgbhip_problem* prob, int32_t level, int32_t* out, int64_t cap);
+int mgbhip_newton_launch_counts(mgbhip_problem* prob, int64_t* out8);
 
 #define MGBHIP_INTERP_FEM1D 1
 #define MGBHIP_INTERP_QK 2
diff --git a/multigridbarrier.jl_amd/csrc/api.cpp b/multigridbarrier.jl_amd/csrc/api.cpp
--- a/multigridbarrier.jl_amd/csrc/api.cpp
+++ b/multigridbarrier.jl_amd/csrc/api.cpp
@@ -765,6 +765,16 @@
     MGB_REQUIRE(out != nullptr, "null argument");
     MGB_REQUIRE(P->levels[level].solver.analyzed, "mgbhip_solver_chain: the level has not been factored yet");
     P->levels[level].solver.chain_stats(out);
+    return MGBHIP_OK;
+    MGB_API_END
+}
+
+int mgbhip_newton_launch_counts(mgbhip_problem* P, int64_t* out) {
+    MGB_API_BEGIN
+    MGB_REQUIRE(P != nullptr && out != nullptr, "null argument");
+    const mgbhip::Counters& c = P->cnt;
+    out[0] = c.newton; out[1] = c.waits; out[2] = c.finish; out[3] = c.border_tail;
+    out[4] = c.z_copies; out[5] = c.solver_rows; out[6] = c.factor; out[7] = c.robust_factor;
     return MGBHIP_OK;
     MGB_API_END
 }
diff --git a/multigridbarrier.jl_amd/csrc/driver.cpp b/multigridbarrier.jl_amd/csrc/driver.cpp
--- a/multigridbarrier.jl_amd/csrc/driver.cpp
+++ b/multigridbarrier.jl_amd/csrc/driver.cpp
@@ -16,6 +16,10 @@
 
 bool debug_on() {
     static const bool on = env_on("MGBHIP_DEBUG");
+    return on;
+}
+bool z_copies() {
+    static const bool on = env_on("MGBHIP_Z_COPIES");
     return on;
 }
 #define DBG(...) do { if (debug_on()) { fprintf(stderr, __VA_ARGS__); } } while (0)
@@ -43,6 +47,7 @@
 
 VecStats vec_stats(mgbhip_problem* P, int level, const double* d_v, int64_t len) {
     hipStream_t st = P->stream();
+    ++P->cnt.finish;
     launch_vec_stats(d_v, len, P->d_scratch.p, P->d_scal.p + 2, st, P->own_mask(level));
     P->read_scalars(2, 2);
     if (P->sharded()) P->allreduce_host(P->pin.d + 2, 2, 0);
@@ -51,6 +56,7 @@
 
 double dev_dot(mgbhip_problem* P, int level, const double* a, const double* b, int64_t len) {
     hipStream_t st = P->stream();
+    ++P->cnt.finish;
     launch_dot(a, b, len, P->d_scratch.p, P->d_scal.p + 4, st, P->own_mask(level));
     P->read_scalars(4, 1);
     if (P->sharded()) P->allreduce_host(P->pin.d + 4, 1, 0);
@@ -92,6 +98,7 @@
     if (restrict_fused_out) *restrict_fused_out = restrict_fused;
     if (onfly && !restrict_fused) launch_step(P->d_x.p, P->d_nv.p, *step, P->d_xn.p, C.m, P->d_flag.p, P->step_stamp, st);
     const double seq = P->next_seq();
+    ++P->cnt.finish;
     launch_trial_finish(P->d_gn.p, C.m, P->d_scratch.p, fused ? P->d_partials.p : nullptr, elem_grid(P->p, P->N), P->d_scal.p,
                         P->d_flag.p, P->pin.dev, st, P->own_mask(C.level), seq, restrict_fused);
     P->wait_results(seq);
@@ -207,11 +214,13 @@
             P->factor(C.level, C.rhs_of_g());
             P->trisolve_carried(C.level, P->d_nv.p);
             const double seq = P->next_seq();
+            ++P->cnt.finish;
             launch_dir_finish(P->d_nv.p, P->d_g.p, C.m, P->d_scratch.p, P->d_scal.p, L.solver.status_flags_rw(), P->pin.dev, st,
                               P->own_mask(C.level), seq);
             L.solver.flags_cleared();
             P->wait_results(seq);
-            P->pin.i[1] = P->pin.d[5] != 0.0 ? 1 : 0;
+            const bool border_pivot_bad = L.solver.border_skipped() && !std::isfinite(P->pin.d[4]);
+            P->pin.i[1] = (P->pin.d[5] != 0.0 || border_pivot_bad) ? 1 : 0;
             leaf_flag |= P->pin.d[6] != 0.0 ? 1 : 0;
             P->pin.i[2] = leaf_flag;
             fstatus = MfSolver::status_from(P->pin.i + 1, L.solver.factored_condensed);
@@ -231,6 +240,7 @@
         }
         if (fstatus != MGBHIP_OK && P->lu_fallback(C.level, P->d_g.p, P->d_nv.p)) {
             DBG("newton[lev %d] k=%d: LDL' met a zero pivot; direction from the pivoted LU fallback\n", C.level, k);
+            ++P->cnt.finish;
             launch_dir_finish(P->d_nv.p, P->d_g.p, C.m, P->d_scratch.p, P->d_scal.p, L.solver.status_flags_rw(), P->pin.dev, st,
                               P->own_mask(C.level));
             L.solver.flags_cleared();
@@ -294,14 +304,29 @@
     auto eta = [&](int j, int J, const Stop& stop, int maxit) -> bool {
         (void)j;
         const int lev = J - 1;
-        MGB_HIP_CHECK(hipMemcpyAsync(P->d_z0.p, P->d_z.p, zn * sizeof(double), hipMemcpyDeviceToDevice, st));
-        NewtonCtx C{P, lev, P->d_z0.p, d_c, P->levels[lev].m};
+        const Level& Lv = P->levels[lev];
+        const bool swap_form = !z_copies() && (size_t)Lv.rows == zn;
+        if (!swap_form) {
+            MGB_HIP_CHECK(hipMemcpyAsync(P->d_z0.p, P->d_z.p, zn * sizeof(double), hipMemcpyDeviceToDevice, st));
+            ++P->cnt.z_copies;
+        }
+        NewtonCtx C{P, lev, swap_form ? P->d_z.p : P->d_z0.p, d_c, Lv.m};
         NewtonResult r = newton(C, opt, stop, maxit);
         out.its[lev] += r.k;
         if (r.converged) {
-            const Level& Lv = P->levels[lev];
             StageScope scp(P->ctx->timers, "prolong");
-            launch_csr_matvec(Lv.rows, Lv.Rptr.p, Lv.Rcol.p, Lv.Rval.p, P->d_x.p, P->d_z.p, true, false, st);
+            if (swap_form) {
+                launch_csr_matvec_add_to(Lv.rows, Lv.Rptr.p, Lv.Rcol.p, Lv.Rval.p, P->d_x.p, P->d_z.p, P->d_z0.p, st);
+                std::swap(P->d_z, P->d_z0);
+                if (P->z_guard == 1) { std::swap(P->d_z0, P->d_tmp); P->z_guard = 2; }
+            } else {
+                if (P->z_guard == 1) {
+                    MGB_HIP_CHECK(hipMemcpyAsync(P->d_tmp.p, P->d_z.p, zn * sizeof(double), hipMemcpyDeviceToDevice, st));
+                    ++P->cnt.z_copies;
+                    P->z_guard = 2;
+                }
+                launch_csr_matvec(Lv.rows, Lv.Rptr.p, Lv.Rcol.p, Lv.Rval.p, P->d_x.p, P->d_z.p, true, false, st);
+            }
         }
         return r.converged;
     };
@@ -370,6 +395,7 @@
     P->d_z.upload(z, zn, st);
     P->d_c0.upload(c, cn, st);
     P->cnt = Counters();
+    P->z_guard = 0;
     auto tb = std::chrono::steady_clock::now();
     auto now = [&] { return std::chrono::duration<double>(std::chrono::steady_clock::now() - tb).count(); };
     double t = opt.t;
@@ -433,8 +459,14 @@
             const double t1 = kappa * t;
             setc(t1);
             P->d_tmp.ensure(zn);
-            MGB_HIP_CHECK(hipMemcpyAsync(P->d_tmp.p, P->d_z.p, zn * sizeof(double), hipMemcpyDeviceToDevice, st));
+            if (z_copies()) {
+                MGB_HIP_CHECK(hipMemcpyAsync(P->d_tmp.p, P->d_z.p, zn * sizeof(double), hipMemcpyDeviceToDevice, st));
+                ++P->cnt.z_copies;
+            } else
+                P->z_guard = 1;
             S = mgb_step(P, P->d_c.p, opt, opt.finalize && t1 >= target, false);
+            const int guard = P->z_guard;
+            P->z_guard = 0;
             record(k, S.its, true);
             if (S.converged) {
                 int64_t mx = 0;
@@ -443,7 +475,11 @@
                 t = t1;
                 break;
             }
-            MGB_HIP_CHECK(hipMemcpyAsync(P->d_z.p, P->d_tmp.p, zn * sizeof(double), hipMemcpyDeviceToDevice, st));
+            if (z_copies()) {
+                MGB_HIP_CHECK(hipMemcpyAsync(P->d_z.p, P->d_tmp.p, zn * sizeof(double), hipMemcpyDeviceToDevice, st));
+                ++P->cnt.z_copies;
+            } else if (guard == 2)
+                std::swap(P->d_z, P->d_tmp);
             kappa = std::sqrt(kappa);
         }
         diag(k);
diff --git a/multigridbarrier.jl_amd/csrc/kernels.hpp b/multigridbarrier.jl_amd/csrc/kernels.hpp
--- a/multigridbarrier.jl_amd/csrc/kernels.hpp
+++ b/multigridbarrier.jl_amd/csrc/kernels.hpp
@@ -98,6 +98,8 @@
 
 void launch_csr_matvec(int64_t rows, const int32_t* ptr, const int32_t* col, const double* val,
                        const double* x, double* y, bool add, bool long_rows, hipStream_t st);
+void launch_csr_matvec_add_to(int64_t rows, const int32_t* ptr, const int32_t* col, const double* val, const double* x,
+                              const double* base, double* out, hipStream_t st);
 int csr_chunks(int64_t max_row_len);
 void launch_csr_matvec_chunked(int64_t rows, const int32_t* ptr, const int32_t* col, const double* val,
                                const double* x, double* y, double* scratch, int nchunk, hipStream_t st);
@@ -106,7 +108,7 @@
 void launch_step(const double* x, const double* n, double s, double* xn, int64_t len, int32_t* moved, int32_t stamp,
                  hipStream_t st);
 void launch_scale_copy(const double* src, double alpha, double* dst, int64_t len, hipStream_t st);
-void launch_border_tail(const double* g, double* tail, int64_t m, hipStream_t st);
+void launch_border_tail(const double* g, double* tail, int64_t m, hipStream_t st, double* x_border = nullptr);
 void launch_axpy(double alpha, const double* x, double* y, int64_t len, hipStream_t st);
 void launch_fill(double value, double* y, int64_t len, hipStream_t st);
 
diff --git a/multigridbarrier.jl_amd/csrc/mf_numeric.hip b/multigridbarrier.jl_amd/csrc/mf_numeric.hip
--- a/multigridbarrier.jl_amd/csrc/mf_numeric.hip
+++ b/multigridbarrier.jl_amd/csrc/mf_numeric.hip
@@ -174,6 +174,25 @@
             if (!L.cls) max_big = std::max(max_big, L.count);
         }
     d_dscr.alloc((size_t)max_big * 2 * NB * NB);
+    {
+        static const bool off = env_on("MGBHIP_NO_BORDER_SKIP");
+        bool ok = !off && plan.border && !level_launches.empty() && !level_solves.empty();
+        for (auto& lev : level_launches)
+            for (auto& L : lev) ok = ok && !L.iface;
+        if (ok) {
+            int live = 0;
+            const MfLaunch* root = nullptr;
+            for (auto& L : level_launches.back())
+                if (L.count) { ++live; root = &L; }
+            int live_s = 0;
+            for (auto& L : level_solves.back())
+                if (L.count) ++live_s;
+            ok = live == 1 && live_s == 1 && root->count == 1 && root->cls != 0 && root->first == nf - 1 && plan.fronts[nf - 1].m == 1 &&
+                 plan.fronts[nf - 1].k == 1 && plan.front_idx[plan.fronts[nf - 1].idx_off] == (int32_t)plan.n;
+        }
+        border_skip_ok = ok;
+        border_skipped_ = false;
+    }
     {
         int64_t need[2] = {0, 0};
         if (sw.bwd_split) bwd_split_scratch(level_solves, need);
@@ -217,7 +236,7 @@
     MGB_HIP_CHECK(hipStreamSynchronize(st));
 }
 
-void MfSolver::factor(const double* d_values, hipStream_t st, StageTimers* timers, bool direct, bool condensed) {
+void MfSolver::factor(const double* d_values, hipStream_t st, StageTimers* timers, bool direct, bool condensed, bool carried) {
     MGB_REQUIRE(!direct || d_a_src_direct.n > 0, "MfSolver::factor: no direct value map");
     MGB_REQUIRE(!condensed || (direct && condensed_ok), "MfSolver::factor: condensed leaves are not enabled");
     MGB_REQUIRE(analyzed, "MfSolver::factor before analyze");
@@ -230,12 +249,16 @@
     if (!status_zero) MGB_HIP_CHECK(hipMemsetAsync(d_status.p, 0, sizeof(int32_t), st));
     status_zero = false;
     factored_condensed = condensed;
+    border_skipped_ = carried && border_skip_ok && !robust;
+    const int last_level = (int)level_launches.size() - 1;
     int lvno = -1;
     for (auto& lev : level_launches) {
         LevelScope lvscope(timers, "fac", ++lvno);
         for (auto& L : lev) {
             if (L.count == 0) continue;
             if (condensed && lvno == 0) continue;
+            if (border_skipped_ && lvno == last_level) continue;
+            ++rows_issued;
             if (L.tiny) launch_factor_tiny(a, L);
             else if (L.wave && L.cls <= 32) launch_factor_wave<32>(a, L);
             else if (L.wave) launch_factor_wave<48>(a, L);
@@ -278,7 +301,7 @@
     if (timers) timers->end();
 }
 
-void MfSolver::solve_border(double* d_x_np1, hipStream_t st, StageTimers* timers) {
+void MfSolver::solve_border(double* d_x_np1, hipStream_t st, StageTimers* timers, bool x_border_set) {
     MGB_REQUIRE(analyzed, "MfSolver::solve_border before analyze");
     if (timers) timers->begin("trisolve");
     const size_t n = (size_t)plan.n;
@@ -290,7 +313,8 @@
         MGB_HIP_CHECK(hipMemcpyAsync(d_y.p + n, d_one.p, sizeof(double), hipMemcpyDeviceToDevice, st));
         y_border_one = true;
     }
-    backward_pass(d_x_np1, st, timers);
+    if (border_skipped_ && !x_border_set) MGB_HIP_CHECK(hipMemcpyAsync(d_x_np1 + n, d_one.p, sizeof(double), hipMemcpyDeviceToDevice, st));
+    backward_pass(d_x_np1, st, timers, border_skipped_);
     MGB_HIP_CHECK(hipGetLastError());
     if (timers) timers->end();
 }
@@ -313,13 +337,16 @@
     }
 }
 
-void MfSolver::backward_pass(double* d_x, hipStream_t st, StageTimers* timers) {
+void MfSolver::backward_pass(double* d_x, hipStream_t st, StageTimers* timers, bool skip_border_root) {
     const SolveArgs a = solve_args(nullptr, d_x, st);
-    for (int32_t l = (int32_t)level_solves.size() - 1; l >= 0; --l) {
+    const int32_t top = (int32_t)level_solves.size() - 1;
+    for (int32_t l = top; l >= 0; --l) {
+        if (skip_border_root && l == top) continue;
         LevelScope lvscope(timers, "bwd", l);
         for (auto it = level_solves[l].rbegin(); it != level_solves[l].rend(); ++it) {
             const MfLaunch& L = *it;
             if (L.count == 0) continue;
+            ++rows_issued;
             if (L.tiny) launch_backward_tiny(a, L);
             else if (L.cls) launch_backward_small(a, L);
             else if (L.inv && factored_inv) launch_bwd_inv(a, L);
diff --git a/multigridbarrier.jl_amd/csrc/mf_solver.hpp b/multigridbarrier.jl_amd/csrc/mf_solver.hpp
--- a/multigridbarrier.jl_amd/csrc/mf_solver.hpp
+++ b/multigridbarrier.jl_amd/csrc/mf_solver.hpp
@@ -46,7 +46,8 @@
                  const double* coords = nullptr, int dim = 0, bool protect_peeled = false,
                  const int32_t* top = nullptr, int64_t ntop = 0);
     std::function<void(double*, int64_t)> iface_reduce;
-    void factor(const double* d_values, hipStream_t st, StageTimers* timers, bool direct = false, bool condensed = false);
+    void factor(const double* d_values, hipStream_t st, StageTimers* timers, bool direct = false, bool condensed = false,
+                bool carried = false);
     bool enable_condensed(int64_t N, int P, const int32_t* ucol, int64_t slack0, int64_t nnz, int64_t tail_base, hipStream_t st);
     bool condensed_ready() const { return condensed_ok; }
     bool leaves_packed() const { return leaf_packed; }
@@ -61,7 +62,10 @@
     void set_direct_map(const int32_t* value_map, int64_t nnz, int64_t tail_base, hipStream_t st);
     bool has_direct_map() const { return d_a_src_direct.n > 0; }
     void solve(const double* d_b, double* d_x, hipStream_t st, StageTimers* timers);
-    void solve_border(double* d_x_np1, hipStream_t st, StageTimers* timers);
+    void solve_border(double* d_x_np1, hipStream_t st, StageTimers* timers, bool x_border_set = false);
+    bool border_skip() const { return border_skip_ok; }
+    bool border_skipped() const { return border_skipped_; }
+    int64_t rows_issued = 0;
     void chain_stats(double* out8) const;
     int64_t launches(int32_t* out, int64_t cap) const;
     int status(hipStream_t st);
@@ -82,7 +86,7 @@
                 d_uvec.p, d_tbig.p, d_tsol.p, st, d_bwd_g.p, d_bwd_cnt.n ? d_bwd_cnt.p : nullptr};
     }
     void forward_pass(const double* d_b_np1, hipStream_t st, StageTimers* timers);
-    void backward_pass(double* d_x_np1, hipStream_t st, StageTimers* timers);
+    void backward_pass(double* d_x_np1, hipStream_t st, StageTimers* timers, bool skip_border_root = false);
     DevBuf<double> d_bx, d_xx, d_one;
     DevBuf<FrontDev> d_fronts;
     DevBuf<int32_t> d_front_idx, d_children, d_rel, d_a_src, d_a_src_direct, d_a_dst, d_a_colptr;
@@ -106,6 +110,8 @@
     int gather_ct = 0;
     int32_t lds_cap = 88;
     bool uses_inv = false;
+    bool border_skip_ok = false;
+    bool border_skipped_ = false;
     bool y_border_one = false;
     bool y_zero = false;
     bool status_zero = false, leaf_zero = false;
diff --git a/multigridbarrier.jl_amd/csrc/problem.cpp b/multigridbarrier.jl_amd/csrc/problem.cpp
--- a/multigridbarrier.jl_amd/csrc/problem.cpp
+++ b/multigridbarrier.jl_amd/csrc/problem.cpp
@@ -716,6 +716,7 @@
 void mgbhip_problem::wait_results(double seq) {
     static const bool poll = !env_on("MGBHIP_NO_POLL");
     hipStream_t st = stream();
+    ++cnt.waits;
     if (poll && seq != 0.0) {
         volatile const double* stamp = pin.d + 15;
         const Stopwatch sw;
@@ -840,19 +841,26 @@
     const FactorPlan plan = L.H.about_to_factor(hel_owner, level, rhs);
     hipStream_t st = stream();
     ensure_analysis(level);
+    const bool carried = plan.write == HTail::Rhs;
+    const int64_t rows0 = L.solver.rows_issued;
+    if (carried) ++cnt.border_tail;
+    if (L.solver.robust) ++cnt.robust_factor;
+    double* x_border = (carried && L.solver.border_skip() && d_nv.n >= (size_t)L.m + 1) ? d_nv.p + L.m : nullptr;
     if (plan.slab()) {
         ensure_direct(level);
-        launch_border_tail(rhs, d_hel.p + hel_cap + L.nshared, L.m, st);
-        L.solver.factor(d_hel.p, st, &ctx->timers, true, plan.condensed());
+        launch_border_tail(rhs, d_hel.p + hel_cap + L.nshared, L.m, st, x_border);
+        L.solver.factor(d_hel.p, st, &ctx->timers, true, plan.condensed(), true);
     } else {
         if (plan.write == HTail::Rhs) {
-            launch_border_tail(rhs, L.Hval.p + L.nnz, L.m, st);
+            launch_border_tail(rhs, L.Hval.p + L.nnz, L.m, st, x_border);
         } else if (plan.write == HTail::Identity) {
             MGB_HIP_CHECK(hipMemsetAsync(L.Hval.p + L.nnz, 0, sizeof(double) * (size_t)L.m, st));
             launch_fill(1.0, L.Hval.p + L.nnz + L.m, 1, st);
         }
-        L.solver.factor(L.Hval.p, st, &ctx->timers);
-    }
+        L.solver.factor(L.Hval.p, st, &ctx->timers, false, false, carried);
+    }
+    cnt.solver_rows += L.solver.rows_issued - rows0;
+    nv_border_level = x_border ? level : -1;
     L.H.factors_ready(plan);
     cnt.factor++;
 }
@@ -877,11 +885,16 @@
 void mgbhip_problem::trisolve(int level, const double* d_g, double* d_xout) {
     Level& L = levels[level];
     L.H.may_solve();
+    nv_border_level = -1;
     L.solver.solve(d_g, d_xout, stream(), &ctx->timers);
 }
 
 void mgbhip_problem::trisolve_carried(int level, double* d_xout_np1) {
     Level& L = levels[level];
     L.H.may_solve_carried();
-    L.solver.solve_border(d_xout_np1, stream(), &ctx->timers);
-}
+    const bool x_border_set = nv_border_level == level && d_xout_np1 == d_nv.p;
+    nv_border_level = -1;
+    const int64_t rows0 = L.solver.rows_issued;
+    L.solver.solve_border(d_xout_np1, stream(), &ctx->timers, x_border_set);
+    cnt.solver_rows += L.solver.rows_issued - rows0;
+}
diff --git a/multigridbarrier.jl_amd/csrc/problem.hpp b/multigridbarrier.jl_amd/csrc/problem.hpp
--- a/multigridbarrier.jl_amd/csrc/problem.hpp
+++ b/multigridbarrier.jl_amd/csrc/problem.hpp
@@ -86,6 +86,7 @@
 struct Counters {
     int64_t f0 = 0, f1 = 0, f2 = 0, factor = 0, newton = 0;
     double solve_seconds = 0;
+    int64_t waits = 0, finish = 0, border_tail = 0, z_copies = 0, solver_rows = 0, robust_factor = 0;
 };
 
 }
@@ -111,6 +112,7 @@
     mgbhip::DevBuf<double> d_z, d_z0, d_zfull, d_c, d_ret, d_hel, d_partials, d_scal, d_scratch, d_nodeF, d_nodeDz, d_dnDz, d_dnY, d_tchunk;
     mgbhip::DevBuf<double> d_x, d_g, d_nv, d_xn, d_gn, d_tmp, d_c0;
     mgbhip::DevBuf<int32_t> d_flag;
+    int z_guard = 0;
     int32_t step_stamp = 0;
     mgbhip::PinnedBuf pin;
     mgbhip::Counters cnt;
@@ -164,6 +166,7 @@
     void factor(int level, const double* rhs = nullptr);
     void trisolve(int level, const double* d_g, double* d_xout);
     void trisolve_carried(int level, double* d_xout_np1);
+    int nv_border_level = -1;
     bool lu_fallback(int level, const double* d_g, double* d_xout);
     mgbhip::DevBuf<double> d_lu;
     mgbhip::DevBuf<int32_t> d_lustat;
diff --git a/multigridbarrier.jl_amd/csrc/vector_kernels.hpp b/multigridbarrier.jl_amd/csrc/vector_kernels.hpp
--- a/multigridbarrier.jl_amd/csrc/vector_kernels.hpp
+++ b/multigridbarrier.jl_amd/csrc/vector_kernels.hpp
@@ -16,6 +16,18 @@
     double s = 0.0;
     for (int32_t q = ptr[i]; q < ptr[i + 1]; ++q) s += val[q] * x[col[q]];
     y[i] = ADD ? y[i] + s : s;
+}
+
+__global__ __launch_bounds__(256) void csr_matvec_row_add_to_kernel(int64_t rows, const int32_t* __restrict__ ptr,
+                                                                    const int32_t* __restrict__ col,
+                                                                    const double* __restrict__ val,
+                                                                    const double* __restrict__ x,
+                                                                    const double* __restrict__ base, double* __restrict__ out) {
+    const int64_t i = (int64_t)blockIdx.x * 256 + threadIdx.x;
+    if (i >= rows) return;
+    double s = 0.0;
+    for (int32_t q = ptr[i]; q < ptr[i + 1]; ++q) s += val[q] * x[col[q]];
+    out[i] = base[i] + s;
 }
 
 template <bool ADD>
@@ -111,10 +123,14 @@
     if (i < len) dst[i] = alpha * src[i];
 }
 
-__global__ __launch_bounds__(256) void border_tail_kernel(const double* __restrict__ g, double* __restrict__ tail, int64_t m) {
+__global__ __launch_bounds__(256) void border_tail_kernel(const double* __restrict__ g, double* __restrict__ tail, int64_t m,
+                                                          double* __restrict__ x_border) {
     const int64_t i = (int64_t)blockIdx.x * 256 + threadIdx.x;
     if (i < m) tail[i] = -1.0 * g[i];
-    else if (i == m) tail[i] = -1.0;
+    else if (i == m) {
+        tail[i] = -1.0;
+        if (x_border) *x_border = 1.0;
+    }
 }
 
 __global__ __launch_bounds__(256) void axpy_kernel(double alpha, const double* __restrict__ x,
@@ -166,6 +182,14 @@
     MGB_HIP_CHECK(hipGetLastError());
 }
 
+void launch_csr_matvec_add_to(int64_t rows, const int32_t* ptr, const int32_t* col, const double* val, const double* x,
+                              const double* base, double* out, hipStream_t st) {
+    if (rows == 0) return;
+    hipLaunchKernelGGL(csr_matvec_row_add_to_kernel, dim3((unsigned)((rows + 255) / 256)), dim3(256), 0, st, rows, ptr, col, val, x,
+                       base, out);
+    MGB_HIP_CHECK(hipGetLastError());
+}
+
 int csr_chunks(int64_t max_row_len) { return (int)((max_row_len + CHUNK - 1) / CHUNK); }
 
 void launch_csr_matvec_chunked(int64_t rows, const int32_t* ptr, const int32_t* col, const double* val,
@@ -199,8 +223,8 @@
     MGB_HIP_CHECK(hipGetLastError());
 }
 
-void launch_border_tail(const double* g, double* tail, int64_t m, hipStream_t st) {
-    hipLaunchKernelGGL(border_tail_kernel, dim3((unsigned)((m + 1 + 255) / 256)), dim3(256), 0, st, g, tail, m);
+void launch_border_tail(const double* g, double* tail, int64_t m, hipStream_t st, double* x_border) {
+    hipLaunchKernelGGL(border_tail_kernel, dim3((unsigned)((m + 1 + 255) / 256)), dim3(256), 0, st, g, tail, m, x_border);
     MGB_HIP_CHECK(hipGetLastError());
 }
 
diff --git a/multigridbarrier.jl_amd/device.py b/multigridbarrier.jl_amd/device.py
--- a/multigridbarrier.jl_amd/device.py
+++ b/multigridbarrier.jl_amd/device.py
@@ -101,7 +101,7 @@
     "mgbhip_vec_alloc", "mgbhip_vec_free", "mgbhip_vec_len", "mgbhip_vec_upload", "mgbhip_vec_download",
     "mgbhip_vec_fill", "mgbhip_vec_copy", "mgbhip_vec_axpy", "mgbhip_vec_scale", "mgbhip_vec_dot",
     "mgbhip_vec_norm", "mgbhip_vec_isfinite", "mgbhip_f0_d", "mgbhip_f1_d", "mgbhip_f2_d", "mgbhip_solve_d",
-    "mgbhip_prolong_add", "mgbhip_level_plan", "mgbhip_elem_plan", "mgbhip_trial_values", "mgbhip_solver_launches", "mgbhip_interpolate", "mgbhip_interpolate_grad",
+    "mgbhip_prolong_add", "mgbhip_level_plan", "mgbhip_elem_plan", "mgbhip_trial_values", "mgbhip_solver_launches", "mgbhip_newton_launch_counts", "mgbhip_interpolate", "mgbhip_interpolate_grad",
     "mgbhip_locator_create", "mgbhip_locator_elements", "mgbhip_locator_evaluate", "mgbhip_locator_destroy",
     "mgbhip_closest_create", "mgbhip_closest_fetch", "mgbhip_closest_evaluate", "mgbhip_closest_destroy",
     "mgbhip_quadrature_create", "mgbhip_quadrature_points", "mgbhip_quadrature_weights", "mgbhip_quadrature_integrate",
@@ -174,6 +174,7 @@
     lib.mgbhip_trial_values.argtypes = [C.c_void_p, C.c_int32, _dp, _dp, C.c_double, _dp, _dp, _dp, _dp, _dp, _ip, _ip, _ip]
     lib.mgbhip_solver_launches.argtypes = [C.c_void_p, C.c_int32, _ip, C.c_int64]
     lib.mgbhip_solver_launches.restype = C.c_int64
+    lib.mgbhip_newton_launch_counts.argtypes = [C.c_void_p, C.POINTER(C.c_int64)]
     vp = C.c_void_p
     lib.mgbhip_vec_alloc.argtypes = [vp, C.c_int64, C.POINTER(vp)]
     lib.mgbhip_vec_free.argtypes = [vp]
@@ -754,6 +755,12 @@
             _check(self.lib, int(-n))
         return self.launch_rows(np.frombuffer(out, dtype=np.int32)[:16 * int(n)])
 
+    def newton_launch_counts(self) -> dict:
+        out = (C.c_int64 * 8)()
+        _check(self.lib, self.lib.mgbhip_newton_launch_counts(self.handle, out))
+        keys = ("newton", "waits", "finish", "border_tail", "z_copies", "solver_launches", "factorizations", "robust_factorizations")
+        return dict(zip(keys, (int(v) for v in out)))
+
     def close(self):
         if self.handle:
             self.lib.mgbhip_problem_destroy(self.handle)
```
